# vitoplantamura/OnnxStream

Measured on AMD Instinct MI355X. Metric: sd15_unet_step_latency_ms+images_per_sec_512x512_20step, higher is better.
Workload: dtype f16

## Files before the change

### include/osgpu.h

```cpp
#ifndef OSGPU_H
#define OSGPU_H

#include <stddef.h>
#include <stdint.h>

#ifdef __cplusplus
extern "C" {
#endif

typedef struct osg_ctx osg_ctx;
typedef struct osg_graph osg_graph;

typedef enum { OSG_U8 = 1, OSG_F16 = 2, OSG_F32 = 3, OSG_I64 = 4 } osg_dtype;

typedef enum {
  OSG_ACT_NONE = 0,
  OSG_ACT_SILU = 1,
  OSG_ACT_SIGMOID = 2,
  OSG_ACT_GEGLU = 3
} osg_act;

typedef enum {
  OSG_UN_SIGMOID = 0,
  OSG_UN_ERF = 1,
  OSG_UN_SQRT = 2,
  OSG_UN_SIN = 3,
  OSG_UN_COS = 4,
  OSG_UN_NEG = 5,
  OSG_UN_POW = 6,
  OSG_UN_SILU = 7,
  OSG_UN_GELU_ERF = 8
} osg_unary_kind;

typedef enum {
  OSG_BIN_ADD = 0,
  OSG_BIN_SUB = 1,
  OSG_BIN_MUL = 2,
  OSG_BIN_DIV = 3
} osg_binary_kind;

int osg_device_count(void);
int osg_init(int device, osg_ctx** out);
void osg_destroy(osg_ctx* ctx);
const char* osg_last_error(const osg_ctx* ctx);
const char* osg_device_name(const osg_ctx* ctx);
void* osg_stream(const osg_ctx* ctx);
int osg_set_autotune(osg_ctx* ctx, int on);
int osg_tune_misses(void);

int osg_malloc(osg_ctx* ctx, size_t bytes, void** dptr);
int osg_free(osg_ctx* ctx, void* dptr);
int osg_upload(osg_ctx* ctx, void* dst, const void* host_src, size_t bytes);
int osg_upload_sync(osg_ctx* ctx, void* dst, const void* host_src, size_t bytes);
int osg_host_register(osg_ctx* ctx, void* host_ptr, size_t bytes);
int osg_host_unregister(osg_ctx* ctx, void* host_ptr);
int osg_upload_pinned(osg_ctx* ctx, void* dst, const void* pinned_host_src, size_t bytes);
int osg_upload_pinned_async(osg_ctx* ctx, void* dst, const void* pinned_host_src, size_t bytes);
int osg_copy_fence(osg_ctx* ctx);
int osg_download(osg_ctx* ctx, void* host_dst, const void* src, size_t bytes);
int osg_marker_record(osg_ctx* ctx, int slot);
int osg_copy_wait_marker(osg_ctx* ctx, int slot);
int osg_copy(osg_ctx* ctx, void* dst, const void* src, size_t bytes);
int osg_memset(osg_ctx* ctx, void* dst, int value, size_t bytes);
int osg_sync(osg_ctx* ctx);

int osg_graph_begin(osg_ctx* ctx);
int osg_graph_end(osg_ctx* ctx, osg_graph** out);
int osg_graph_launch(osg_ctx* ctx, osg_graph* g);
void osg_graph_destroy(osg_graph* g);

int osg_timer_start(osg_ctx* ctx);
int osg_timer_stop(osg_ctx* ctx, float* ms);
int osg_timer_mark(osg_ctx* ctx, int index);
int osg_timer_between(osg_ctx* ctx, int a, int b, float* ms);

void osg_range_push(const char* name);
void osg_range_pop(void);

int osg_conv2d_nhwc(osg_ctx* ctx, osg_dtype dtype, const void* x, const void* w_ohwi, const void* bias, osg_dtype bias_dtype,
                    const void* residual, void* y, int N, int H, int W, int Cin, int Cout, int KH, int KW, int stride_h,
                    int stride_w, int pad_top, int pad_left, int pad_bottom, int pad_right, osg_act act);

int osg_conv2d_nhwc_rb(osg_ctx* ctx, osg_dtype dtype, const void* x, const void* w_ohwi, const void* bias, osg_dtype bias_dtype,
                       const void* image_bias, long image_bias_ld, const void* residual, void* y, int N, int H, int W, int Cin, int Cout,
                       int KH, int KW, int stride_h, int stride_w, int pad_top, int pad_left, int pad_bottom, int pad_right, osg_act act);

int osg_conv2d_nhwc_v(osg_ctx* ctx, osg_dtype dtype, const void* x, const void* w_ohwi, const void* bias, osg_dtype bias_dtype,
                      const void* image_bias, long image_bias_ld, const void* residual, void* y, long y_ld, void* y2, long y2_ld, int N, int H, int W,
                      int Cin, int Cout, int KH, int KW, int stride_h, int stride_w, int pad_top, int pad_left, int pad_bottom, int pad_right,
                      osg_act act);

int osg_gemm(osg_ctx* ctx, osg_dtype dtype, const void* A, const void* B, int b_is_nk, const void* bias, osg_dtype bias_dtype,
             const void* residual, void* C, int M, int N, int K, int batch, long stride_a, long stride_b, long stride_c,
             osg_act act);

int osg_gemm_w8(osg_ctx* ctx, const void* A, const void* Bq_nk, float w_scale, int w_zero_point, const void* bias, osg_dtype bias_dtype,
                const void* residual, void* C, int M, int N, int K, osg_act act);
int osg_conv2d_nhwc_w8(osg_ctx* ctx, const void* x, const void* wq_ohwi, float w_scale, int w_zero_point, const void* bias,
                       osg_dtype bias_dtype, const void* image_bias, long image_bias_ld, const void* residual, void* y, int N, int H, int W,
                       int Cin, int Cout, int KH, int KW, int stride_h, int stride_w, int pad_top, int pad_left, int pad_bottom,
                       int pad_right, osg_act act);
int osg_gemm_w8_v(osg_ctx* ctx, const void* A, const void* Bq_nk, float w_scale, int w_zero_point, const float* w_scale_vec,
                  const float* w_zero_point_vec, const void* bias, osg_dtype bias_dtype, const void* residual, void* C, int M, int N, int K,
                  osg_act act);
int osg_conv2d_nhwc_w8_v(osg_ctx* ctx, const void* x, const void* wq_ohwi, float w_scale, int w_zero_point, const float* w_scale_vec,
                         const float* w_zero_point_vec, const void* bias, osg_dtype bias_dtype, const void* image_bias, long image_bias_ld,
                         const void* residual, void* y, long y_ld, void* y2, long y2_ld, int N, int H, int W, int Cin, int Cout, int KH, int KW,
                         int stride_h, int stride_w, int pad_top, int pad_left, int pad_bottom, int pad_right, osg_act act);

int osg_transpose_kn_to_nk(osg_ctx* ctx, osg_dtype dtype, const void* src_kn, void* dst_nk, int K, int N);
int osg_gemm_ln(osg_ctx* ctx, const void* x, const void* w_nk_folded, const float* c1, const float* c2, float eps, const float* rowstats,
                const void* residual, void* y, int M, int N, int K, osg_act act);
int osg_gemm_rowstats(osg_ctx* ctx, const void* A, const void* B_nk, const void* bias, osg_dtype bias_dtype, const void* residual, void* C,
                      int M, int N, int K, osg_act act, float* rowstats);
int osg_last_route(const osg_ctx* ctx, int out[5]);
int osg_last_kernel(const osg_ctx* ctx, int out[8]);

int osg_gemm_kernarg_check(osg_ctx* ctx, long lda, int splits);
int osg_attention_kernarg_check(osg_ctx* ctx, long kv_stride, int heads, int kv_div);

int osg_attention(osg_ctx* ctx, osg_dtype dtype, const void* q, const void* k, const void* v, void* o, int heads, int Tq, int Tkv,
                  int D, float scale, int k_is_dt);
int osg_attention_strided(osg_ctx* ctx, osg_dtype dtype, const void* q, long q_tok, long q_head, long q_batch, const void* k,
                          long k_tok, long k_head, long k_batch, const void* v, long v_tok, long v_head, long v_batch, void* o,
                          long o_tok, long o_head, long o_batch, int batch, int heads, int Tq, int Tkv, int D, float scale);
typedef struct {
  const void *a1, *x0;
  const void *wo1, *bo1;
  const void *g2, *be2;
  float eps2;
  const void *wq2, *bq2;
  const void *kp, *vtp;
  float scale;
  int Tk;
  const void *wo2, *bo2;
  const void *g3, *be3;
  float eps3;
  const void *w1, *b1, *w2, *b2;
  const void *wpo, *bpo, *xin;
  void *out, *out2;
  long ldo, ldo2;
  int M, rows_per_img, C, heads;
  void* dbg[8];
  int rows_per_block;
} osg_tblock_tail_args;
int osg_tblock_tail_supported(int M, int rows_per_img, int C, int heads, int Tk);
int osg_tblock_tail(osg_ctx* ctx, const osg_tblock_tail_args* a);
int osg_tblock_pack_weight(osg_ctx* ctx, const void* w_nk, int N, int K, void* w_kn8);
size_t osg_tblock_kv_pack_elems(int imgs, int heads, int D);
int osg_tblock_kv_pack_jobs(osg_ctx* ctx, const void* base, long ld, int imgs, int Tk, int heads, int njobs, const int* jobs_dev, void* dst);
int osg_rms_norm(osg_ctx* ctx, osg_dtype dtype, const void* x, const void* w, void* y, long rows, int C, float eps);
int osg_rope(osg_ctx* ctx, osg_dtype dtype, const void* x, const void* cos_t, const void* sin_t, void* y, long bh, long T, int d);
int osg_sdpa(osg_ctx* ctx, osg_dtype dtype, const void* q, const void* k, const void* v, const void* mask, void* o, int batch, int q_heads,
             int kv_heads, int Tq, int Tkv, int D, float scale);

int osg_instance_norm(osg_ctx* ctx, osg_dtype dtype, const void* x, const float* scale, const float* bias, void* y, int rows,
                      long L, int n_scale, float eps);
int osg_group_norm_nhwc(osg_ctx* ctx, osg_dtype dtype, const void* x, const void* gamma, const void* beta, void* y, int N, long HW,
                        int C, int groups, float eps, osg_act act);
int osg_set_stat_sinks(osg_ctx* ctx, void* table0, int groups0, int cpg0, int ch_off0, void* table1, int groups1, int cpg1, int ch_off1, int rows_per_image);
int osg_group_norm_stats_nhwc(osg_ctx* ctx, const void* x, const void* gamma, const void* beta, void* y, int N, long HW, int C, int G, float eps, osg_act act,
                              const void* stat_table);
int osg_layer_norm(osg_ctx* ctx, osg_dtype dtype, const void* x, const void* gamma, const void* beta, void* y, long rows, int C,
                   float eps);
int osg_reduce_mean_last(osg_ctx* ctx, osg_dtype dtype, const void* x, void* y, long rows, long C);
int osg_softmax_last(osg_ctx* ctx, osg_dtype dtype, const void* x, void* y, long rows, long C);

int osg_unary(osg_ctx* ctx, osg_dtype dtype, osg_unary_kind kind, const void* x, void* y, long n, float param);
int osg_binary(osg_ctx* ctx, osg_dtype dtype, osg_binary_kind kind, const void* a, const long* a_shape, const void* b,
               const long* b_shape, void* y, int rank);
int osg_geglu(osg_ctx* ctx, osg_dtype dtype, const void* x, void* y, long rows, long C);

int osg_sampler_prepare(osg_ctx* ctx, const float* x, float* sample, float* timestep, int prompts, long L, float c_in, float t,
                        long t_per_sample);
int osg_sampler_cfg_euler_a(osg_ctx* ctx, float* x, const float* eps, const float* noise, int prompts, long L, float c_out,
                            float guidance, float sigma, float d_sigma, float sigma_up, float clip);
typedef enum {
    OSG_MS_DPMPP_FIRST = 0, OSG_MS_DPMPP_2M = 1, OSG_MS_EULER_D = 2, OSG_MS_IPNDM1 = 3, OSG_MS_IPNDM_V1 = 4, OSG_MS_IPNDM2 = 5, OSG_MS_IPNDM3 = 6,
    OSG_MS_IPNDM_VO1 = 7, OSG_MS_IPNDM_VO2 = 8, OSG_MS_IPNDM_VO3 = 9, OSG_MS_TAYLOR1 = 10, OSG_MS_TAYLOR2 = 11, OSG_MS_DDIM = 12, OSG_MS_FORMS = 13
} osg_multistep_form;
int osg_sampler_cfg_multistep(osg_ctx* ctx, int form, float* x, const float* eps, float* h0, const float* h1, const float* h2, const float* h3,
                              int prompts, long L, float c_out, float guidance, float sigma, float k0, float k1, float k2, float k3, float k4,
                              double da, double db);
int osg_sampler_prepare_rescale(osg_ctx* ctx, float* x, float* sample, float* timestep, int prompts, long L, float x_scale, float c_in, float t,
                                long t_per_sample);
int osg_sampler_prepare_single(osg_ctx* ctx, float* x, float* sample, float* timestep, int prompts, long L, float x_scale, float c_in, float t,
                               long t_per_sample);
int osg_sampler_euler_a_single(osg_ctx* ctx, float* x, const float* eps, const float* noise, int prompts, long L, float c_out, float sigma,
                               float d_sigma, float sigma_up, float clip);
int osg_sampler_multistep_single(osg_ctx* ctx, int form, float* x, const float* eps, float* h0, const float* h1, const float* h2, const float* h3,
                                 int prompts, long L, float c_out, float sigma, float k0, float k1, float k2, float k3, float k4, double da,
                                 double db);

int osg_decode_gather(osg_ctx* ctx, const float* latents, float* tiles, int images, int H, int W, int tile, float factor);
int osg_decode_blend(osg_ctx* ctx, const float* tiles, float* image, unsigned char* pixels, int images, int H, int W, int tile, int up);

int osg_transpose(osg_ctx* ctx, int elem_size, const void* x, void* y, int rank, const long* shape, const int* perm);
int osg_copy_2d(osg_ctx* ctx, int elem_size, const void* src, long src_pitch, long src_off, void* dst, long dst_pitch,
                long dst_off, long outer, long inner);
int osg_concat2(osg_ctx* ctx, int elem_size, const void* a, long inner_a, const void* b, long inner_b, void* dst, long outer);
int osg_resize_nearest(osg_ctx* ctx, int elem_size, const void* x, void* y, int N, int C, int H, int W, int Ho, int Wo, int nhwc);
int osg_gather_rows(osg_ctx* ctx, int elem_size, const void* x, const int64_t* idx, void* y, long n_idx, long row_elems, long n_rows);
int osg_maxpool_nhwc(osg_ctx* ctx, osg_dtype dtype, const void* x, void* y, int N, int H, int W, int C, int KH, int KW, int sh,
                     int sw, int pt, int pl, int pb, int pr);

int osg_convert(osg_ctx* ctx, osg_dtype src_dtype, osg_dtype dst_dtype, const void* x, void* y, long n, float scale, int zero_point);

int osg_qu8_conv2d_nhwc(osg_ctx* ctx, const void* x, float x_scale, int x_zp, const void* w_ohwi, float w_scale, int w_zp, const float* bias_f32,
                        float out_scale, int out_zp, void* y, int N, int H, int W, int Cin, int Cout, int KH, int KW, int stride_h, int stride_w,
                        int pad_top, int pad_left, int pad_bottom, int pad_right);
int osg_qu8_conv_tap_sums(osg_ctx* ctx, const void* w_ohwi, int Cout, int KH, int KW, int Cin, int* tap_sums);
int osg_qu8_conv2d_nhwc_t(osg_ctx* ctx, const void* x, float x_scale, int x_zp, const void* w_ohwi, float w_scale, int w_zp, const float* bias_f32,
                          float out_scale, int out_zp, void* y, int N, int H, int W, int Cin, int Cout, int KH, int KW, int stride_h, int stride_w,
                          int pad_top, int pad_left, int pad_bottom, int pad_right, const int* tap_sums);
int osg_qu8_gemm(osg_ctx* ctx, const void* A, long lda, float a_scale, int a_zp, const void* B_nk, float b_scale, int b_zp, const float* bias_f32,
                 float out_scale, int out_zp, void* C, int M, int N, int K, int batch, long stride_a, long stride_b, long stride_c);
int osg_qu8_lut(osg_ctx* ctx, const void* x, void* y, long n, const void* lut256);
int osg_qu8_binary(osg_ctx* ctx, osg_binary_kind kind, const void* a, const long* a_shape, float a_scale, int a_zp, const void* b, const long* b_shape,
                   float b_scale, int b_zp, void* y, float out_scale, int out_zp, int rank);
int osg_qu8_instance_norm(osg_ctx* ctx, const void* x, void* y, int rows, long L, int n_scale, const float* scale, const float* bias, float eps,
                          float in_scale, int in_zp, float out_scale, int out_zp);
int osg_qu8_affine_act(osg_ctx* ctx, const void* x, float x_scale, int x_zp, const void* g, float g_scale, int g_zp, float m_scale, int m_zp, const void* b,
                       float b_scale, int b_zp, float a_scale, int a_zp, const void* sig_lut, float s_scale, int s_zp, float o_scale, int o_zp, void* y, long n, int C,
                       long inner);
int osg_qu8_norm_affine_act_nhwc(osg_ctx* ctx, const void* x, long HW, int C, int G, int n_scale, const float* scale, const float* bias, float eps, float x_scale,
                                 int x_zp, float n_out_scale, int n_out_zp, const void* g, float g_scale, int g_zp, float m_scale, int m_zp, const void* b, float b_scale,
                                 int b_zp, float a_scale, int a_zp, const void* sig_lut, float s_scale, int s_zp, float o_scale, int o_zp, void* y);
int osg_qu8_instance_norm_nhwc(osg_ctx* ctx, const void* x, void* y, long HW, int C, int G, int n_scale, const float* scale, const float* bias, float eps,
                               float in_scale, int in_zp, float out_scale, int out_zp);
int osg_qu8_softmax_last(osg_ctx* ctx, const void* x, void* y, long rows, long C, const void* lut_u32_256);

int osg_kdbg_read(osg_ctx* ctx, void* host_dst, size_t bytes);

#ifdef __cplusplus
}
#endif
#endif
```

### onnxstream_amd/csrc/osg_common.h

```cpp
#pragma once
#include <hip/hip_runtime.h>
#include <hip/hip_fp16.h>
#include <cstdio>
#include <cstdint>
#include <string>
#include <map>
#include <vector>
#include "osgpu.h"

struct osg_ctx {
    int device = 0;
    hipStream_t compute = nullptr;
    hipStream_t copy = nullptr;
    hipStream_t copy2 = nullptr;
    hipEvent_t ev_copy2 = nullptr;
    int copy_streams = 2, copy_rr = 0;
    bool copy_dirty[2] = {false, false};
    hipEvent_t ev_copy = nullptr;
    struct PendingSink { long long* table = nullptr; int groups = 0, cpg = 0, ch_off = 0; } pending_sink[2];
    int pending_hw = 0;
    bool tuning = false, sink_fused = false;
    int last_route[5] = {-1, -1, 0, 0, 0};
    int last_kernel[8] = {-1, 0, 0, 0, 0, 0, 0, 0};
    hipEvent_t ev_t0 = nullptr, ev_t1 = nullptr;
    static constexpr int kStages = 2;
    void* stage[kStages] = {nullptr, nullptr};
    hipEvent_t stage_free[kStages] = {nullptr, nullptr};
    size_t stage_bytes = 0;
    int stage_next = 0;
    void* ws = nullptr;
    size_t ws_bytes = 0;
    void* ws2 = nullptr;
    size_t ws2_bytes = 0;
    static constexpr long kTickets = 1 << 16;
    int* tickets = nullptr;
    bool xcd_ids8 = false;
    int* xcd_err = nullptr;
    int* xcd_err_dev = nullptr;
    bool capturing = false;
    bool autotune = false;
    hipEvent_t ev_a0 = nullptr, ev_a1 = nullptr;
    void* evict = nullptr;
    std::vector<hipEvent_t> marks;
    static constexpr int kMarkers = 256;
    hipEvent_t markers[kMarkers] = {};
    std::string err;
    std::string name;
    int num_cu = 256;
};

inline bool osg_first_on_device(unsigned long long& mask) {
    int dev = 0;
    if (hipGetDevice(&dev) != hipSuccess || dev < 0 || dev > 63) return true;
    if ((mask >> dev) & 1ull) return false;
    mask |= 1ull << dev;
    return true;
}

inline void osg_set_route(osg_ctx* ctx, int family, int instantiation, int splits, int fold) {
    int* r = ctx->last_route;
    r[0] = family; r[1] = instantiation; r[2] = splits; r[3] = fold; r[4] = 0;
}

inline void osg_set_kernel(osg_ctx* ctx, int family, int a = 0, int b = 0, int c = 0, int d = 0, int e = 0, int f = 0, int g = 0) {
    int* r = ctx->last_kernel;
    r[0] = family; r[1] = a; r[2] = b; r[3] = c; r[4] = d; r[5] = e; r[6] = f; r[7] = g;
}

struct osg_graph {
    hipGraph_t graph = nullptr;
    hipGraphExec_t exec = nullptr;
};

#define OSG_FAIL(ctx, msg)                 \
    do {                                   \
        (ctx)->err = (msg);                \
        return 1;                          \
    } while (0)

#define OSG_HIP(ctx, call)                                                                        \
    do {                                                                                          \
        hipError_t e__ = (call);                                                                  \
        if (e__ != hipSuccess) {                                                                  \
            (ctx)->err = std::string(#call) + ": " + hipGetErrorString(e__);                      \
            return 1;                                                                             \
        }                                                                                         \
    } while (0)

#define OSG_LAUNCH_CHECK(ctx)                                                                     \
    do {                                                                                          \
        hipError_t e__ = hipGetLastError();                                                       \
        if (e__ != hipSuccess) {                                                                  \
            (ctx)->err = std::string("kernel launch: ") + hipGetErrorString(e__);                 \
            return 1;                                                                             \
        }                                                                                         \
    } while (0)

int osg_ensure_workspace(osg_ctx* ctx, size_t bytes);
int osg_ensure_workspace2(osg_ctx* ctx, size_t bytes);

typedef _Float16 f16;
typedef _Float16 f16x8 __attribute__((ext_vector_type(8)));
typedef _Float16 f16x4 __attribute__((ext_vector_type(4)));
typedef _Float16 f16x2 __attribute__((ext_vector_type(2)));
typedef float f32x4 __attribute__((ext_vector_type(4)));
typedef float f32x16 __attribute__((ext_vector_type(16)));

__device__ __forceinline__ float osg_sigmoid(float x) {
    return __builtin_amdgcn_rcpf(1.0f + __builtin_amdgcn_exp2f(x * -1.44269504088896341f));
}
__device__ __forceinline__ float osg_gelu_erf(float g) {
    const float xs = g * 0.70710678118654752440f, ax = fabsf(xs);
    const float t = __builtin_amdgcn_rcpf(fmaf(0.3275911f, ax, 1.0f));
    const float poly = ((((1.061405429f * t - 1.453152027f) * t + 1.421413741f) * t - 0.284496736f) * t + 0.254829592f) * t;
    const float e = __builtin_amdgcn_exp2f(ax * ax * -1.44269504088896341f);
    const float er = copysignf(fmaf(-poly, e, 1.0f), xs);
    return 0.5f * g * (1.0f + er);
}
__device__ __forceinline__ float osg_apply_act(float v, int act) {
    if (act == OSG_ACT_SILU) return v * osg_sigmoid(v);
    if (act == OSG_ACT_SIGMOID) return osg_sigmoid(v);
    return v;
}

template <typename T> __device__ __forceinline__ float to_f32(T v);
template <> __device__ __forceinline__ float to_f32<f16>(f16 v) { return (float)v; }
template <> __device__ __forceinline__ float to_f32<float>(float v) { return v; }
template <typename T> __device__ __forceinline__ T from_f32(float v);
template <> __device__ __forceinline__ f16 from_f32<f16>(float v) { return (f16)v; }
template <> __device__ __forceinline__ float from_f32<float>(float v) { return v; }

template <class T>
__device__ __forceinline__ void osg_pin_one(const T& v) { asm volatile("" ::"s"(v)); }
template <class... T>
__device__ __forceinline__ void osg_pin_all(const T&... v) { (osg_pin_one(v), ...); }

template <int CTRL>
__device__ __forceinline__ float osg_dpp(float v) {
    return __int_as_float(__builtin_amdgcn_update_dpp(0, __float_as_int(v), CTRL, 0xf, 0xf, false));
}
__device__ __forceinline__ float wave_sum_valu(float v) {
    v += osg_dpp<0xB1>(v);
    v += osg_dpp<0x4E>(v);
    v += osg_dpp<0x124>(v);
    v += osg_dpp<0x128>(v);
    float a = v, b = v;
    asm volatile("s_nop 1\n\tv_permlane16_swap_b32 %0, %1" : "+v"(a), "+v"(b));
    v = a + b;
    a = v; b = v;
    asm volatile("s_nop 1\n\tv_permlane32_swap_b32 %0, %1" : "+v"(a), "+v"(b));
    return a + b;
}

__device__ __forceinline__ float wave_sum(float v) {
#pragma unroll
    for (int o = 32; o > 0; o >>= 1) v += __shfl_xor(v, o, 64);
    return v;
}
__device__ __forceinline__ float wave_max(float v) {
#pragma unroll
    for (int o = 32; o > 0; o >>= 1) v = fmaxf(v, __shfl_xor(v, o, 64));
    return v;
}
```

### onnxstream_amd/csrc/osg_ctx.hip

```cpp
#include "osg_common.h"
#include "osg_gemm_common.h"
#include "osg_tune.h"
#include <algorithm>
#include <cstring>
#include <map>
#include <mutex>
#include <set>

namespace osg_tune {
static std::mutex g_mu;
static std::map<Key, Choice> g_table;
static bool g_loaded = false;
static const char* cache_path() { return getenv("OSG_TUNE_CACHE"); }
static void load_locked() {
    if (g_loaded) return;
    g_loaded = true;
    const char* path = cache_path();
    if (!path) return;
    FILE* f = fopen(path, "r");
    if (!f) return;
    Key k{};
    Choice c{};
    while (fscanf(f, "%d %d %d %d %d %d %d %d %d %d %d %d %d %d %d %d %d %d %f", &k.kind, &k.device, &k.M, &k.N, &k.K, &k.batch, &k.H, &k.W, &k.Cin, &k.KW,
                  &k.sh, &k.sw, &k.flags, &c.family, &c.cfg, &c.nst, &c.splits, &c.bn, &c.us) == 19) {
// ... 50 lines not shown
    int (*pop)() = nullptr;
    Roctx() {
        void* h = dlopen("libroctx64.so", RTLD_NOW | RTLD_GLOBAL);
        if (!h) h = dlopen("libroctx64.so.4", RTLD_NOW | RTLD_GLOBAL);
        if (!h) return;
        push = (int (*)(const char*))dlsym(h, "roctxRangePushA");
        pop = (int (*)())dlsym(h, "roctxRangePop");
    }
};
Roctx& roctx() { static Roctx r; return r; }
}

namespace {
__global__ void xcc_probe_kernel(int* out) {
    unsigned v;
    asm volatile("s_getreg_b32 %0, hwreg(HW_REG_XCC_ID)" : "=s"(v));
    if (threadIdx.x == 0) out[blockIdx.x] = (int)(v & 15u);
}

void calibrate_xcd(osg_ctx* c) {
    constexpr int kBlocks = 256;
    int* d = nullptr;
    int h[kBlocks];
    if (hipHostMalloc((void**)&c->xcd_err, 64, hipHostMallocMapped) != hipSuccess) { c->xcd_err = nullptr; return; }
    *c->xcd_err = 0;
    if (hipHostGetDevicePointer((void**)&c->xcd_err_dev, c->xcd_err, 0) != hipSuccess) return;
    if (hipMalloc((void**)&d, sizeof(h)) != hipSuccess) return;
    bool ok = true;
    for (int rep = 0; rep < 3 && ok; rep++) {
        hipLaunchKernelGGL(xcc_probe_kernel, dim3(kBlocks), dim3(64), 0, c->compute, d);
        ok = hipMemcpyAsync(h, d, sizeof(h), hipMemcpyDeviceToHost, c->compute) == hipSuccess && hipStreamSynchronize(c->compute) == hipSuccess;
        for (int i = 0; ok && i < kBlocks; i++) ok = h[i] == h[i & 7];
        for (int i = 0; ok && i < 8; i++)
            for (int j = 0; j < i; j++) ok = ok && h[i] != h[j];
    }
    (void)hipGetLastError();
    hipFree(d);
    if (getenv("OSG_XCD_DEBUG")) {
        fprintf(stderr, "[osg] XCC_ID of workgroups 0..15 of a launch:");
        for (int i = 0; i < 16; i++) fprintf(stderr, " %d", h[i]);
        fprintf(stderr, "  -> round robin over 8 XCDs: %s\n", ok ? "yes" : "no");
    }
    if (!ok) return;
    c->xcd_ids8 = true;
    for (int i = 0; i < 8; i++) c->xcd_ids8 = c->xcd_ids8 && h[i] >= 0 && h[i] < 8;
}

int xcd_check(osg_ctx* c) {
    if (c->xcd_err && *(volatile int*)c->xcd_err) {
        const int what = *(volatile int*)c->xcd_err;
        *c->xcd_err = 0;
        if (c->tickets && hipMemsetAsync(c->tickets, 0, osg_ctx::kTickets * sizeof(int), c->compute) == hipSuccess) hipStreamSynchronize(c->compute);
        if (what == 2) OSG_FAIL(c, "split-K fold: a k-slice workgroup did not publish its partial sums within 20 ms (results of this pass are invalid); set OSG_SPLITK_FOLD=0");
        OSG_FAIL(c, "split-K fold: the device raised its error flag (results of this pass are invalid); set OSG_SPLITK_FOLD=0");
    }
    return 0;
}
}

extern "C" {

void osg_range_push(const char* name) { if (roctx().push) roctx().push(name); }
void osg_range_pop(void) { if (roctx().pop) roctx().pop(); }

int osg_device_count(void) {
    int n = 0;
    if (hipGetDeviceCount(&n) != hipSuccess) return 0;
    return n;
}

int osg_init(int device, osg_ctx** out) {
    if (!out) return 1;
    *out = nullptr;
    int n = 0;
    if (hipGetDeviceCount(&n) != hipSuccess || n <= 0) return 2;
    if (device < 0 || device >= n) return 3;
    if (hipSetDevice(device) != hipSuccess) return 4;
    osg_ctx* c = new osg_ctx();
    c->device = device;
    hipDeviceProp_t prop;
    if (hipGetDeviceProperties(&prop, device) == hipSuccess) {
        c->name = prop.gcnArchName;
        c->num_cu = prop.multiProcessorCount;
    }
    bool ok = hipStreamCreateWithFlags(&c->compute, hipStreamNonBlocking) == hipSuccess &&
              hipStreamCreateWithFlags(&c->copy, hipStreamNonBlocking) == hipSuccess &&
              hipStreamCreateWithFlags(&c->copy2, hipStreamNonBlocking) == hipSuccess &&
              hipEventCreateWithFlags(&c->ev_copy2, hipEventDisableTiming) == hipSuccess &&
              hipEventCreateWithFlags(&c->ev_copy, hipEventDisableTiming) == hipSuccess &&
              hipEventCreate(&c->ev_t0) == hipSuccess && hipEventCreate(&c->ev_t1) == hipSuccess &&
              hipEventCreate(&c->ev_a0) == hipSuccess && hipEventCreate(&c->ev_a1) == hipSuccess;
    c->stage_bytes = 64u << 20;
    if (const char* e = getenv("OSG_COPY_STREAMS")) c->copy_streams = atoi(e) > 1 ? 2 : 1;
    for (int i = 0; ok && i < osg_ctx::kStages; i++) {
        ok = hipHostMalloc(&c->stage[i], c->stage_bytes, hipHostMallocDefault) == hipSuccess &&
             hipEventCreateWithFlags(&c->stage_free[i], hipEventDisableTiming) == hipSuccess;
    }
    ok = ok && hipMalloc((void**)&c->tickets, osg_ctx::kTickets * sizeof(int)) == hipSuccess &&
         hipMemsetAsync(c->tickets, 0, osg_ctx::kTickets * sizeof(int), c->compute) == hipSuccess &&
         hipStreamSynchronize(c->compute) == hipSuccess;
    if (!ok) {
        delete c;
        return 5;
    }
    calibrate_xcd(c);
    *out = c;
    return 0;
}

void osg_destroy(osg_ctx* c) {
    if (!c) return;
    hipSetDevice(c->device);
    hipDeviceSynchronize();
    for (int i = 0; i < osg_ctx::kStages; i++) {
        if (c->stage[i]) hipHostFree(c->stage[i]);
        if (c->stage_free[i]) hipEventDestroy(c->stage_free[i]);
    }
    if (c->tickets) hipFree(c->tickets);
    if (c->xcd_err) hipHostFree(c->xcd_err);
    if (c->evict) hipFree(c->evict);
    if (c->ws) hipFree(c->ws);
    if (c->ws2) hipFree(c->ws2);
    if (c->ev_copy) hipEventDestroy(c->ev_copy);
    if (c->ev_copy2) hipEventDestroy(c->ev_copy2);
    if (c->copy2) hipStreamDestroy(c->copy2);
    if (c->ev_t0) hipEventDestroy(c->ev_t0);
    if (c->ev_t1) hipEventDestroy(c->ev_t1);
    if (c->ev_a0) hipEventDestroy(c->ev_a0);
    if (c->ev_a1) hipEventDestroy(c->ev_a1);
    for (auto& e : c->markers)
        if (e) hipEventDestroy(e);
    for (auto& e : c->marks)
        if (e) hipEventDestroy(e);
    if (c->compute) hipStreamDestroy(c->compute);
    if (c->copy) hipStreamDestroy(c->copy);
    delete c;
}

int osg_set_autotune(osg_ctx* c, int on) {
    if (!c) return 1;
    c->autotune = on != 0;
    return 0;
}

const char* osg_last_error(const osg_ctx* c) { return c ? c->err.c_str() : "null context"; }
const char* osg_device_name(const osg_ctx* c) { return c ? c->name.c_str() : ""; }
void* osg_stream(const osg_ctx* c) { return c ? (void*)c->compute : nullptr; }
int osg_last_route(const osg_ctx* c, int out[5]) {
    if (!c || !out) return 1;
    for (int i = 0; i < 5; i++) out[i] = c->last_route[i];
    return 0;
}

int osg_last_kernel(const osg_ctx* c, int out[8]) {
    if (!c || !out) return 1;
    for (int i = 0; i < 8; i++) out[i] = c->last_kernel[i];
    return 0;
}

int osg_malloc(osg_ctx* c, size_t bytes, void** dptr) {
    if (c->capturing) OSG_FAIL(c, "osg_malloc inside graph capture");
    OSG_HIP(c, hipSetDevice(c->device));
    OSG_HIP(c, hipMalloc(dptr, bytes ? bytes : 16));
    return 0;
}

int osg_free(osg_ctx* c, void* dptr) {
    if (!dptr) return 0;
    OSG_HIP(c, hipFree(dptr));
    return 0;
}

int osg_upload(osg_ctx* c, void* dst, const void* src, size_t bytes) {
    if (c->capturing) OSG_FAIL(c, "osg_upload inside graph capture");
    const char* s = (const char*)src;
    char* d = (char*)dst;
    size_t off = 0;
    while (off < bytes) {
        size_t n = bytes - off < c->stage_bytes ? bytes - off : c->stage_bytes;
        int i = c->stage_next;
        c->stage_next = (i + 1) % osg_ctx::kStages;
        OSG_HIP(c, hipEventSynchronize(c->stage_free[i]));
        std::memcpy(c->stage[i], s + off, n);
        OSG_HIP(c, hipMemcpyAsync(d + off, c->stage[i], n, hipMemcpyHostToDevice, c->copy));
        OSG_HIP(c, hipEventRecord(c->stage_free[i], c->copy));
        off += n;
    }
    OSG_HIP(c, hipEventRecord(c->ev_copy, c->copy));
    OSG_HIP(c, hipStreamWaitEvent(c->compute, c->ev_copy, 0));
    return 0;
}

int osg_upload_pinned(osg_ctx* c, void* dst, const void* pinned_src, size_t bytes) {
    if (c->capturing) OSG_FAIL(c, "osg_upload_pinned inside graph capture");
    OSG_HIP(c, hipMemcpyAsync(dst, pinned_src, bytes, hipMemcpyHostToDevice, c->copy));
    OSG_HIP(c, hipEventRecord(c->ev_copy, c->copy));
    OSG_HIP(c, hipStreamWaitEvent(c->compute, c->ev_copy, 0));
    return 0;
}

int osg_upload_pinned_async(osg_ctx* c, void* dst, const void* pinned_src, size_t bytes) {
    if (c->capturing) OSG_FAIL(c, "osg_upload_pinned_async inside graph capture");
    const int q = c->copy_streams > 1 ? (c->copy_rr++ & 1) : 0;
    OSG_HIP(c, hipMemcpyAsync(dst, pinned_src, bytes, hipMemcpyHostToDevice, q ? c->copy2 : c->copy));
    c->copy_dirty[q] = true;
    return 0;
}

int osg_copy_fence(osg_ctx* c) {
    if (c->capturing) OSG_FAIL(c, "osg_copy_fence inside graph capture");
    if (c->copy_dirty[0]) {
        OSG_HIP(c, hipEventRecord(c->ev_copy, c->copy));
        OSG_HIP(c, hipStreamWaitEvent(c->compute, c->ev_copy, 0));
        c->copy_dirty[0] = false;
    }
    if (c->copy_dirty[1]) {
        OSG_HIP(c, hipEventRecord(c->ev_copy2, c->copy2));
        OSG_HIP(c, hipStreamWaitEvent(c->compute, c->ev_copy2, 0));
        c->copy_dirty[1] = false;
    }
    return 0;
}

int osg_marker_record(osg_ctx* c, int slot) {
    if (slot < 0 || slot >= osg_ctx::kMarkers) OSG_FAIL(c, "osg_marker_record: slot out of range");
    if (c->capturing) OSG_FAIL(c, "osg_marker_record inside graph capture");
    if (!c->markers[slot]) OSG_HIP(c, hipEventCreateWithFlags(&c->markers[slot], hipEventDisableTiming));
    OSG_HIP(c, hipEventRecord(c->markers[slot], c->compute));
    return 0;
}

int osg_copy_wait_marker(osg_ctx* c, int slot) {
    if (slot < 0 || slot >= osg_ctx::kMarkers) OSG_FAIL(c, "osg_copy_wait_marker: slot out of range");
    if (!c->markers[slot]) return 0;
    OSG_HIP(c, hipStreamWaitEvent(c->copy, c->markers[slot], 0));
    OSG_HIP(c, hipStreamWaitEvent(c->copy2, c->markers[slot], 0));
    return 0;
}

int osg_host_register(osg_ctx* c, void* ptr, size_t bytes) {
    OSG_HIP(c, hipHostRegister(ptr, bytes, hipHostRegisterDefault));
    return 0;
}

int osg_host_unregister(osg_ctx* c, void* ptr) {
    OSG_HIP(c, hipHostUnregister(ptr));
    return 0;
}

int osg_upload_sync(osg_ctx* c, void* dst, const void* src, size_t bytes) {
    if (c->capturing) OSG_FAIL(c, "osg_upload_sync inside graph capture");
    OSG_HIP(c, hipMemcpyAsync(dst, src, bytes, hipMemcpyHostToDevice, c->compute));
    OSG_HIP(c, hipStreamSynchronize(c->compute));
    return 0;
}

int osg_download(osg_ctx* c, void* dst, const void* src, size_t bytes) {
    if (c->capturing) OSG_FAIL(c, "osg_download inside graph capture");
    OSG_HIP(c, hipMemcpyAsync(dst, src, bytes, hipMemcpyDeviceToHost, c->compute));
    OSG_HIP(c, hipStreamSynchronize(c->compute));
    return xcd_check(c);
}

int osg_copy(osg_ctx* c, void* dst, const void* src, size_t bytes) {
    OSG_HIP(c, hipMemcpyAsync(dst, src, bytes, hipMemcpyDeviceToDevice, c->compute));
    return 0;
}

int osg_memset(osg_ctx* c, void* dst, int value, size_t bytes) {
    OSG_HIP(c, hipMemsetAsync(dst, value, bytes, c->compute));
    return 0;
}

int osg_sync(osg_ctx* c) {
    OSG_HIP(c, hipStreamSynchronize(c->copy));
    OSG_HIP(c, hipStreamSynchronize(c->copy2));
    OSG_HIP(c, hipStreamSynchronize(c->compute));
    return xcd_check(c);
}

int osg_graph_begin(osg_ctx* c) {
    if (c->capturing) OSG_FAIL(c, "already capturing");
    OSG_HIP(c, hipStreamSynchronize(c->copy));
    OSG_HIP(c, hipStreamSynchronize(c->copy2));
    if (c->tickets) OSG_HIP(c, hipMemsetAsync(c->tickets, 0, osg_ctx::kTickets * sizeof(int), c->compute));
    OSG_HIP(c, hipStreamBeginCapture(c->compute, hipStreamCaptureModeThreadLocal));
    c->capturing = true;
    return 0;
}

int osg_graph_end(osg_ctx* c, osg_graph** out) {
    if (!c->capturing) OSG_FAIL(c, "not capturing");
    c->capturing = false;
    hipGraph_t g = nullptr;
    OSG_HIP(c, hipStreamEndCapture(c->compute, &g));
    hipGraphExec_t ex = nullptr;
    hipError_t e = hipGraphInstantiate(&ex, g, nullptr, nullptr, 0);
    if (e != hipSuccess) {
        hipGraphDestroy(g);
        OSG_FAIL(c, std::string("hipGraphInstantiate: ") + hipGetErrorString(e));
    }
    osg_graph* r = new osg_graph();
    r->graph = g;
    r->exec = ex;
    *out = r;
    return 0;
// ... 80 lines not shown
```

### onnxstream_amd/csrc/osg_gemm.hip

```cpp
#include "osg_gemm_common.h"
#include "osg_tune.h"
#include <algorithm>
#include <climits>
#include <cmath>
#include <cstdio>
#include <cstdlib>

using namespace osg_mm;

namespace {

template <int BM, int BN, int BK, bool CONV, bool VEC>
__global__ __launch_bounds__(256) void gemm_kernel(GemmParams p) {
    constexpr int LDS = BK + 8;
    constexpr int CPR = BK / 8;
    constexpr int ROWS_PER_PASS = 256 / CPR;
    constexpr int A_IT = BM / ROWS_PER_PASS;
    constexpr int B_IT = BN / ROWS_PER_PASS;
    constexpr int WM = BM / 2, WN = BN / 2;
    constexpr int TM = WM / 16, TN = WN / 16;
    static_assert(A_IT >= 1 && B_IT >= 1, "tile too small for 256 threads");

    extern __shared__ __attribute__((aligned(16))) f16 smem[];
    f16* As0 = smem;
// ... 241 lines not shown
        if (p.C2) *reinterpret_cast<f16x4*>(p.C2 + (long)m * p.ldc2 + n) = o;
    }
}

__global__ __launch_bounds__(256) void splitk_reduce_kernel(const float* __restrict__ partial, f16* __restrict__ C,
                                                            const void* __restrict__ bias, int bias_f32,
                                                            const f16* __restrict__ residual, long MN, int N, int splits, int batch,
                                                            long strideC, int act, const f16* __restrict__ rowbias, int rb_rows, long rb_ld, long ldc,
                                                            f16* __restrict__ C2, long ldc2) {
    long idx = (long)blockIdx.x * 256 + threadIdx.x;
    long total = MN * batch;
    if (idx >= total) return;
    int b = (int)(idx / MN);
    long e = idx - (long)b * MN;
    float v = 0.f;
    for (int s = 0; s < splits; s++) v += partial[((long)(b * splits + s)) * MN + e];
    int n = (int)(e % N);
    if (bias) v += bias_f32 ? ((const float*)bias)[n] : (float)((const f16*)bias)[n];
    if (rowbias) v += (float)rowbias[(e / N / rb_rows) * rb_ld + n];
    if (residual) v += (float)residual[b * strideC + e];
    const f16 o = (f16)osg_apply_act(v, act);
    if (ldc == N && !C2) C[b * strideC + e] = o;
    else {
        const long m = e / N;
        C[m * ldc + n] = o;
        if (C2) C2[m * ldc2 + n] = o;
    }
}

template <int SB>
__global__ __launch_bounds__(256) void splitk_reduce4_kernel(const float* __restrict__ partial, f16* __restrict__ C, const void* __restrict__ bias, int bias_f32,
                                                             const f16* __restrict__ residual, long MN, int N, int splits, int batch, long strideC, int act,
                                                             const f16* __restrict__ rowbias, int rb_rows, long rb_ld, long ldc, f16* __restrict__ C2, long ldc2) {
    osg_pin_all(partial, C, bias, bias_f32, residual, MN, N, splits, batch, strideC, act, rowbias, rb_rows, rb_ld, ldc, C2, ldc2);
    const long idx = ((long)blockIdx.x * 256 + threadIdx.x) * 4;
    const long total = MN * batch;
    if (idx >= total) return;
    const int b = (int)(idx / MN);
    const long e = idx - (long)b * MN;
    const long m = e / N;
    const int n = (int)(e - m * N);
    const bool has_b32 = bias && bias_f32, has_b16 = bias && !bias_f32;
    const f16* safe = reinterpret_cast<const f16*>(partial);
    const f32x4 bv_l = *reinterpret_cast<const f32x4*>(has_b32 ? (const float*)bias + n : partial);
    const f16x4 b16_l = *reinterpret_cast<const f16x4*>(has_b16 ? (const f16*)bias + n : safe);
    const f16x4 rb_l = *reinterpret_cast<const f16x4*>(rowbias ? rowbias + (m / (rb_rows > 0 ? rb_rows : 1)) * rb_ld + n : safe);
    const f16x4 rv_l = *reinterpret_cast<const f16x4*>(residual ? residual + b * strideC + e : safe);
    const float* src = partial + (long)b * splits * MN + e;
    f32x4 v = {0.f, 0.f, 0.f, 0.f};
    for (int s0 = 0; s0 < splits; s0 += SB) {
        f32x4 part[SB];
#pragma unroll
        for (int u = 0; u < SB; u++) part[u] = *reinterpret_cast<const f32x4*>(src + (long)min(s0 + u, splits - 1) * MN);
#pragma unroll
        for (int u = 0; u < SB; u++)
            if (s0 + u < splits) v += part[u];
    }
#pragma unroll
    for (int r = 0; r < 4; r++) {
        v[r] += bias ? (has_b32 ? bv_l[r] : (float)b16_l[r]) : -0.0f;
        v[r] += rowbias ? (float)rb_l[r] : -0.0f;
        v[r] += residual ? (float)rv_l[r] : -0.0f;
    }
    f16x4 o;
#pragma unroll
    for (int r = 0; r < 4; r++) o[r] = (f16)osg_apply_act(v[r], act);
    if (ldc == N && !C2) *reinterpret_cast<f16x4*>(C + b * strideC + e) = o;
    else {
        *reinterpret_cast<f16x4*>(C + m * ldc + n) = o;
        if (C2) *reinterpret_cast<f16x4*>(C2 + m * ldc2 + n) = o;
    }
}

template <int BM, int BN, int BK, bool CONV, bool VEC>
int launch_cfg(osg_ctx* ctx, const GemmParams& p, int batch) {
    constexpr int LDS = BK + 8;
    size_t smem = (size_t)2 * (BM + BN) * LDS * sizeof(f16);
    auto kern = gemm_kernel<BM, BN, BK, CONV, VEC>;
    static unsigned long long attr_mask = 0;
    if (osg_first_on_device(attr_mask) && smem > 48 * 1024) {
        OSG_HIP(ctx, hipFuncSetAttribute((const void*)kern, hipFuncAttributeMaxDynamicSharedMemorySize, (int)smem));
    }
    dim3 grid((p.N + BN - 1) / BN, (p.M + BM - 1) / BM, batch * p.splits);
    hipLaunchKernelGGL(kern, grid, dim3(256), smem, ctx->compute, p);
    OSG_LAUNCH_CHECK(ctx);
    return 0;
}


static KeyForm key_form(const GemmParams& p) {
    KeyForm f;
    f.act = (int)p.act; f.residual = p.residual != nullptr; f.rowbias = p.rowbias != nullptr; f.bias_f32 = p.bias_f32 != 0; f.ln = p.ln_c1 != nullptr;
    f.rs_in = p.rs_in != nullptr; f.rs_out = p.rs_out != nullptr; f.w8 = p.w8 != 0;
    return f;
}
static bool tune_safe(const GemmParams& p) { return (const void*)p.C != (const void*)p.A && (const void*)p.C != (const void*)p.residual; }

static V2Form v2_form(const GemmParams& p, bool conv) {
    V2Form f;
    f.conv = conv; f.ln1 = p.ln_c1 && !p.rs_in; f.ln2 = p.ln_c1 && p.rs_in; f.geglu = p.act == OSG_ACT_GEGLU; f.rowstats = p.rs_out != nullptr; f.w8 = p.w8 != 0;
    f.nch = v2_nch(p.rs_np);
    return f;
}

template <class Candidates, class Launch>
int run_measured(osg_ctx* ctx, const osg_tune::Key& key, const GemmParams& p, const char* what, Candidates&& candidates, Launch&& launch) {
    osg_tune::Choice row;
    if (!osg_tune::lookup(key, &row)) {
        const std::vector<Candidate> cands = candidates();
        row = cands.empty() ? tune_row(V2Choice{0, 4, 1}) : cands[0].row;
        if (!ctx->capturing && tune_safe(p) && !cands.empty() && !osg_tune::frozen()) {
            static const bool dump = getenv("OSG_TUNE_DUMP") != nullptr;
            row.us = -1.f;
            for (const Candidate& c : cands) {
                const float us = osg_tune::time_us(ctx, [&] { return launch(c.row); });
                if (dump && c.row.family == 1) {
                    const Halo3Choice h = row_halo3(c.row);
                    fprintf(stderr, "[tune] %s M=%d N=%d K=%d flags=%d: halo bn=%d splits=%d loaders=%d fold=%d -> %.2f us (model %.0f)\n", what, p.M, p.N, p.K, key.flags, h.bn, h.splits,
                            h.loaders, h.fold, us, c.model);
                } else if (dump) {
                    const V2Choice v = row_v2(c.row);
                    fprintf(stderr, "[tune] %s M=%d N=%d K=%d flags=%d: tile %dx%d nst=%d splits=%d ks=%d fold=%d spec=%d -> %.2f us (model %.0f)\n", what, p.M, p.N, p.K, key.flags,
                            kV2BM[v.cfg], kV2BN[v.cfg], v.nst, v.splits, v.ks, v.fold, v.spec, us, c.model);
                }
                if (us >= 0.f && (row.us < 0.f || us < row.us)) { row = c.row; row.us = us; }
            }
            if (row.us < 0.f) OSG_FAIL(ctx, "osg_gemm / osg_conv2d_nhwc: autotune could not time any configuration");
            osg_tune::store(key, row);
        } else if (osg_tune::frozen())
            osg_tune::remember(key, row);
    }
    return launch(row);
}

template <bool CONV>
int launch_v2_choice(osg_ctx* ctx, GemmParams p, int batch, V2Choice ch) {
    const V2Route r = resolve_v2(ch, v2_form(p, CONV));
    if (r.entry < 0) OSG_FAIL(ctx, "osg_gemm: no kernel takes this form (LayerNorm or row statistics with uint8 weight codes, LayerNorm in a convolution)");
    const V2Entry& e = kV2Entries[r.entry];
    const auto [slices, kt_per] = split_slices(p.K / 64, ch.splits);
    p.splits = slices;
    p.k_per_split = kt_per * 64;
    p.tickets = nullptr;
    p.fold_acc = 0;
    if (p.splits > 1) {
        size_t need = (size_t)batch * p.splits * p.M * p.N * sizeof(float);
        if (r.fold) need = std::max(need, osg_mm::splitk_fold_route(ctx, p, (long)batch * ((p.M + e.bm - 1) / e.bm) * ((p.N + e.bn - 1) / e.bn), e.bm, e.bn));
        if (osg_ensure_workspace(ctx, need)) return 1;
        p.partial = (float*)ctx->ws;
    }
    const double a_unique = CONV ? (double)p.a_bytes : (double)p.M * p.K * 2.0;
    p.n_major = (double)p.N * p.K * (p.w8 ? 1.0 : 2.0) > a_unique;
    static constexpr int (*units[4])(int, osg_ctx*, GemmParams&, int) = {launch_v2_unit<0>, launch_v2_unit<1>, launch_v2_unit<2>, launch_v2_unit<3>};
    if (const int rc = units[v2_unit(e)](r.entry, ctx, p, batch)) return rc;
    osg_set_route(ctx, 0, r.entry, p.splits, p.fold_acc);
    if (p.splits > 1 && !p.fold_acc) return launch_splitk_reduce(ctx, p, batch);
    return 0;
}

template <bool CONV>
int run_gemm_v2(osg_ctx* ctx, GemmParams p, int batch, const V2Choice* forced) {
    if (forced) return launch_v2_choice<CONV>(ctx, p, batch, *forced);
    const SelectEnv env = select_env(ctx);
    const V2Form form = v2_form(p, CONV);
    if (env.measured && !apply_knobs<V2Choice>(kGemmKnobs, nullptr))
        return run_measured(ctx, tune_key(CONV ? 2 : 0, select_shape(p, batch), key_form(p)), p, CONV ? "conv" : "gemm",
                            [&] { return gemm_candidates(env, p.M, p.N, p.K, batch, form); },
                            [&](const osg_tune::Choice& row) { return launch_v2_choice<CONV>(ctx, p, batch, row_v2(row)); });
    V2Choice ch = model_choice(env, p.M, p.N, p.K, batch, form);
    apply_knobs(kGemmKnobs, &ch);
    if (!v2_allows_split(form)) ch.splits = 1;
    return launch_v2_choice<CONV>(ctx, p, batch, ch);
}

template <bool CONV>
int run_gemm(osg_ctx* ctx, GemmParams p, int batch, const V2Choice* forced = nullptr) {
    if (epi_check(ctx, p)) return 1;
    {
        static const bool force_v1 = getenv("OSG_GEMM_V1") != nullptr;
        const bool shape_ok = v2_takes(select_shape(p, batch), CONV);
        const bool align_ok = (((uintptr_t)p.A | (uintptr_t)p.Bt) & 15) == 0 && (p.strideA % 8 == 0) && (p.strideB % 8 == 0);
        const double a_ext = CONV ? (double)p.a_bytes_l : ((double)(p.M - 1) * p.lda + p.K) * 2.0;
        const double b_ext = (double)p.N * p.K * (p.w8 ? 1.0 : 2.0);
        if (p.w8 && !(shape_ok && align_ok && a_ext < 2147483648.0 && b_ext < 2147483648.0))
            OSG_FAIL(ctx, "osg_gemm_w8 / osg_conv2d_nhwc_w8: K (Cin) must be a multiple of 64, the operands 16-byte aligned and smaller than 2 GiB");
        if ((!force_v1 || p.w8) && shape_ok && align_ok && a_ext < 2147483648.0 && b_ext < 2147483648.0) {
            p.a_bytes = (unsigned)a_ext;
            p.b_bytes = (unsigned)b_ext;
            return run_gemm_v2<CONV>(ctx, p, batch, forced);
        }
        if (p.act == OSG_ACT_GEGLU) OSG_FAIL(ctx, "osg_gemm: GEGLU epilogue needs 16-byte aligned operands (direct-to-LDS kernel only)");
        if (p.ln_c1 || p.rs_out) OSG_FAIL(ctx, "osg_gemm_ln / osg_gemm_rowstats: need K % 64 == 0 and 16-byte aligned operands (direct-to-LDS kernel only)");
    }
    const bool vec = CONV ? (p.Cin % 8 == 0) : (p.K % 8 == 0 && p.lda % 8 == 0);
    const V1Choice v1 = choose_v1(ctx->num_cu, p.M, p.N, p.K, batch);
    const int cfg = v1.cfg, BK = 32;
    const auto [splits, kt_per] = split_slices((p.K + BK - 1) / BK, v1.splits);
    p.splits = splits;
    p.k_per_split = kt_per * BK;
    if (splits > 1) {
        size_t need = (size_t)batch * splits * p.M * p.N * sizeof(float);
        if (osg_ensure_workspace(ctx, need)) return 1;
        p.partial = (float*)ctx->ws;
    }
    int rc;
#define OSG_DISPATCH(BM_, BN_)                                                   \
    (vec ? launch_cfg<BM_, BN_, 32, CONV, true>(ctx, p, batch) : launch_cfg<BM_, BN_, 32, CONV, false>(ctx, p, batch))
    if (cfg == 0) rc = OSG_DISPATCH(128, 128);
    else if (cfg == 1) rc = OSG_DISPATCH(128, 64);
    else rc = OSG_DISPATCH(64, 64);
#undef OSG_DISPATCH
    if (rc) return rc;
    osg_set_route(ctx, 2, cfg | (vec ? 4 : 0) | (CONV ? 8 : 0), splits, 0);
    if (splits > 1) return launch_splitk_reduce(ctx, p, batch);
    return 0;
}


__global__ __launch_bounds__(256) void transpose_kn_nk_kernel(const f16* __restrict__ src, f16* __restrict__ dst, int K, int N) {
    __shared__ f16 tile[32][33];
    int k0 = blockIdx.y * 32, n0 = blockIdx.x * 32;
    int tx = threadIdx.x & 31, ty = threadIdx.x >> 5;
    for (int r = ty; r < 32; r += 8) {
        int k = k0 + r, n = n0 + tx;
        tile[r][tx] = (k < K && n < N) ? src[(long)k * N + n] : (f16)0;
    }
    __syncthreads();
    for (int r = ty; r < 32; r += 8) {
        int n = n0 + r, k = k0 + tx;
        if (n < N && k < K) dst[(long)n * K + k] = tile[tx][r];
    }
}

}

template <int SB>
__global__ __launch_bounds__(256) void splitk_reduce_stats_kernel(const float* __restrict__ partial, f16* __restrict__ C, const void* __restrict__ bias, int bias_f32,
                                                                  const f16* __restrict__ residual, int M, int N, int splits, int act, const f16* __restrict__ rowbias,
                                                                  int rb_rows, long rb_ld, long ldc, f16* __restrict__ C2, long ldc2, StatSink s0, StatSink s1, int hw,
                                                                  int imgs, int per_xcd) {
    osg_pin_all(partial, C, bias, bias_f32, residual, M, N, splits, act, rowbias, rb_rows, rb_ld, ldc, C2, ldc2, hw, imgs, per_xcd);
    constexpr int RPT = 2;
    __shared__ float st[16][64][2];
    const int cq = threadIdx.x & 15, rl = threadIdx.x >> 4;
    const int m0 = blockIdx.x * 32, n0 = blockIdx.y * 64, n = n0 + cq * 4;
    const long MN = (long)M * N;
    float cs[4] = {0.f, 0.f, 0.f, 0.f}, cq2[4] = {0.f, 0.f, 0.f, 0.f};
    if (n < N) {
        const bool has_b32 = bias && bias_f32, has_b16 = bias && !bias_f32;
        const f16* safe = reinterpret_cast<const f16*>(partial);
        const f32x4 bv_l = *reinterpret_cast<const f32x4*>(has_b32 ? (const float*)bias + n : partial);
        const f16x4 b16_l = *reinterpret_cast<const f16x4*>(has_b16 ? (const f16*)bias + n : safe);
        f32x4 part[RPT][SB];
        f16x4 rb_l[RPT], rv_l[RPT];
#pragma unroll
        for (int k = 0; k < RPT; k++) {
            const int m = min(m0 + rl + 16 * k, M - 1);
            const long e = (long)m * N + n;
            rb_l[k] = *reinterpret_cast<const f16x4*>(rowbias ? rowbias + (long)(m / (rb_rows > 0 ? rb_rows : 1)) * rb_ld + n : safe);
            rv_l[k] = *reinterpret_cast<const f16x4*>(residual ? residual + e : safe);
#pragma unroll
            for (int u = 0; u < SB; u++) part[k][u] = *reinterpret_cast<const f32x4*>(partial + (long)min(u, splits - 1) * MN + e);
        }
#pragma unroll
        for (int k = 0; k < RPT; k++) {
            const int m = m0 + rl + 16 * k;
            if (m >= M) break;
            const long e = (long)m * N + n;
            f32x4 v = {0.f, 0.f, 0.f, 0.f};
#pragma unroll
            for (int u = 0; u < SB; u++)
                if (u < splits) v += part[k][u];
            for (int z0 = SB; z0 < splits; z0 += SB) {
                f32x4 more[SB];
#pragma unroll
                for (int u = 0; u < SB; u++) more[u] = *reinterpret_cast<const f32x4*>(partial + (long)min(z0 + u, splits - 1) * MN + e);
#pragma unroll
                for (int u = 0; u < SB; u++)
                    if (z0 + u < splits) v += more[u];
            }
            f16x4 o;
#pragma unroll
            for (int r = 0; r < 4; r++) {
                float x = v[r];
                x += bias ? (has_b32 ? bv_l[r] : (float)b16_l[r]) : -0.0f;
                x += rowbias ? (float)rb_l[k][r] : -0.0f;
                x += residual ? (float)rv_l[k][r] : -0.0f;
                o[r] = (f16)osg_apply_act(x, act);
                const float f = (float)o[r];
                cs[r] += f;
                cq2[r] = fmaf(f, f, cq2[r]);
            }
            *reinterpret_cast<f16x4*>(C + (long)m * ldc + n) = o;
            if (C2) *reinterpret_cast<f16x4*>(C2 + (long)m * ldc2 + n) = o;
        }
    }
#pragma unroll
    for (int r = 0; r < 4; r++) { st[rl][cq * 4 + r][0] = cs[r]; st[rl][cq * 4 + r][1] = cq2[r]; }
    __syncthreads();
    if (threadIdx.x >= 64) return;
    const int lane = threadIdx.x, wn = min(64, N - n0), n_img = m0 / hw;
    const StatSink sk[2] = {s0, s1};
    for (int k = 0; k < 2; k++) {
        if (!sk[k].table) continue;
        const int c_lo = n0 + sk[k].ch_off, c_hi = c_lo + wn;
        const int g = c_lo / sk[k].cpg + lane;
        if (g * sk[k].cpg < c_hi) {
            const int a = max(g * sk[k].cpg, c_lo) - c_lo, b = min((g + 1) * sk[k].cpg, c_hi) - c_lo;
// ... 287 lines not shown
```

### onnxstream_amd/csrc/osg_gemm2.h

```cpp
#pragma once
#include "osg_gemm_common.h"
#include "osg_tune.h"
#include <array>
#include <type_traits>

#ifndef OSG_GEMM_PIN
#define OSG_GEMM_PIN 1
#endif

namespace {
using namespace osg_mm;

template <int BM, int BN, int NST, bool CONV, int MODE = 0, int SPEC = 0, int LN = 0, int NCH = 5, int KS = 1, int WGN = 2, int WQ = 0>
__global__ __launch_bounds__((SPEC || KS == 2) ? 512 : 256) void gemm2_kernel(const void* A, const void* Bt, int M, int N, int K, int k_per_split, unsigned a_bytes, unsigned b_bytes,
                                                                              int grid, int lda, unsigned sp_nm, GemmParams pk) {
    GemmParams p = pk;
    p.A = (const f16*)A; p.Bt = (const f16*)Bt; p.M = M; p.N = N; p.K = K; p.k_per_split = k_per_split; p.a_bytes = a_bytes; p.b_bytes = b_bytes; p.grid = grid; p.lda = lda;
    p.splits = (int)(sp_nm & ((1u << kPackSplitsBits) - 1)); p.n_major = (sp_nm & kPackNMajor) != 0;
    p.mt = (M + BM - 1) / BM; p.nt = (N + BN - 1) / BN;
    p.kdbg = nullptr;
    if (OSG_UNLIKELY(sp_nm & kPackKdbg)) p.kdbg = kernarg_rare(pk.kdbg);
#if OSG_GEMM_PIN
    if constexpr (CONV) {
        OSG_PIN(p.H); OSG_PIN(p.W); OSG_PIN(p.Cin); OSG_PIN(p.Ho); OSG_PIN(p.Wo); OSG_PIN(p.KW); OSG_PIN(p.sh); OSG_PIN(p.sw); OSG_PIN(p.pt); OSG_PIN(p.pl);
    }
    if constexpr (WQ) { OSG_PIN(p.wq_sc); OSG_PIN(p.wq_zp); OSG_PIN(p.w_zp); }
    if constexpr (LN == 2) { OSG_PIN(p.rs_in); OSG_PIN(p.rs_np); }
#endif
    static_assert(KS == 1 || (KS == 2 && !SPEC && MODE == 0 && LN != 1), "KS = 2: plain kernel only (row statistics come from the producer, LN = 2, or not at all)");
    static_assert(WGN == 1 || WGN == 2, "wave grid: 2 x 2 or 4 x 1");
    static_assert(!WQ || LN == 0, "W8: no folded LayerNorm");
    constexpr int ROWB = 128;
    constexpr int ROWB_B = WQ ? 64 : 128;
    constexpr int BRW = WQ ? 16 : 8;
    constexpr int BNP = (BN + 4 * BRW - 1) / (4 * BRW) * (4 * BRW);
    constexpr int A_BYTES = BM * ROWB, B_BYTES = BNP * ROWB_B, GSTAGE = A_BYTES + B_BYTES, STAGE = KS * GSTAGE;
    constexpr int A_LD = BM / 32, B_LD = BNP / (4 * BRW);
    constexpr int WM = BM / (4 / WGN), WN = BN / WGN, TM = WM / 16, TN = WN / 16;
    static_assert(BM % 32 == 0 && WM % 16 == 0 && WN % 16 == 0, "a wave's part of the tile is made of whole 16 x 16 blocks");
    constexpr int INFLIGHT = (NST - 2) * (A_LD + B_LD);
    constexpr unsigned OOB = 0x80000000u;
    static_assert(INFLIGHT <= 63, "vmcnt is a 6-bit counter");

    extern __shared__ __attribute__((aligned(16))) char smem2[];
    typedef __attribute__((address_space(3))) void* lds_ptr;

    kdbg_stamp(p, 0);
    const int tid = threadIdx.x;
    const int lane = tid & 63;
    const int wave8 = __builtin_amdgcn_readfirstlane(tid >> 6);
    const bool loader = SPEC && wave8 >= 4, math = !SPEC || wave8 < 4;
    const bool loads = !SPEC || loader;
    const int wave = wave8 & 3;
    const int grp = KS == 2 ? (wave8 >> 2) : 0;
    const int wm0 = (WGN == 2 ? (wave >> 1) : wave) * WM;
    const int wn0 = (WGN == 2 ? (wave & 1) : 0) * WN;

    const int total = p.grid;
    int L;
    {
        const int bid = blockIdx.x, x = bid & 7, i = bid >> 3, q = total >> 3, r = total & 7;
        L = (x < r ? x * (q + 1) : r * (q + 1) + (x - r) * q) + i;
    }
    const int per_batch = p.mt * p.nt * p.splits;
    int zb, m_tile, n_tile, zs;
    {
        zb = L / (per_batch);
        int rem = L - zb * per_batch;
        if (p.n_major) {
            n_tile = rem / (p.splits * p.mt); rem -= n_tile * p.splits * p.mt;
            zs = rem / (p.mt); m_tile = rem - zs * p.mt;
        } else {
            m_tile = rem / (p.splits * p.nt); rem -= m_tile * p.splits * p.nt;
            zs = rem / (p.nt); n_tile = rem - zs * p.nt;
        }
    }
    const int m0 = m_tile * BM, n0 = n_tile * BN;
    const int kbeg = zs * p.k_per_split;
    const int kend = min(p.K, kbeg + p.k_per_split);
    const int nkt = (kend - kbeg) >> 6;
    const int nsteps = (nkt + KS - 1) / KS;

    const f16* Ab = p.A;
    const f16* Bb = p.Bt;
    if (OSG_UNLIKELY(sp_nm & kPackBatch)) {
        Ab += (long)zb * kernarg_rare(pk.strideA);
        Bb += (long)zb * kernarg_rare(pk.strideB);
    }
    __amdgpu_buffer_rsrc_t rsA = __builtin_amdgcn_make_buffer_rsrc((void*)Ab, 0, p.a_bytes, 0x00020000);
    __amdgpu_buffer_rsrc_t rsB = __builtin_amdgcn_make_buffer_rsrc((void*)Bb, 0, p.b_bytes, 0x00020000);

    const int rsub = lane >> 3;
    const int gch = (lane & 7) ^ rsub;
    int a_base[A_LD];
    int a_hi0[A_LD], a_wi0[A_LD];
#pragma unroll
    for (int j = 0; j < A_LD; j++) {
        const int m = m0 + (j * 4 + wave) * 8 + rsub;
        if (CONV) {
            const int mm = m < p.M ? m : 0;
            const int hw = p.Ho * p.Wo;
            const int n_img = mm / hw;
            const int r2 = mm - n_img * hw;
            const int ho = r2 / p.Wo, wo = r2 - ho * p.Wo;
            a_hi0[j] = m < p.M ? ho * p.sh - p.pt : -0x40000000;
            a_wi0[j] = wo * p.sw - p.pl;
            a_base[j] = (((n_img * p.H + (ho * p.sh - p.pt)) * p.W + (wo * p.sw - p.pl)) * p.Cin + gch * 8) * 2;
        } else {
            a_base[j] = m < p.M ? (int)(((long)m * p.lda + gch * 8) * 2) : (int)OOB;
            a_hi0[j] = a_wi0[j] = 0;
        }
    }
    int b_base[B_LD];
#pragma unroll
    for (int j = 0; j < B_LD; j++) {
        if constexpr (WQ) {
            const int nl = (j * 4 + wave) * 16 + (lane >> 2), n = n0 + nl;
            b_base[j] = (n < p.N && (BNP == BN || nl < BN)) ? (int)((long)n * p.K + (((lane & 3) ^ ((lane >> 4) & 3)) << 4)) : (int)OOB;
        } else {
            const int nl = (j * 4 + wave) * 8 + rsub, n = n0 + nl;
            b_base[j] = (n < p.N && (BNP == BN || nl < BN)) ? (int)(((long)n * p.K + gch * 8) * 2) : (int)OOB;
        }
    }

    int ik = kbeg + 64 * grp, i_c0 = 0, i_kh = 0, i_kw = 0;
    if (CONV) {
        const int cell = ik / p.Cin;
        i_c0 = ik - cell * p.Cin;
        i_kh = cell / p.KW;
        i_kw = cell - i_kh * p.KW;
    }
    auto issue_tile = [&](int stage) {
        char* As = smem2 + stage * STAGE + grp * GSTAGE;
        char* Bs = As + A_BYTES;
        const bool live = ik < kend;
        const unsigned kill = live ? 0u : OOB;
        if (CONV) {
            const int tap_off = ((i_kh * p.W + i_kw) * p.Cin + i_c0) * 2;
#pragma unroll
            for (int j = 0; j < A_LD; j++) {
                const int hi = a_hi0[j] + i_kh, wi = a_wi0[j] + i_kw;
                const bool ok = live && (unsigned)hi < (unsigned)p.H && (unsigned)wi < (unsigned)p.W;
                const unsigned off = ok ? (unsigned)(a_base[j] + tap_off) : OOB;
                __builtin_amdgcn_raw_ptr_buffer_load_lds(rsA, (lds_ptr)(As + (j * 4 + wave) * 1024), 16, off, 0, 0, 0);
            }
#pragma unroll
            for (int adv = 0; adv < KS; adv++) {
                i_c0 += 64;
                if (i_c0 >= p.Cin) { i_c0 = 0; if (++i_kw == p.KW) { i_kw = 0; ++i_kh; } }
            }
        } else {
#pragma unroll
            for (int j = 0; j < A_LD; j++)
                __builtin_amdgcn_raw_ptr_buffer_load_lds(rsA, (lds_ptr)(As + (j * 4 + wave) * 1024), 16, (unsigned)a_base[j] | kill, ik * 2, 0, 0);
        }
#pragma unroll
        for (int j = 0; j < B_LD; j++)
            __builtin_amdgcn_raw_ptr_buffer_load_lds(rsB, (lds_ptr)(Bs + (j * 4 + wave) * 1024), 16, (unsigned)b_base[j] | kill, WQ ? ik : ik * 2, 0, 0);
        ik += 64 * KS;
    };

    f32x4 acc[TM][TN];
#pragma unroll
    for (int i = 0; i < TM; i++)
#pragma unroll
        for (int j = 0; j < TN; j++) acc[i][j] = f32x4{0.f, 0.f, 0.f, 0.f};

    const int frow = lane & 15;
    const int fsw = (((lane >> 4) ^ (frow & 7)) << 4);
    const int a_rd = (wm0 + frow) * ROWB + fsw;
    const int b_rd = WQ ? A_BYTES + (wn0 + frow) * ROWB_B + ((((lane >> 5) & 1) ^ ((frow >> 2) & 3)) << 4) + ((lane >> 4) & 1) * 8 : A_BYTES + (wn0 + frow) * ROWB + fsw;

    f32x4 pst[LN == 2 ? NCH : 1];
    if constexpr (LN == 2) {
        const int m = min(m0 + wm0 + (lane & 15) + 16 * ((lane >> 4) % TM), p.M - 1);
        const float* src = p.rs_in + (long)m * p.rs_np * 2;
        const int nch = p.rs_np >> 1;
#pragma unroll
        for (int c = 0; c < NCH; c++)
            pst[c] = *reinterpret_cast<const f32x4*>(src + 4 * min(c, nch - 1));
        asm volatile("" ::: "memory");
    }

    constexpr bool EPRE = TM * TN <= 8;
    W8Ops<WQ ? TN : 1, true> w8;
    if constexpr (WQ) { if (math) w8_prefetch<TN, true>(p, w8, n0, wn0, lane); }
    if (loads) {
#pragma unroll
        for (int s2 = 0; s2 < NST - 1; s2++) issue_tile(s2);
    }
#if OSG_GEMM_PIN
    OSG_PIN(p.bias); OSG_PIN(p.residual); OSG_PIN(p.rowbias); OSG_PIN(p.rb_ld); OSG_PIN(p.strideC); OSG_PIN(p.ln_c1); OSG_PIN(p.rb_rows);
    OSG_PIN(p.bias_f32); OSG_PIN(p.act); OSG_PIN(p.no_epre);
#endif
    EpiOps<TM, TN, CONV, EPRE> epre;
    epre.have = false;
    if (math && !p.ln_c1 && grp == 0) epi_prefetch<TM, TN, CONV, EPRE>(p, epre, m0, n0, wm0, wn0, lane, zb);
    kdbg_stamp(p, 1);
    if constexpr (WQ) { if (math) w8_finalize<TN, true>(w8); }

    float ls[TM], lq[TM];
#pragma unroll
    for (int i = 0; i < TM; i++) ls[i] = lq[i] = 0.f;

    int cur = 0, nxt = NST - 1;
    for (int kt = 0; kt < nsteps; kt++) {
        if (loads) asm volatile("s_waitcnt vmcnt(%0)" ::"n"(INFLIGHT) : "memory");
        __builtin_amdgcn_s_barrier();
        if (kt == 0) kdbg_stamp(p, 2);
        if (loads) issue_tile(nxt);
        const char* St = smem2 + cur * STAGE + grp * GSTAGE;
        if (math)
#pragma unroll
        for (int ks = 0; ks < (MODE == 1 ? 0 : 2); ks++) {
            f16x8 a[TM], b[TN];
#pragma unroll
            for (int i = 0; i < TM; i++) a[i] = *reinterpret_cast<const f16x8*>(St + ((a_rd + i * 16 * ROWB) ^ (ks << 6)));
#pragma unroll
            for (int j = 0; j < TN; j++) {
                if constexpr (WQ) b[j] = w8_frag(*reinterpret_cast<const u32x2v*>(St + ((b_rd + j * 16 * ROWB_B) ^ (ks << 5))), w8.zz[j]);
                else b[j] = *reinterpret_cast<const f16x8*>(St + ((b_rd + j * 16 * ROWB) ^ (ks << 6)));
            }
#pragma unroll
            for (int i = 0; i < TM; i++)
#pragma unroll
                for (int j = 0; j < TN; j++) acc[i][j] = __builtin_amdgcn_mfma_f32_16x16x32_f16(b[j], a[i], acc[i][j], 0, 0, 0);
            if constexpr (LN == 1) ln_accumulate<TM>(a, ls, lq);
        }
        cur = cur + 1 == NST ? 0 : cur + 1;
        nxt = nxt + 1 == NST ? 0 : nxt + 1;
    }
    kdbg_stamp(p, 3);
    asm volatile("s_waitcnt vmcnt(0)" ::: "memory");
    if (loader) return;
    if constexpr (WQ) w8_scale_acc<TM, TN>(w8, acc);
    if constexpr (KS == 2) {
        __builtin_amdgcn_s_barrier();
        f32x4* red = reinterpret_cast<f32x4*>(smem2) + (wave * (TM * TN + 1)) * 64 + lane;
        if (grp == 1) {
#pragma unroll
            for (int i = 0; i < TM; i++)
#pragma unroll
                for (int j = 0; j < TN; j++) red[(i * TN + j) * 64] = acc[i][j];
        }
        asm volatile("s_waitcnt lgkmcnt(0)" ::: "memory");
        __builtin_amdgcn_s_barrier();
        if (grp == 1) return;
#pragma unroll
        for (int i = 0; i < TM; i++)
#pragma unroll
            for (int j = 0; j < TN; j++) acc[i][j] += red[(i * TN + j) * 64];
    }
    if constexpr (LN == 2) {
        const int nch = p.rs_np >> 1;
        float S = 0.f, Q = 0.f;
#pragma unroll
        for (int c = 0; c < NCH; c++) {
            asm volatile("" : "+v"(pst[c]));
            if (c < nch) { S += pst[c][0] + pst[c][2]; Q += pst[c][1] + pst[c][3]; }
        }
#pragma unroll
        for (int i = 0; i < TM; i++) {
            ls[i] = __shfl(S, (lane & 15) + 16 * i, 64);
            lq[i] = __shfl(Q, (lane & 15) + 16 * i, 64);
        }
    }
    if constexpr (LN != 0) ln_apply<TM, TN, LN == 1>(p, acc, ls, lq, n0, wn0, lane);
    if (OSG_UNLIKELY_IF(!SPEC, p.act == OSG_ACT_GEGLU)) {
        if constexpr (TN % 2 == 0) gemm_epilogue_geglu<TM, TN>(p, acc, m0, n0, wm0, wn0, lane, zb);
        return;
    }
    kdbg_stamp(p, 4);
    float* stat_lds = nullptr;
    if (OSG_UNLIKELY_IF(!SPEC, p.sink[0].table || p.sink[1].table)) {
        __builtin_amdgcn_s_barrier();
        stat_lds = reinterpret_cast<float*>(smem2) + wave * (WN * 2);
    }
    if constexpr (KS == 1 && !SPEC && LN == 0 && MODE == 0) {
        if (OSG_UNLIKELY_IF(!SPEC, p.splits > 1 && p.fold_acc)) {
            if (!splitk_fold_acc<TM, TN>(p, acc, (zb * p.mt + m_tile) * p.nt + n_tile, zs, reinterpret_cast<int*>(smem2), tid)) return;
            EpiOps<TM, TN, CONV, false> none;
            none.have = false;
            gemm_epilogue_fast<TM, TN, CONV, false>(p, acc, m0, n0, wm0, wn0, lane, zb, none, nullptr);
            return;
        }
    }
    gemm_epilogue<TM, TN, CONV, EPRE, !SPEC>(p, acc, m0, n0, wm0, wn0, lane, zb, zb * p.splits + zs, epre, stat_lds);
    kdbg_stamp(p, 5);
    if (OSG_UNLIKELY_IF(!SPEC, p.kdbg != nullptr)) { asm volatile("s_waitcnt vmcnt(0)" ::: "memory"); kdbg_stamp(p, 6); }
}

template <int BM, int BN, int NST, bool CONV, int MODE = 0, int SPEC = 0, int LN = 0, int NCH = 5, int KS = 1, int WGN = 2, int WQ = 0>
int launch_v2(osg_ctx* ctx, GemmParams& p, int batch) {
    constexpr size_t smem = WQ ? (size_t)NST * KS * (BM * 128 + (BN + 63) / 64 * 64 * 64) : (size_t)NST * KS * (BM + (BN + 31) / 32 * 32) * 128;
    static_assert(smem <= 160 * 1024, "LDS budget");
    static_assert(KS == 1 || (size_t)4 * ((BM / 32) * (BN / 32) + 1) * 1024 <= smem, "KS = 2: the accumulator hand-over must fit the ring");
    auto kern = gemm2_kernel<BM, BN, NST, CONV, MODE, SPEC, LN, NCH, KS, WGN, WQ>;
    static unsigned long long attr_mask = 0;
    if (osg_first_on_device(attr_mask)) {
        OSG_HIP(ctx, hipFuncSetAttribute((const void*)kern, hipFuncAttributeMaxDynamicSharedMemorySize, (int)smem));
    }
    p.mt = (p.M + BM - 1) / BM;
    p.nt = (p.N + BN - 1) / BN;
    dim3 grid((unsigned)(p.mt * p.nt * batch * p.splits));
    p.grid = (int)grid.x;
    p.no_epre = osg_mm::no_epi_prefetch();
    p.kdbg = kdbg_buffer(ctx, grid.x);
    const osg_mm::StatSink sinks_in[2] = {p.sink[0], p.sink[1]};
    if (p.sink[0].table || p.sink[1].table) {
        const bool ok = !ctx->tuning && p.splits == 1 && batch == 1 && MODE == 0 && LN == 0 && !SPEC && p.act != OSG_ACT_GEGLU && (p.N & 3) == 0 && ((p.ldc | p.ldc2) & 3) == 0 &&
                        p.sink_hw > 0 && p.sink_hw % BM == 0 && p.M % p.sink_hw == 0;
        if (ok) { ctx->sink_fused = true; p.sink_imgs = p.M / p.sink_hw; p.sink_per_xcd = ctx->xcd_ids8 ? 1 : 0; }
        else p.sink[0].table = p.sink[1].table = nullptr;
    }
    int lda32;
    unsigned sp_nm;
    const int bad = kernarg_pack(ctx, p.lda, p.splits, p.n_major, p.kdbg != nullptr, batch > 1, &lda32, &sp_nm);
    if (!bad) hipLaunchKernelGGL(kern, grid, dim3((SPEC || KS == 2) ? 512 : 256), smem, ctx->compute, (const void*)p.A, (const void*)p.Bt, p.M, p.N, p.K, p.k_per_split, p.a_bytes, p.b_bytes, p.grid, lda32, sp_nm, p);
    p.sink[0] = sinks_in[0]; p.sink[1] = sinks_in[1];
    if (bad) return 1;
    OSG_LAUNCH_CHECK(ctx);
    return 0;
}

using V2Launch = int (*)(osg_ctx*, GemmParams&, int);
template <int UNIT, int I>
constexpr V2Launch v2_launcher() {
    constexpr V2Entry e = kV2Entries[I];
    if constexpr (v2_unit(e) == UNIT) return launch_v2<e.bm, e.bn, e.nst, e.conv != 0, 0, e.spec, e.ln, e.nch, e.ks, e.wgn, e.wq>;
    else return nullptr;
}
template <int UNIT, size_t... I>
constexpr std::array<V2Launch, kV2Count> v2_launchers(std::index_sequence<I...>) { return {v2_launcher<UNIT, (int)I>()...}; }
template <int UNIT>
int launch_v2_in_unit(int entry, osg_ctx* ctx, GemmParams& p, int batch) {
    static constexpr std::array<V2Launch, kV2Count> table = v2_launchers<UNIT>(std::make_index_sequence<kV2Count>{});
    return table[entry](ctx, p, batch);
}

}
```

### onnxstream_amd/csrc/osg_gemm_common.h

```cpp
#pragma once
#include <utility>
#include <vector>
#include "osg_common.h"
#include "osg_gemm_select.h"

#include <algorithm>
#include <type_traits>
#ifndef OSG_EPI_STORE_AUX
#define OSG_EPI_STORE_AUX 0
#endif
namespace osg_mm {

struct StatSink {
    long long* table;
    int groups, cpg, ch_off;
};
constexpr int kStatCopies = 8;
constexpr float kStatSX = 1048576.f;
__host__ __device__ inline int stat_q_shift(long elems) {
    int lg = 0;
    while ((1L << lg) < elems) lg++;
    const int e = 36 - lg;
    return e < 10 ? 10 : (e > 20 ? 20 : e);
}
__host__ __device__ inline float stat_q_scale(long elems) { return (float)(1L << stat_q_shift(elems)); }

struct GemmParams {
    const f16* A;
    const f16* Bt;
    long long* kdbg;
    long lda;
    long strideA, strideB;
    int M, N, K;
    int splits, k_per_split;
    unsigned a_bytes, b_bytes;
    int mt, nt, n_major;
    int grid;
    int H, W, Cin, Ho, Wo, KW, sh, sw, pt, pl;
    const void* bias;
    const f16* residual;
    const f16* rowbias;
    long rb_ld;
    long strideC;
    const float* ln_c1;
    const float* rs_in;
    int rb_rows;
    int bias_f32, act;
    int no_epre;
    int rs_np;
    unsigned rb_bytes;
    f16* C;
    float* partial;
    long a_bytes_l;
    int* tickets;
    int* xcd_err;
    float w_scale;
    int w_zp;
    const float* wq_sc;
    const float* wq_zp;
    int w8;
    float ln_eps;
    float* rs_out;
    long ldc;
    f16* C2;
    long ldc2;
    StatSink sink[2];
    int sink_hw;
    int sink_imgs, sink_per_xcd;
    int fold_acc;
};
constexpr int kPackSplitsBits = 16;
constexpr unsigned kPackNMajor = 1u << 16, kPackKdbg = 1u << 17, kPackBatch = 1u << 18;
template <class T>
__device__ __forceinline__ T kernarg_rare(T v) {
    asm volatile("" : "+s"(v));
    return v;
}
inline int kernarg_pack(osg_ctx* ctx, long lda, int splits, int n_major, bool kdbg, bool batched, int* lda32, unsigned* sp_nm) {
    if (lda < 0 || lda > 0x7fffffffL) {
        ctx->err = "contraction launch: the row pitch of A does not fit the 32-bit kernel parameter";
        return 1;
    }
    if (splits < 1 || splits >= (1 << kPackSplitsBits)) {
        ctx->err = "contraction launch: the number of k-slices does not fit its 16-bit kernel parameter field";
        return 1;
    }
    *lda32 = (int)lda;
    *sp_nm = (unsigned)splits | (n_major ? kPackNMajor : 0u) | (kdbg ? kPackKdbg : 0u) | (batched ? kPackBatch : 0u);
    return 0;
}
#define OSG_PIN(x) asm volatile("" ::"s"(x))
#define OSG_LIKELY(x) __builtin_expect(!!(x), 1)
#define OSG_UNLIKELY(x) __builtin_expect(!!(x), 0)
#define OSG_UNLIKELY_IF(h, x) ((h) ? __builtin_expect(!!(x), 0) : !!(x))

typedef unsigned int u32x2v __attribute__((ext_vector_type(2)));
typedef _Float16 f16x2w __attribute__((ext_vector_type(2)));
__device__ __forceinline__ f16x8 w8_frag(u32x2v c, f16x2w zz) {
    union { unsigned u; f16x2w h; } d0, d1, d2, d3;
    d0.u = __builtin_amdgcn_perm(0x64646464u, c[0], 0x04010400u);
    d1.u = __builtin_amdgcn_perm(0x64646464u, c[0], 0x04030402u);
    d2.u = __builtin_amdgcn_perm(0x64646464u, c[1], 0x04010400u);
    d3.u = __builtin_amdgcn_perm(0x64646464u, c[1], 0x04030402u);
    d0.h -= zz; d1.h -= zz; d2.h -= zz; d3.h -= zz;
    return f16x8{d0.h[0], d0.h[1], d1.h[0], d1.h[1], d2.h[0], d2.h[1], d3.h[0], d3.h[1]};
}
template <int TN, bool SC = true>
struct W8Ops {
    float zraw[TN];
    f16x2w zz[TN];
    f32x4 sc[SC ? TN : 1];
};
template <int TN, bool SC>
__device__ __forceinline__ void w8_prefetch(const GemmParams& p, W8Ops<TN, SC>& w, int n0, int wn0, int lane) {
    if (p.wq_sc) {
#pragma unroll
        for (int j = 0; j < TN; j++) {
            w.zraw[j] = p.wq_zp[min(n0 + wn0 + j * 16 + (lane & 15), p.N - 1)];
            if constexpr (SC) w.sc[j] = *reinterpret_cast<const f32x4*>(p.wq_sc + min(n0 + wn0 + j * 16 + (lane >> 4) * 4, p.N - 4));
        }
    } else {
#pragma unroll
        for (int j = 0; j < TN; j++) {
            w.zraw[j] = (float)p.w_zp;
            if constexpr (SC) w.sc[j] = f32x4{p.w_scale, p.w_scale, p.w_scale, p.w_scale};
        }
    }
    asm volatile("" ::: "memory");
}
template <int TN, bool SC>
__device__ __forceinline__ void w8_finalize(W8Ops<TN, SC>& w) {
#pragma unroll
    for (int j = 0; j < TN; j++) {
        const f16 h = (f16)(1024.0f + w.zraw[j]);
        w.zz[j] = f16x2w{h, h};
    }
}
template <int TM, int TN>
__device__ __forceinline__ void w8_scale_acc(const W8Ops<TN, true>& w, f32x4 (&acc)[TM][TN]) {
#pragma unroll
    for (int i = 0; i < TM; i++)
#pragma unroll
        for (int j = 0; j < TN; j++) acc[i][j] *= w.sc[j];
}
template <int TM, int TN>
__device__ __forceinline__ void w8_scale_acc_late(const GemmParams& p, f32x4 (&acc)[TM][TN], int n0, int wn0, int lane) {
#pragma unroll
    for (int j = 0; j < TN; j++) {
        f32x4 s = {p.w_scale, p.w_scale, p.w_scale, p.w_scale};
        if (p.wq_sc) s = *reinterpret_cast<const f32x4*>(p.wq_sc + min(n0 + wn0 + j * 16 + (lane >> 4) * 4, p.N - 4));
#pragma unroll
        for (int i = 0; i < TM; i++) acc[i][j] *= s;
    }
}

__device__ __forceinline__ void kdbg_stamp(const GemmParams& p, int slot) {
    if (__builtin_expect(p.kdbg != nullptr, 0) && threadIdx.x == 0) p.kdbg[(long)blockIdx.x * 8 + slot] = wall_clock64();
}

typedef _Float16 f16x2v __attribute__((ext_vector_type(2)));
template <int TM>
__device__ __forceinline__ void ln_accumulate(const f16x8 (&a)[TM], float (&ls)[TM], float (&lq)[TM]) {
    const f16x2v ones = {(f16)1.0f, (f16)1.0f};
#pragma unroll
    for (int i = 0; i < TM; i++)
#pragma unroll
        for (int e = 0; e < 4; e++) {
            const f16x2v pr = {a[i][2 * e], a[i][2 * e + 1]};
            ls[i] = __builtin_amdgcn_fdot2(pr, ones, ls[i], false);
            lq[i] = __builtin_amdgcn_fdot2(pr, pr, lq[i], false);
        }
}
template <int TM, int TN, bool PARTIAL>
__device__ __forceinline__ void ln_apply(const GemmParams& p, f32x4 (&acc)[TM][TN], float (&ls)[TM], float (&lq)[TM], int n0, int wn0, int lane) {
#pragma unroll
    for (int i = 0; i < TM; i++) {
        float s = ls[i], q = lq[i];
        if (PARTIAL) {
            s += __shfl_xor(s, 16, 64); q += __shfl_xor(q, 16, 64);
            s += __shfl_xor(s, 32, 64); q += __shfl_xor(q, 32, 64);
        }
        const double ik = (double)(1.0f / (float)p.K);
        const double mean_d = (double)s * ik;
        const float var = fmaxf((float)((double)q * ik - mean_d * mean_d), 0.f);
        const float mean = (float)mean_d;
        const float rstd = 1.0f / sqrtf(var + p.ln_eps);
#pragma unroll
        for (int j = 0; j < TN; j++) {
            const int n = n0 + wn0 + j * 16 + (lane >> 4) * 4;
            f32x4 c = {0.f, 0.f, 0.f, 0.f};
            if (n < p.N) c = *reinterpret_cast<const f32x4*>(p.ln_c1 + n);
#pragma unroll
            for (int r = 0; r < 4; r++) acc[i][j][r] = rstd * (acc[i][j][r] - mean * c[r]);
        }
    }
}

template <int TM, int TN, bool RB = true, bool ON = true>
struct EpiOps {
    bool have;
    f32x4 bias32[ON ? TN : 1];
    f16x4 bias16[ON ? TN : 1];
    f16x4 rb[ON && RB ? TM : 1][ON && RB ? TN : 1];
    f16x4 res[ON ? TM : 1][ON ? TN : 1];
};
template <int TM, int TN, bool RB, bool ON>
__device__ __forceinline__ void epi_prefetch(const GemmParams& p, EpiOps<TM, TN, RB, ON>& e, int m0, int n0, int wm0, int wn0, int lane, int zb) {
    const int N = p.N;
    e.have = ON && !p.no_epre && p.splits == 1 && (N & 3) == 0 && p.act != OSG_ACT_GEGLU && N >= 4 && (RB || !p.rowbias);
    if constexpr (!ON) return;
    if (__builtin_expect(!e.have, 0)) return;
    const f16* __restrict__ R = p.residual ? p.residual + zb * p.strideC : nullptr;
#pragma unroll
    for (int j = 0; j < TN; j++) {
        const int n = min(n0 + wn0 + j * 16 + (lane >> 4) * 4, N - 4);
        if (p.bias) {
            if (p.bias_f32) e.bias32[j] = *reinterpret_cast<const f32x4*>((const float*)p.bias + n);
            else e.bias16[j] = *reinterpret_cast<const f16x4*>((const f16*)p.bias + n);
        }
    }
#pragma unroll
    for (int i = 0; i < TM; i++) {
        const int m = min(m0 + wm0 + i * 16 + (lane & 15), p.M - 1);
#pragma unroll
        for (int j = 0; j < TN; j++) {
            const int n = min(n0 + wn0 + j * 16 + (lane >> 4) * 4, N - 4);
            if constexpr (RB) {
                if (p.rowbias) e.rb[i][j] = *reinterpret_cast<const f16x4*>(p.rowbias + (long)(m / p.rb_rows) * p.rb_ld + n);
            }
            if (R) e.res[i][j] = *reinterpret_cast<const f16x4*>(R + (long)m * N + n);
        }
    }
    asm volatile("" ::: "memory");
}

__device__ __forceinline__ void stat_add(int per_xcd, unsigned long long* table, long copy_stride, long cell, float S, float Q, float qscale) {
    const unsigned long long vs = (unsigned long long)__float2ll_rn(S * kStatSX), vq = (unsigned long long)__float2ll_rn(Q * qscale);
    if (per_xcd) {
        unsigned xcc;
        asm volatile("s_getreg_b32 %0, hwreg(HW_REG_XCC_ID)" : "=s"(xcc));
        unsigned long long* c = table + (long)(xcc & 7u) * copy_stride + cell;
        __hip_atomic_fetch_add(c, vs, __ATOMIC_RELAXED, __HIP_MEMORY_SCOPE_WORKGROUP);
        __hip_atomic_fetch_add(c + 1, vq, __ATOMIC_RELAXED, __HIP_MEMORY_SCOPE_WORKGROUP);
    } else {
        atomicAdd(table + cell, vs);
        atomicAdd(table + cell + 1, vq);
    }
}

template <int CTRL>
__device__ __forceinline__ float dpp_get(float v) {
    return __int_as_float(__builtin_amdgcn_update_dpp(0, __float_as_int(v), CTRL, 0xf, 0xf, false));
}
__device__ __forceinline__ float dpp_sum16(float v) {
    v += dpp_get<0xB1>(v);
    v += dpp_get<0x4E>(v);
    v += dpp_get<0x124>(v);
    v += dpp_get<0x128>(v);
    return v;
}
template <int TM, int TN>
__device__ __forceinline__ void gemm_colstats(const GemmParams& p, const f16x4 (&o)[TM][TN], int mrow0, int ncol0, int lane, float* st) {
    const int mb = mrow0 + (lane & 15);
#pragma unroll
    for (int j = 0; j < TN; j++)
#pragma unroll
        for (int r = 0; r < 4; r++) {
            float s = 0.f, q = 0.f;
#pragma unroll
            for (int i = 0; i < TM; i++)
                if (mb + i * 16 < p.M) {
                    const float f = (float)o[i][j][r];
                    s += f;
                    q = fmaf(f, f, q);
                }
            s = dpp_sum16(s);
            q = dpp_sum16(q);
            if ((lane & 15) == 0) {
                const int c = j * 16 + (lane >> 4) * 4 + r;
                st[c * 2] = s;
                st[c * 2 + 1] = q;
            }
        }
    asm volatile("s_waitcnt lgkmcnt(0)" ::: "memory");
    const int n_img = mrow0 / p.sink_hw;
    const int wn = min(TN * 16, p.N - ncol0);
#pragma unroll
    for (int k = 0; k < 2; k++) {
        const StatSink sk = p.sink[k];
        if (!sk.table || wn <= 0) continue;
        const int c_lo = ncol0 + sk.ch_off, c_hi = c_lo + wn;
        const int g = c_lo / sk.cpg + lane;
        if (g * sk.cpg < c_hi) {
            const int a = max(g * sk.cpg, c_lo) - c_lo, b = min((g + 1) * sk.cpg, c_hi) - c_lo;
            float S = 0.f, Q = 0.f;
            for (int c = a; c < b; c++) { S += st[c * 2]; Q += st[c * 2 + 1]; }
            stat_add(p.sink_per_xcd, reinterpret_cast<unsigned long long*>(sk.table), (long)p.sink_imgs * sk.groups * 2, ((long)n_img * sk.groups + g) * 2, S, Q,
                     stat_q_scale((long)p.sink_hw * sk.cpg));
        }
    }
}

constexpr unsigned kEpiOob = 0x80000000u;
constexpr int kEpiMaxBM = 128;
__host__ __device__ inline unsigned epi_extent(int rows_left, long pitch, int N) {
    const long bytes = ((long)(rows_left - 1) * pitch + N) * 2;
    return bytes < (long)kEpiOob ? (unsigned)bytes : kEpiOob;
}
inline int epi_check(osg_ctx* ctx, GemmParams& p) {
    const long ldc = p.ldc ? p.ldc : (long)p.N;
    const long pitch = std::max(std::max(ldc, p.C2 ? p.ldc2 : 0L), (long)p.N);
    if ((long)kEpiMaxBM * pitch * 2 >= (long)kEpiOob) {
        ctx->err = "contraction epilogue: an output row pitch of 8 Mi elements or more does not fit the 32-bit store offsets of a 128-row tile";
        return 1;
    }
    p.rb_bytes = 0;
    if (p.rowbias) {
        const long rb_rows = p.rb_rows > 0 ? p.rb_rows : 1;
        const long bytes = (((long)p.M - 1) / rb_rows * p.rb_ld + p.N) * 2;
        if (bytes >= (long)kEpiOob) {
            ctx->err = "contraction epilogue: the per-image bias must be smaller than 2 GiB";
            return 1;
        }
        p.rb_bytes = (unsigned)bytes;
    }
    return 0;
}

template <int TM, int TN, bool RB, bool ON, bool BATCH = true>
__device__ __forceinline__ void gemm_epilogue_fast(const GemmParams& p, f32x4 (&acc)[TM][TN], int m0, int n0, int wm0, int wn0, int lane, int zb,
                                                   const EpiOps<TM, TN, RB, ON>& pre, float* stat_lds = nullptr) {
    const int N = p.N;
    f16* __restrict__ C = p.C + zb * p.strideC;
    const f16* __restrict__ R = p.residual ? p.residual + zb * p.strideC : nullptr;
    const long ldc = p.ldc ? p.ldc : (long)N;
    const int nb = n0 + wn0 + (lane >> 4) * 4;
    const int mb = m0 + wm0 + (lane & 15);
    bool done = false;
    if constexpr (ON) {
        if (pre.have) {
            done = true;
            if (p.bias) {
                if (p.bias_f32) {
#pragma unroll
                    for (int i = 0; i < TM; i++)
#pragma unroll
                        for (int j = 0; j < TN; j++) acc[i][j] += pre.bias32[j];
                } else {
#pragma unroll
                    for (int i = 0; i < TM; i++)
#pragma unroll
                        for (int j = 0; j < TN; j++)
#pragma unroll
                            for (int r = 0; r < 4; r++) acc[i][j][r] += (float)pre.bias16[j][r];
                }
            }
            if constexpr (RB) {
                if (p.rowbias) {
#pragma unroll
                    for (int i = 0; i < TM; i++)
#pragma unroll
                        for (int j = 0; j < TN; j++)
#pragma unroll
                            for (int r = 0; r < 4; r++) acc[i][j][r] += (float)pre.rb[i][j][r];
                }
            }
            if (R) {
#pragma unroll
                for (int i = 0; i < TM; i++)
#pragma unroll
                    for (int j = 0; j < TN; j++)
#pragma unroll
                        for (int r = 0; r < 4; r++) acc[i][j][r] += (float)pre.res[i][j][r];
            }
        }
    }
    if constexpr (BATCH) if (!done) {
        const bool hb32 = p.bias && p.bias_f32, hb16 = p.bias && !p.bias_f32, hrb = p.rowbias != nullptr, hres = R != nullptr;
        typedef unsigned u32x2 __attribute__((ext_vector_type(2)));
        typedef unsigned u32x4 __attribute__((ext_vector_type(4)));
        const unsigned nbytes = (unsigned)N * 2u;
        __amdgpu_buffer_rsrc_t rsB32 = __builtin_amdgcn_make_buffer_rsrc((void*)p.bias, 0, hb32 ? nbytes * 2u : 0u, 0x00020000);
        __amdgpu_buffer_rsrc_t rsB16 = __builtin_amdgcn_make_buffer_rsrc((void*)p.bias, 0, hb16 ? nbytes : 0u, 0x00020000);
        __amdgpu_buffer_rsrc_t rsRB = __builtin_amdgcn_make_buffer_rsrc((void*)p.rowbias, 0, hrb ? p.rb_bytes : 0u, 0x00020000);
        __amdgpu_buffer_rsrc_t rsR = __builtin_amdgcn_make_buffer_rsrc((void*)(hres ? R + (long)m0 * N : nullptr), 0, hres ? epi_extent(p.M - m0, N, N) : 0u, 0x00020000);
        if (TM * TN <= 16 && OSG_LIKELY(!hrb && !hres)) {
            if (hb32) {
                f32x4 b32[TN];
#pragma unroll
                for (int j = 0; j < TN; j++) b32[j] = __builtin_bit_cast(f32x4, __builtin_amdgcn_raw_buffer_load_b128(rsB32, (unsigned)nb * 4u + j * 64, 0, 0));
#pragma unroll
                for (int i = 0; i < TM; i++)
#pragma unroll
                    for (int j = 0; j < TN; j++)
#pragma unroll
                        for (int r = 0; r < 4; r++) acc[i][j][r] += b32[j][r];
            } else if (hb16) {
                f16x4 b16[TN];
#pragma unroll
                for (int j = 0; j < TN; j++) b16[j] = __builtin_bit_cast(f16x4, __builtin_amdgcn_raw_buffer_load_b64(rsB16, (unsigned)nb * 2u + j * 32, 0, 0));
#pragma unroll
                for (int i = 0; i < TM; i++)
#pragma unroll
                    for (int j = 0; j < TN; j++)
#pragma unroll
                        for (int r = 0; r < 4; r++) acc[i][j][r] += (float)b16[j][r];
            }
        } else {
        f32x4 b32[TN];
        f16x4 b16[TN];
#pragma unroll
        for (int j = 0; j < TN; j++) {
            b32[j] = __builtin_bit_cast(f32x4, __builtin_amdgcn_raw_buffer_load_b128(rsB32, (unsigned)nb * 4u + j * 64, 0, 0));
            b16[j] = __builtin_bit_cast(f16x4, __builtin_amdgcn_raw_buffer_load_b64(rsB16, (unsigned)nb * 2u + j * 32, 0, 0));
        }
        constexpr int IB = TM * TN <= 16 ? TM : 1, JB = (TM * TN <= 16 || TN % 2) ? TN : TN / 2;
        static_assert(TN % JB == 0, "column blocks per chunk");
#pragma unroll
        for (int i0 = 0; i0 < TM; i0 += IB)
#pragma unroll
            for (int j0 = 0; j0 < TN; j0 += JB) {
                f16x4 rbv[IB][JB], rsv[IB][JB];
#pragma unroll
                for (int ii = 0; ii < IB; ii++) {
                    const int m = mb + (i0 + ii) * 16;
                    const unsigned ro = hrb ? (unsigned)(((long)(min(m, p.M - 1) / (p.rb_rows > 0 ? p.rb_rows : 1)) * p.rb_ld + nb) * 2) : 0u;
                    const unsigned rs = (unsigned)(wm0 + (lane & 15) + (i0 + ii) * 16) * nbytes + (unsigned)nb * 2u;
#pragma unroll
                    for (int jj = 0; jj < JB; jj++) {
                        rbv[ii][jj] = __builtin_bit_cast(f16x4, __builtin_amdgcn_raw_buffer_load_b64(rsRB, ro + (j0 + jj) * 32, 0, 0));
                        rsv[ii][jj] = __builtin_bit_cast(f16x4, __builtin_amdgcn_raw_buffer_load_b64(rsR, rs + (j0 + jj) * 32, 0, 0));
                    }
                }
#pragma unroll
                for (int ii = 0; ii < IB; ii++)
#pragma unroll
                    for (int jj = 0; jj < JB; jj++)
#pragma unroll
                        for (int r = 0; r < 4; r++) {
                            float x = acc[i0 + ii][j0 + jj][r];
                            x += p.bias ? (hb32 ? b32[j0 + jj][r] : (float)b16[j0 + jj][r]) : -0.0f;
                            x += hrb ? (float)rbv[ii][jj][r] : -0.0f;
                            x += hres ? (float)rsv[ii][jj][r] : -0.0f;
                            acc[i0 + ii][j0 + jj][r] = x;
                        }
            }
        }
    }
    if constexpr (!BATCH) if (!done) {
        if (p.bias) {
#pragma unroll
            for (int j = 0; j < TN; j++) {
                const int n = min(nb + j * 16, N - 4);
                f32x4 bv;
                if (p.bias_f32) bv = *reinterpret_cast<const f32x4*>((const float*)p.bias + n);
                else {
                    const f16x4 b16 = *reinterpret_cast<const f16x4*>((const f16*)p.bias + n);
#pragma unroll
                    for (int r = 0; r < 4; r++) bv[r] = (float)b16[r];
                }
#pragma unroll
                for (int i = 0; i < TM; i++) acc[i][j] += bv;
            }
        }
        if (p.rowbias) {
#pragma unroll
            for (int i = 0; i < TM; i++) {
                const long ro = (long)(min(mb + i * 16, p.M - 1) / p.rb_rows) * p.rb_ld;
#pragma unroll
                for (int j = 0; j < TN; j++) {
                    const f16x4 rb = *reinterpret_cast<const f16x4*>(p.rowbias + ro + min(nb + j * 16, N - 4));
#pragma unroll
                    for (int r = 0; r < 4; r++) acc[i][j][r] += (float)rb[r];
                }
            }
        }
        if (R) {
#pragma unroll
            for (int i = 0; i < TM; i++) {
                const long ro = (long)min(mb + i * 16, p.M - 1) * N;
#pragma unroll
                for (int j = 0; j < TN; j++) {
                    const f16x4 rv = *reinterpret_cast<const f16x4*>(R + ro + min(nb + j * 16, N - 4));
#pragma unroll
                    for (int r = 0; r < 4; r++) acc[i][j][r] += (float)rv[r];
                }
            }
        }
    }
    if (OSG_UNLIKELY_IF(BATCH, p.act != OSG_ACT_NONE)) {
        const int act = p.act;
#pragma unroll
        for (int i = 0; i < TM; i++)
#pragma unroll
            for (int j = 0; j < TN; j++)
#pragma unroll
                for (int r = 0; r < 4; r++) acc[i][j][r] = osg_apply_act(acc[i][j][r], act);
    }
    f16x4 o[TM][TN];
#pragma unroll
    for (int i = 0; i < TM; i++)
#pragma unroll
        for (int j = 0; j < TN; j++)
#pragma unroll
            for (int r = 0; r < 4; r++) o[i][j][r] = (f16)acc[i][j][r];
#if OSG_EPI_STORE_AUX >= 0
    {
        typedef unsigned u32x2 __attribute__((ext_vector_type(2)));
        const int mr = wm0 + (lane & 15), rows_left = p.M - m0;
        __amdgpu_buffer_rsrc_t rsC = __builtin_amdgcn_make_buffer_rsrc((void*)(C + (long)m0 * ldc), 0, epi_extent(rows_left, ldc, N), 0x00020000);
#pragma unroll
        for (int i = 0; i < TM; i++) {
            const int r = mr + i * 16;
#pragma unroll
            for (int j = 0; j < TN; j++) {
                const int n = nb + j * 16;
                const unsigned off = (r < rows_left && n < N) ? ((unsigned)r * (unsigned)ldc + (unsigned)n) * 2u : kEpiOob;
                __builtin_amdgcn_raw_buffer_store_b64(__builtin_bit_cast(u32x2, o[i][j]), rsC, off, 0, OSG_EPI_STORE_AUX);
            }
        }
        if (OSG_UNLIKELY_IF(BATCH, p.C2 != nullptr)) {
            __amdgpu_buffer_rsrc_t rsC2 = __builtin_amdgcn_make_buffer_rsrc((void*)(p.C2 + (long)m0 * p.ldc2), 0, epi_extent(rows_left, p.ldc2, N), 0x00020000);
#pragma unroll
            for (int i = 0; i < TM; i++) {
                const int r = mr + i * 16;
#pragma unroll
                for (int j = 0; j < TN; j++) {
                    const int n = nb + j * 16;
                    const unsigned off = (r < rows_left && n < N) ? ((unsigned)r * (unsigned)p.ldc2 + (unsigned)n) * 2u : kEpiOob;
                    __builtin_amdgcn_raw_buffer_store_b64(__builtin_bit_cast(u32x2, o[i][j]), rsC2, off, 0, OSG_EPI_STORE_AUX);
                }
            }
        }
    }
#else
#pragma unroll
    for (int i = 0; i < TM; i++) {
        const int m = mb + i * 16;
#pragma unroll
        for (int j = 0; j < TN; j++) {
            const int n = nb + j * 16;
            if (m < p.M && n < N) *reinterpret_cast<f16x4*>(C + (long)m * ldc + n) = o[i][j];
        }
    }
    if (p.C2) {
        f16* __restrict__ C2 = p.C2;
#pragma unroll
        for (int i = 0; i < TM; i++) {
            const int m = mb + i * 16;
#pragma unroll
            for (int j = 0; j < TN; j++) {
                const int n = nb + j * 16;
                if (m < p.M && n < N) *reinterpret_cast<f16x4*>(C2 + (long)m * p.ldc2 + n) = o[i][j];
            }
        }
    }
#endif
    if (OSG_UNLIKELY_IF(BATCH, stat_lds != nullptr)) gemm_colstats<TM, TN>(p, o, m0 + wm0, n0 + wn0, lane, stat_lds);
    if (OSG_UNLIKELY_IF(BATCH, p.rs_out != nullptr)) {
#pragma unroll
        for (int i = 0; i < TM; i++) {
            const int m = mb + i * 16;
            if (m >= p.M) continue;
#pragma unroll
            for (int h = 0; h < TN / 2; h++) {
                float s = 0.f, q = 0.f;
#pragma unroll
                for (int jj = 0; jj < 2; jj++) {
                    const int j = 2 * h + jj;
                    if (nb + j * 16 < N) {
#pragma unroll
                        for (int r = 0; r < 4; r++) {
                            const float f = (float)o[i][j][r];
                            s += f;
                            q = fmaf(f, f, q);
                        }
                    }
                }
                s += __shfl_xor(s, 16, 64); q += __shfl_xor(q, 16, 64);
                s += __shfl_xor(s, 32, 64); q += __shfl_xor(q, 32, 64);
                const int slot = ((n0 + wn0) >> 5) + h;
                if ((lane >> 4) == 0 && slot < p.rs_np) {
                    float* d = p.rs_out + ((long)m * p.rs_np + slot) * 2;
                    d[0] = s;
                    d[1] = q;
                }
            }
        }
    }
}

template <int TM, int TN, bool RB, bool ON, bool BATCH = true>
__device__ __forceinline__ void gemm_epilogue(const GemmParams& p, f32x4 (&acc)[TM][TN], int m0, int n0, int wm0, int wn0, int lane,
                                              int zb, int zslab, const EpiOps<TM, TN, RB, ON>& pre, float* stat_lds = nullptr) {
    const int N = p.N;
    if (OSG_LIKELY(p.splits == 1)) {
        if (OSG_LIKELY((N & 3) == 0 && ((p.ldc | p.ldc2) & 3) == 0)) {
            gemm_epilogue_fast<TM, TN, RB, ON, BATCH>(p, acc, m0, n0, wm0, wn0, lane, zb, pre, stat_lds);
            return;
        }
        f16* __restrict__ C = p.C + zb * p.strideC;
        const f16* __restrict__ R = p.residual ? p.residual + zb * p.strideC : nullptr;
        const long ldc = p.ldc ? p.ldc : (long)N;
        f16* __restrict__ C2 = p.C2;
#pragma unroll
        for (int i = 0; i < TM; i++) {
            const int m = m0 + wm0 + i * 16 + (lane & 15);
            if (m >= p.M) continue;
#pragma unroll
            for (int j = 0; j < TN; j++) {
                const int n = n0 + wn0 + j * 16 + (lane >> 4) * 4;
                if (n >= N) continue;
#pragma unroll
                for (int r = 0; r < 4; r++) {
                    if (n + r >= N) break;
                    float x = acc[i][j][r];
                    if (p.bias) x += p.bias_f32 ? ((const float*)p.bias)[n + r] : (float)((const f16*)p.bias)[n + r];
                    if (p.rowbias) x += (float)p.rowbias[(long)(m / p.rb_rows) * p.rb_ld + n + r];
                    if (R) x += (float)R[(long)m * N + n + r];
                    const f16 o1 = (f16)osg_apply_act(x, p.act);
                    C[(long)m * ldc + n + r] = o1;
                    if (C2) C2[(long)m * p.ldc2 + n + r] = o1;
                }
            }
        }
    } else {
        float* __restrict__ P = p.partial + ((long)zslab) * p.M * N;
#pragma unroll
        for (int i = 0; i < TM; i++) {
            const int m = m0 + wm0 + i * 16 + (lane & 15);
            if (m >= p.M) continue;
#pragma unroll
            for (int j = 0; j < TN; j++) {
                const int n = n0 + wn0 + j * 16 + (lane >> 4) * 4;
                if (n >= N) continue;
                if ((N & 3) == 0) {
                    *reinterpret_cast<f32x4*>(P + (long)m * N + n) = acc[i][j];
                } else {
#pragma unroll
                    for (int r = 0; r < 4; r++)
                        if (n + r < N) P[(long)m * N + n + r] = acc[i][j][r];
                }
            }
        }
    }
}


template <int TM, int TN>
__device__ __forceinline__ void gemm_epilogue(const GemmParams& p, f32x4 (&acc)[TM][TN], int m0, int n0, int wm0, int wn0, int lane, int zb, int zslab) {
    EpiOps<TM, TN, false, false> none;
    none.have = false;
    gemm_epilogue<TM, TN, false, false>(p, acc, m0, n0, wm0, wn0, lane, zb, zslab, none);
}

template <int TM, int TN>
__device__ __forceinline__ void gemm_epilogue_geglu(const GemmParams& p, f32x4 (&acc)[TM][TN], int m0, int n0, int wm0, int wn0, int lane,
                                                    int zb) {
    static_assert(TN % 2 == 0, "GEGLU epilogue needs value/gate tile pairs");
    const int No = p.N >> 1;
    f16* __restrict__ C = p.C + zb * p.strideC;
    const bool hb32 = p.bias && p.bias_f32, hb16 = p.bias && !p.bias_f32;
    f32x4 b32[TN];
    f16x4 b16[TN];
#pragma unroll
    for (int j = 0; j < TN; j++) {
        const int n = min(n0 + wn0 + j * 16 + (lane >> 4) * 4, p.N - 4);
        b32[j] = *reinterpret_cast<const f32x4*>(hb32 ? (const float*)p.bias + n : (const float*)p.A);
        b16[j] = *reinterpret_cast<const f16x4*>(hb16 ? (const f16*)p.bias + n : p.A);
    }
#pragma unroll
    for (int i = 0; i < TM; i++) {
        const int m = m0 + wm0 + i * 16 + (lane & 15);
        if (m >= p.M) continue;
#pragma unroll
        for (int j = 0; j < TN; j += 2) {
            const int n = n0 + wn0 + j * 16 + (lane >> 4) * 4;
            if (n >= p.N) continue;
            const int c = ((n0 + wn0 + j * 16) >> 1) + (lane >> 4) * 4;
            f16x4 o;
#pragma unroll
            for (int r = 0; r < 4; r++) {
                const float v = acc[i][j][r] + (p.bias ? (hb32 ? b32[j][r] : (float)b16[j][r]) : -0.0f);
                const float g = acc[i][j + 1][r] + (p.bias ? (hb32 ? b32[j + 1][r] : (float)b16[j + 1][r]) : -0.0f);
                o[r] = (f16)(v * osg_gelu_erf(g));
            }
            *reinterpret_cast<f16x4*>(C + (long)m * No + c) = o;
        }
    }
}

template <int TM, int TN>
__device__ __forceinline__ bool splitk_fold_acc(const GemmParams& p, f32x4 (&acc)[TM][TN], int tile_id, int zs, int* flag, int tid) {
    constexpr int NV = TM * TN;
    f32x4* __restrict__ slab = reinterpret_cast<f32x4*>(p.partial) + ((long)tile_id * p.splits) * (NV * 256) + tid;
    unsigned* w = reinterpret_cast<unsigned*>(p.tickets) + 2 * tile_id;
    __syncthreads();
    if (tid == 0) *flag = (int)__hip_atomic_fetch_add(w, 1u, __ATOMIC_RELAXED, __HIP_MEMORY_SCOPE_AGENT);
    __syncthreads();
    const bool is_last = *flag == p.splits - 1;
    if (!is_last) {
        f32x4* dst = slab + (long)zs * (NV * 256);
#pragma unroll
        for (int i = 0; i < TM; i++)
#pragma unroll
            for (int j = 0; j < TN; j++) {
                asm volatile("global_store_dwordx4 %0, %1, off sc1" ::"v"(dst + (i * TN + j) * 256), "v"(acc[i][j]) : "memory");
            }
        asm volatile("s_waitcnt vmcnt(0)" ::: "memory");
        __syncthreads();
        if (tid == 0) __hip_atomic_fetch_add(w + 1, 1u, __ATOMIC_RELAXED, __HIP_MEMORY_SCOPE_AGENT);
        return false;
    }
    if (tid == 0) {
        const unsigned want = (unsigned)p.splits - 1;
        const unsigned long long t0 = wall_clock64();
        bool complete = true;
        while (__hip_atomic_load(w + 1, __ATOMIC_RELAXED, __HIP_MEMORY_SCOPE_AGENT) != want) {
            if (wall_clock64() - t0 > 2000000ull) {
                if (p.xcd_err) __hip_atomic_store(p.xcd_err, 2, __ATOMIC_RELAXED, __HIP_MEMORY_SCOPE_SYSTEM);
                complete = false;
                break;
            }
            __builtin_amdgcn_s_sleep(1);
        }
        if (complete) {
            __hip_atomic_store(w, 0u, __ATOMIC_RELAXED, __HIP_MEMORY_SCOPE_AGENT);
            __hip_atomic_store(w + 1, 0u, __ATOMIC_RELAXED, __HIP_MEMORY_SCOPE_AGENT);
        }
    }
    __syncthreads();
    f32x4 sum[TM][TN];
    for (int s = 0; s < p.splits; s++) {
        if (s == zs) {
#pragma unroll
            for (int i = 0; i < TM; i++)
#pragma unroll
                for (int j = 0; j < TN; j++) sum[i][j] = s == 0 ? acc[i][j] : sum[i][j] + acc[i][j];
        } else {
            const f32x4* src = slab + (long)s * (NV * 256);
            f32x4 part[TM][TN];
#pragma unroll
            for (int i = 0; i < TM; i++)
#pragma unroll
                for (int j = 0; j < TN; j++) {
                    asm volatile("global_load_dwordx4 %0, %1, off sc1" : "=v"(part[i][j]) : "v"(src + (i * TN + j) * 256) : "memory");
                }
            asm volatile("s_waitcnt vmcnt(0)" ::: "memory");
#pragma unroll
            for (int i = 0; i < TM; i++)
#pragma unroll
                for (int j = 0; j < TN; j++) {
                    asm volatile("" : "+v"(part[i][j]));
                    sum[i][j] = s == 0 ? part[i][j] : sum[i][j] + part[i][j];
                }
        }
    }
#pragma unroll
    for (int i = 0; i < TM; i++)
#pragma unroll
        for (int j = 0; j < TN; j++) acc[i][j] = sum[i][j];
    return true;
}

int launch_splitk_reduce(osg_ctx* ctx, const GemmParams& p, int batch);
template <int UNIT> int launch_v2_unit(int entry, osg_ctx* ctx, GemmParams& p, int batch);
template <> int launch_v2_unit<0>(int entry, osg_ctx* ctx, GemmParams& p, int batch);
template <> int launch_v2_unit<1>(int entry, osg_ctx* ctx, GemmParams& p, int batch);
template <> int launch_v2_unit<2>(int entry, osg_ctx* ctx, GemmParams& p, int batch);
template <> int launch_v2_unit<3>(int entry, osg_ctx* ctx, GemmParams& p, int batch);
template <int UNIT> int launch3_unit(int entry, osg_ctx* ctx, GemmParams& p);
template <> int launch3_unit<0>(int entry, osg_ctx* ctx, GemmParams& p);
template <> int launch3_unit<1>(int entry, osg_ctx* ctx, GemmParams& p);
int launch_colstats(osg_ctx* ctx, const f16* C, long ldc, int M, int N, int rows_per_image, const StatSink* sinks);
long long* kdbg_buffer(osg_ctx* ctx, long workgroups);
inline int no_epi_prefetch() { static const int v = getenv("OSG_NO_EPI_PREFETCH") ? 1 : 0; return v; }
inline int splitk_fold_mode() {
    const char* e = getenv("OSG_SPLITK_FOLD");
    return e ? atoi(e) : 1;
}
inline size_t splitk_fold_route(osg_ctx* ctx, GemmParams& p, long n_tiles, int bm, int bn) {
    p.fold_acc = 0;
    const int mode = splitk_fold_mode();
    if (mode == 0 || p.splits < 2 || p.splits > 4 || !ctx->tickets || 2 * n_tiles + 16 > osg_ctx::kTickets / 2) return 0;
    if ((p.N & 3) != 0 || ((p.ldc | p.ldc2) & 3) != 0 || p.act == OSG_ACT_GEGLU || p.ln_c1 || p.rs_out) return 0;
    if (p.sink[0].table || p.sink[1].table) return 0;
    p.fold_acc = 1;
    p.tickets = ctx->tickets;
    p.xcd_err = ctx->xcd_err_dev;
    return (size_t)n_tiles * p.splits * bm * bn * sizeof(float);
}
inline SelectEnv select_env(const osg_ctx* ctx) {
    static const bool no_wide = getenv("OSG_TUNE_NO_WIDE") != nullptr, no_spec = getenv("OSG_TUNE_NO_SPEC") != nullptr, no_ks2 = getenv("OSG_TUNE_NO_KS2") != nullptr;
    return SelectEnv{ctx->num_cu, ctx->autotune, splitk_fold_mode(), no_wide, no_spec, no_ks2};
}
inline SelectShape select_shape(const GemmParams& p, int batch) {
    SelectShape s;
    s.M = p.M; s.N = p.N; s.K = p.K; s.batch = batch; s.lda = p.lda;
    s.H = p.H; s.W = p.W; s.Cin = p.Cin; s.Ho = p.Ho; s.Wo = p.Wo; s.KW = p.KW; s.sh = p.sh; s.sw = p.sw; s.pt = p.pt; s.pl = p.pl;
    s.w8 = p.w8 != 0;
    return s;
}
template <class C> struct Knob { const char* name; int C::*field; int (*value)(int); };
inline int knob_int(int v) { return v; }
inline int knob_flag(int v) { return v != 0; }
inline constexpr Knob<V2Choice> kGemmKnobs[] = {
    {"OSG_GEMM_CFG", &V2Choice::cfg, knob_int}, {"OSG_GEMM_SPLITS", &V2Choice::splits, knob_int}, {"OSG_GEMM_NST", &V2Choice::nst, knob_int},
    {"OSG_GEMM_KS", &V2Choice::ks, [](int v) { return v == 2 ? 2 : 1; }},
    {"OSG_GEMM_SPEC", &V2Choice::spec, knob_flag},
    {"OSG_GEMM_FOLD", &V2Choice::fold, knob_flag},
};
inline constexpr Knob<Halo3Choice> kHalo3Knobs[] = {
    {"OSG_CONV3X3_BN", &Halo3Choice::bn, knob_int}, {"OSG_CONV3X3_SPLITS", &Halo3Choice::splits, knob_int},
    {"OSG_CONV3X3_NL", &Halo3Choice::loaders, [](int v) { return v == 8 ? 8 : 4; }}, {"OSG_CONV3X3_FOLD", &Halo3Choice::fold, knob_flag},
};
template <class C, size_t N> bool apply_knobs(const Knob<C> (&knobs)[N], C* ch) {
    bool any = false;
    for (const Knob<C>& k : knobs)
        if (const char* e = getenv(k.name)) {
            any = true;
            if (ch) ch->*k.field = k.value(atoi(e));
        }
    return any;
}
}

int osg_conv3x3_run(osg_ctx* ctx, osg_mm::GemmParams& p);
int osg_conv3x3_prepare(osg_ctx* ctx, osg_mm::GemmParams& p);
int osg_conv3x3_launch(osg_ctx* ctx, osg_mm::GemmParams p, osg_mm::Halo3Choice ch);
```

### onnxstream_amd/osgpu.py

```python
from __future__ import annotations

import ctypes
import os
from typing import Optional, Sequence

import numpy as np

_HERE = os.path.dirname(os.path.abspath(__file__))
LIB_PATH = os.environ.get("OSGPU_LIB") or os.path.join(_HERE, "libosgpu.so")

U8, F16, F32, I64 = 1, 2, 3, 4
_NP2DT = {np.dtype(np.uint8): U8, np.dtype(np.float16): F16, np.dtype(np.float32): F32, np.dtype(np.int64): I64}
ACT_NONE, ACT_SILU, ACT_SIGMOID = 0, 1, 2
UN = dict(sigmoid=0, erf=1, sqrt=2, sin=3, cos=4, neg=5, pow=6, silu=7, gelu_erf=8)
BIN = dict(add=0, sub=1, mul=2, div=3)

EXPORTS = [
    "osg_device_count", "osg_init", "osg_destroy", "osg_last_error", "osg_device_name", "osg_stream", "osg_set_autotune", "osg_tune_misses",
    "osg_malloc", "osg_free", "osg_upload", "osg_upload_sync", "osg_host_register", "osg_host_unregister", "osg_upload_pinned", "osg_upload_pinned_async", "osg_copy_fence", "osg_download", "osg_copy", "osg_memset", "osg_sync",
    "osg_graph_begin", "osg_graph_end", "osg_graph_launch", "osg_graph_destroy", "osg_timer_start", "osg_timer_stop",
    "osg_conv2d_nhwc", "osg_conv2d_nhwc_rb", "osg_conv2d_nhwc_v", "osg_gemm", "osg_gemm_ln", "osg_gemm_rowstats", "osg_last_route", "osg_last_kernel", "osg_gemm_kernarg_check", "osg_attention_kernarg_check", "osg_gemm_w8", "osg_conv2d_nhwc_w8", "osg_gemm_w8_v", "osg_conv2d_nhwc_w8_v", "osg_transpose_kn_to_nk", "osg_attention", "osg_attention_strided", "osg_sdpa", "osg_rms_norm", "osg_rope",
    "osg_instance_norm", "osg_group_norm_nhwc", "osg_layer_norm", "osg_reduce_mean_last", "osg_softmax_last",
    "osg_unary", "osg_binary", "osg_geglu", "osg_transpose", "osg_copy_2d", "osg_concat2", "osg_resize_nearest", "osg_gather_rows",
    "osg_maxpool_nhwc", "osg_convert", "osg_sampler_prepare", "osg_sampler_cfg_euler_a", "osg_sampler_cfg_multistep", "osg_sampler_prepare_rescale",
    "osg_sampler_prepare_single", "osg_sampler_euler_a_single", "osg_sampler_multistep_single",
    "osg_decode_gather", "osg_decode_blend",
    "osg_range_push", "osg_range_pop", "osg_marker_record", "osg_copy_wait_marker", "osg_timer_mark", "osg_timer_between", "osg_set_stat_sinks", "osg_group_norm_stats_nhwc", "osg_qu8_conv2d_nhwc", "osg_qu8_conv2d_nhwc_t", "osg_qu8_conv_tap_sums", "osg_qu8_gemm", "osg_qu8_lut", "osg_qu8_binary", "osg_qu8_instance_norm", "osg_qu8_instance_norm_nhwc", "osg_qu8_affine_act", "osg_qu8_norm_affine_act_nhwc", "osg_qu8_softmax_last", "osg_kdbg_read",
    "osg_tblock_tail_supported", "osg_tblock_tail", "osg_tblock_kv_pack_elems", "osg_tblock_kv_pack_jobs", "osg_tblock_pack_weight", 
]


class OsgError(RuntimeError):
    pass


class TBlockTailArgs(ctypes.Structure):
    _vp, _cf, _ci, _cl = ctypes.c_void_p, ctypes.c_float, ctypes.c_int, ctypes.c_long
    _fields_ = [("a1", _vp), ("x0", _vp), ("wo1", _vp), ("bo1", _vp), ("g2", _vp), ("be2", _vp), ("eps2", _cf), ("wq2", _vp), ("bq2", _vp),
                ("kp", _vp), ("vtp", _vp), ("scale", _cf), ("Tk", _ci), ("wo2", _vp), ("bo2", _vp), ("g3", _vp), ("be3", _vp), ("eps3", _cf),
                ("w1", _vp), ("b1", _vp), ("w2", _vp), ("b2", _vp), ("wpo", _vp), ("bpo", _vp), ("xin", _vp), ("out", _vp), ("out2", _vp),
                ("ldo", _cl), ("ldo2", _cl), ("M", _ci), ("rows_per_img", _ci), ("C", _ci), ("heads", _ci), ("dbg", _vp * 8), ("rows_per_block", _ci)]


def load_library(path: str = LIB_PATH) -> ctypes.CDLL:
    if not os.path.exists(path):
        raise OsgError(f"{path} not found: build it with `python -m onnxstream_amd.build` (hipcc, gfx950)")
    lib = ctypes.CDLL(path)
    vp, ci, cl, cf = ctypes.c_void_p, ctypes.c_int, ctypes.c_long, ctypes.c_float
    lib.osg_init.argtypes = [ci, ctypes.POINTER(vp)]
    lib.osg_destroy.argtypes = [vp]
    lib.osg_destroy.restype = None
    lib.osg_last_error.argtypes = [vp]
    lib.osg_last_error.restype = ctypes.c_char_p
    lib.osg_device_name.argtypes = [vp]
    lib.osg_device_name.restype = ctypes.c_char_p
    lib.osg_stream.argtypes = [vp]
    lib.osg_stream.restype = vp
    lib.osg_malloc.argtypes = [vp, ctypes.c_size_t, ctypes.POINTER(vp)]
    lib.osg_free.argtypes = [vp, vp]
    lib.osg_host_register.argtypes = [vp, vp, ctypes.c_size_t]
    lib.osg_host_unregister.argtypes = [vp, vp]
    for f in ("osg_upload", "osg_upload_sync", "osg_upload_pinned", "osg_upload_pinned_async", "osg_download", "osg_copy"):
        getattr(lib, f).argtypes = [vp, vp, vp, ctypes.c_size_t]
    lib.osg_memset.argtypes = [vp, vp, ci, ctypes.c_size_t]
    lib.osg_sync.argtypes = [vp]
    lib.osg_copy_fence.argtypes = [vp]
    lib.osg_graph_begin.argtypes = [vp]
    lib.osg_graph_end.argtypes = [vp, ctypes.POINTER(vp)]
    lib.osg_graph_launch.argtypes = [vp, vp]
    lib.osg_graph_destroy.argtypes = [vp]
    lib.osg_graph_destroy.restype = None
    lib.osg_timer_start.argtypes = [vp]
    lib.osg_timer_stop.argtypes = [vp, ctypes.POINTER(cf)]
    lib.osg_conv2d_nhwc.argtypes = [vp, ci, vp, vp, vp, ci, vp, vp] + [ci] * 14
    lib.osg_conv2d_nhwc_rb.argtypes = [vp, ci, vp, vp, vp, ci, vp, cl, vp, vp] + [ci] * 14
    lib.osg_conv2d_nhwc_v.argtypes = [vp, ci, vp, vp, vp, ci, vp, cl, vp, vp, cl, vp, cl] + [ci] * 14
    lib.osg_gemm_w8.argtypes = [vp, vp, vp, cf, ci, vp, ci, vp, vp, ci, ci, ci, ci]
    lib.osg_conv2d_nhwc_w8.argtypes = [vp, vp, vp, cf, ci, vp, ci, vp, cl, vp, vp] + [ci] * 14
    lib.osg_gemm_w8_v.argtypes = [vp, vp, vp, cf, ci, vp, vp, vp, ci, vp, vp, ci, ci, ci, ci]
    lib.osg_conv2d_nhwc_w8_v.argtypes = [vp, vp, vp, cf, ci, vp, vp, vp, ci, vp, cl, vp, vp, cl, vp, cl] + [ci] * 14
    lib.osg_gemm.argtypes = [vp, ci, vp, vp, ci, vp, ci, vp, vp, ci, ci, ci, ci, cl, cl, cl, ci]
    lib.osg_transpose_kn_to_nk.argtypes = [vp, ci, vp, vp, ci, ci]
    lib.osg_attention.argtypes = [vp, ci, vp, vp, vp, vp, ci, ci, ci, ci, cf, ci]
    lib.osg_attention_strided.argtypes = [vp, ci, vp, cl, cl, cl, vp, cl, cl, cl, vp, cl, cl, cl, vp, cl, cl, cl, ci, ci, ci, ci,
                                          ci, cf]
    lib.osg_sdpa.argtypes = [vp, ci, vp, vp, vp, vp, vp, ci, ci, ci, ci, ci, ci, cf]
    lib.osg_rms_norm.argtypes = [vp, ci, vp, vp, vp, cl, ci, cf]
    lib.osg_rope.argtypes = [vp, ci, vp, vp, vp, vp, cl, cl, ci]
    lib.osg_instance_norm.argtypes = [vp, ci, vp, vp, vp, vp, ci, cl, ci, cf]
    lib.osg_group_norm_nhwc.argtypes = [vp, ci, vp, vp, vp, vp, ci, cl, ci, ci, cf, ci]
    lib.osg_layer_norm.argtypes = [vp, ci, vp, vp, vp, vp, cl, ci, cf]
    lib.osg_reduce_mean_last.argtypes = [vp, ci, vp, vp, cl, cl]
    lib.osg_softmax_last.argtypes = [vp, ci, vp, vp, cl, cl]
    lib.osg_unary.argtypes = [vp, ci, ci, vp, vp, cl, cf]
    lib.osg_binary.argtypes = [vp, ci, ci, vp, ctypes.POINTER(cl), vp, ctypes.POINTER(cl), vp, ci]
    lib.osg_geglu.argtypes = [vp, ci, vp, vp, cl, cl]
    lib.osg_transpose.argtypes = [vp, ci, vp, vp, ci, ctypes.POINTER(cl), ctypes.POINTER(ci)]
    lib.osg_copy_2d.argtypes = [vp, ci, vp, cl, cl, vp, cl, cl, cl, cl]
    lib.osg_resize_nearest.argtypes = [vp, ci, vp, vp] + [ci] * 7
    lib.osg_gather_rows.argtypes = [vp, ci, vp, vp, vp, cl, cl, cl]
    lib.osg_maxpool_nhwc.argtypes = [vp, ci, vp, vp] + [ci] * 12
    lib.osg_convert.argtypes = [vp, ci, ci, vp, vp, cl, cf, ci]
    lib.osg_concat2.argtypes = [vp, ci, vp, cl, vp, cl, vp, cl]
    lib.osg_gemm_ln.argtypes = [vp, vp, vp, vp, vp, cf, vp, vp, vp, ci, ci, ci, ci]
    lib.osg_gemm_rowstats.argtypes = [vp, vp, vp, vp, ci, vp, vp, ci, ci, ci, ci, vp]
    lib.osg_last_route.argtypes = [vp, ctypes.POINTER(ci)]
    lib.osg_last_kernel.argtypes = [vp, ctypes.POINTER(ci)]
    if hasattr(lib, "osg_gemm_kernarg_check"):
        lib.osg_gemm_kernarg_check.argtypes = [vp, cl, ci]
        lib.osg_attention_kernarg_check.argtypes = [vp, cl, ci, ci]
    lib.osg_sampler_prepare.argtypes = [vp, vp, vp, vp, ci, cl, cf, cf, cl]
    lib.osg_sampler_cfg_euler_a.argtypes = [vp, vp, vp, vp, ci, cl, cf, cf, cf, cf, cf, cf]
    lib.osg_sampler_cfg_multistep.argtypes = [vp, ci, vp, vp, vp, vp, vp, vp, ci, cl, cf, cf, cf, cf, cf, cf, cf, cf, ctypes.c_double, ctypes.c_double]
    lib.osg_sampler_prepare_rescale.argtypes = [vp, vp, vp, vp, ci, cl, cf, cf, cf, cl]
    lib.osg_sampler_prepare_single.argtypes = [vp, vp, vp, vp, ci, cl, cf, cf, cf, cl]
    lib.osg_sampler_euler_a_single.argtypes = [vp, vp, vp, vp, ci, cl, cf, cf, cf, cf, cf]
    lib.osg_sampler_multistep_single.argtypes = [vp, ci, vp, vp, vp, vp, vp, vp, ci, cl, cf, cf, cf, cf, cf, cf, cf, ctypes.c_double, ctypes.c_double]
    lib.osg_decode_gather.argtypes = [vp, vp, vp, ci, ci, ci, ci, cf]
    lib.osg_decode_blend.argtypes = [vp, vp, vp, vp, ci, ci, ci, ci, ci]
    lib.osg_set_stat_sinks.argtypes = [vp, vp, ci, ci, ci, vp, ci, ci, ci, ci]
    lib.osg_group_norm_stats_nhwc.argtypes = [vp, vp, vp, vp, vp, ci, ctypes.c_long, ci, ci, cf, ci, vp]
    lib.osg_qu8_conv2d_nhwc.argtypes = [vp, vp, cf, ci, vp, cf, ci, vp, cf, ci, vp] + [ci] * 13
    lib.osg_qu8_conv2d_nhwc_t.argtypes = [vp, vp, cf, ci, vp, cf, ci, vp, cf, ci, vp] + [ci] * 13 + [vp]
    lib.osg_qu8_conv_tap_sums.argtypes = [vp, vp, ci, ci, ci, ci, vp]
    lib.osg_qu8_gemm.argtypes = [vp, vp, cl, cf, ci, vp, cf, ci, vp, cf, ci, vp, ci, ci, ci, ci, cl, cl, cl]
    lib.osg_qu8_lut.argtypes = [vp, vp, vp, cl, vp]
    lib.osg_qu8_binary.argtypes = [vp, ci, vp, ctypes.POINTER(cl), cf, ci, vp, ctypes.POINTER(cl), cf, ci, vp, cf, ci, ci]
    lib.osg_qu8_instance_norm.argtypes = [vp, vp, vp, ci, cl, ci, vp, vp, cf, cf, ci, cf, ci]
    lib.osg_qu8_affine_act.argtypes = [vp, vp, cf, ci, vp, cf, ci, cf, ci, vp, cf, ci, cf, ci, vp, cf, ci, cf, ci, vp, cl, ci, cl]
    lib.osg_qu8_instance_norm_nhwc.argtypes = [vp, vp, vp, cl, ci, ci, ci, vp, vp, cf, cf, ci, cf, ci]
    lib.osg_qu8_norm_affine_act_nhwc.argtypes = [vp, vp, cl, ci, ci, ci, vp, vp, cf, cf, ci, cf, ci, vp, cf, ci, cf, ci, vp, cf, ci, cf, ci, vp, cf, ci, cf, ci, vp]
    lib.osg_qu8_softmax_last.argtypes = [vp, vp, vp, cl, cl, vp]
    lib.osg_tblock_tail_supported.argtypes = [ci] * 5
    lib.osg_tblock_tail.argtypes = [vp, ctypes.POINTER(TBlockTailArgs)]
    lib.osg_tblock_kv_pack_elems.argtypes = [ci, ci, ci]
    lib.osg_tblock_kv_pack_elems.restype = ctypes.c_size_t
    lib.osg_tblock_kv_pack_jobs.argtypes = [vp, vp, cl, ci, ci, ci, ci, vp, vp]
    lib.osg_tblock_pack_weight.argtypes = [vp, vp, ci, ci, vp]
    return lib


class DevBuf:

    def __init__(self, gpu: "Gpu", shape, dtype):
        self.gpu = gpu
        self.shape = tuple(int(s) for s in shape)
        self.dtype = np.dtype(dtype)
        self.nbytes = int(np.prod(self.shape, dtype=np.int64)) * self.dtype.itemsize
        p = ctypes.c_void_p()
        gpu._ck(gpu.lib.osg_malloc(gpu.ctx, max(self.nbytes, 16), ctypes.byref(p)))
        self.ptr = p.value

    @property
    def size(self):
        return int(np.prod(self.shape, dtype=np.int64))

    def numpy(self) -> np.ndarray:
        out = np.empty(self.shape, self.dtype)
        if self.nbytes:
            self.gpu._ck(self.gpu.lib.osg_download(self.gpu.ctx, out.ctypes.data, self.ptr, self.nbytes))
        return out

    def read_rows(self, lo: int, hi: int) -> np.ndarray:
        row = self.shape[-1]
        assert 0 <= lo <= hi <= self.size // row, (lo, hi, self.shape)
        out = np.empty((hi - lo, row), self.dtype)
        if out.nbytes:
            self.gpu._ck(self.gpu.lib.osg_download(self.gpu.ctx, out.ctypes.data, self.ptr + lo * row * self.dtype.itemsize, out.nbytes))
        return out

    def view(self, offset: int, shape) -> "DevBuf":
        v = DevBuf.__new__(DevBuf)
        v.gpu, v.shape, v.dtype = self.gpu, tuple(int(s) for s in shape), self.dtype
        v.nbytes = int(np.prod(v.shape, dtype=np.int64)) * self.dtype.itemsize
        assert 0 <= offset and offset * self.dtype.itemsize + v.nbytes <= self.nbytes, (offset, shape, self.shape)
        v.ptr, v.base = self.ptr + offset * self.dtype.itemsize, self
        return v

    def free(self):
        if self.ptr and getattr(self, "base", None) is None:
            self.gpu.lib.osg_free(self.gpu.ctx, self.ptr)
        self.ptr = None

    def __del__(self):
        try:
            self.free()
        except Exception:
            pass


class Gpu:
    def __init__(self, device: int = 0, lib_path: str = LIB_PATH):
        self.lib = load_library(lib_path)
        if self.lib.osg_device_count() <= 0:
            raise OsgError("no HIP device visible: the osgpu backend has no CPU fallback")
        c = ctypes.c_void_p()
        rc = self.lib.osg_init(device, ctypes.byref(c))
        if rc:
            raise OsgError(f"osg_init failed with code {rc}")
        self.ctx = c

    def close(self):
        if self.ctx:
            self.lib.osg_destroy(self.ctx)
            self.ctx = None

    def _ck(self, rc):
        if rc:
            raise OsgError(self.lib.osg_last_error(self.ctx).decode())

    @property
    def name(self):
        return self.lib.osg_device_name(self.ctx).decode()

    def empty(self, shape, dtype=np.float16) -> DevBuf:
        b = DevBuf(self, shape, dtype)
        if b.nbytes:
            self.memset(b, 0xFF)
        return b

    def last_route(self):
        r = (ctypes.c_int * 5)()
        self._ck(self.lib.osg_last_route(self.ctx, r))
        return tuple(r)

    def last_kernel(self):
        r = (ctypes.c_int * 8)()
        self._ck(self.lib.osg_last_kernel(self.ctx, r))
        return tuple(r)

    def to_dev(self, arr: np.ndarray, staged: bool = False) -> DevBuf:
        arr = np.ascontiguousarray(arr)
        b = DevBuf(self, arr.shape, arr.dtype)
        if arr.nbytes:
            fn = self.lib.osg_upload if staged else self.lib.osg_upload_sync
            self._ck(fn(self.ctx, b.ptr, arr.ctypes.data, arr.nbytes))
        return b

    def sync(self):
        self._ck(self.lib.osg_sync(self.ctx))

    def memset(self, b: DevBuf, byte: int):
        self._ck(self.lib.osg_memset(self.ctx, b.ptr, byte, b.nbytes))

    def _out(self, out: Optional[DevBuf], shape, dtype) -> DevBuf:
        if out is None:
            return self.empty(shape, dtype)
        if out.size != int(np.prod(shape, dtype=np.int64)) or out.dtype != np.dtype(dtype):
            raise OsgError(f"out= holds {out.shape} {out.dtype}, the op writes {tuple(shape)} {np.dtype(dtype)}")
        return out

    def timer_start(self):
        self._ck(self.lib.osg_timer_start(self.ctx))

    def timer_stop(self) -> float:
        ms = ctypes.c_float()
        self._ck(self.lib.osg_timer_stop(self.ctx, ctypes.byref(ms)))
        return ms.value

    @staticmethod
    def _p(b: Optional[DevBuf]):
        return b.ptr if b is not None else None

    def conv2d_nhwc(self, x: DevBuf, w: DevBuf, bias: Optional[DevBuf], stride=1, pads=(1, 1, 1, 1), residual=None, act=ACT_NONE,
                    image_bias: Optional[DevBuf] = None):
        n, h, wd, cin = x.shape
        cout, kh, kw, cin2 = w.shape
        assert cin == cin2
        sh, sw = (stride, stride) if isinstance(stride, int) else stride
        pt, pl, pb, pr = pads
        ho, wo = (h + pt + pb - kh) // sh + 1, (wd + pl + pr - kw) // sw + 1
        y = self.empty((n, ho, wo, cout), x.dtype)
        bdt = _NP2DT[bias.dtype] if bias is not None else F16
        if image_bias is not None:
            self._ck(self.lib.osg_conv2d_nhwc_rb(self.ctx, _NP2DT[x.dtype], x.ptr, w.ptr, self._p(bias), bdt, image_bias.ptr, cout,
                                                 self._p(residual), y.ptr, n, h, wd, cin, cout, kh, kw, sh, sw, pt, pl, pb, pr, act))
            return y
        self._ck(self.lib.osg_conv2d_nhwc(self.ctx, _NP2DT[x.dtype], x.ptr, w.ptr, self._p(bias), bdt, self._p(residual), y.ptr, n, h,
                                          wd, cin, cout, kh, kw, sh, sw, pt, pl, pb, pr, act))
        return y

    def conv2d_nhwc_view(self, x: DevBuf, w: DevBuf, bias: Optional[DevBuf], wide: DevBuf, col: int, dense: Optional[DevBuf] = None, stride=1,
                         pads=(1, 1, 1, 1), residual=None, act=ACT_NONE, image_bias: Optional[DevBuf] = None, swap=False):
        n, h, wd, cin = x.shape
        cout, kh, kw, _ = w.shape
        sh, sw = (stride, stride) if isinstance(stride, int) else stride
        pt, pl, pb, pr = pads
        bdt = _NP2DT[bias.dtype] if bias is not None else F16
        es = x.dtype.itemsize
        v_ptr, v_ld = wide.ptr + col * es, wide.shape[-1]
        if dense is None:
            y, y_ld, y2, y2_ld = v_ptr, v_ld, None, 0
        elif swap:
            y, y_ld, y2, y2_ld = dense.ptr, 0, v_ptr, v_ld
        else:
            y, y_ld, y2, y2_ld = v_ptr, v_ld, dense.ptr, cout
        self._ck(self.lib.osg_conv2d_nhwc_v(self.ctx, _NP2DT[x.dtype], x.ptr, w.ptr, self._p(bias), bdt, self._p(image_bias), cout if image_bias is not None else 0,
                                            self._p(residual), y, y_ld, y2, y2_ld, n, h, wd, cin, cout, kh, kw, sh, sw, pt, pl, pb, pr, act))

    def gemm(self, a: DevBuf, b: DevBuf, bias=None, residual=None, b_is_nk=False, act=ACT_NONE):
        batch = a.shape[0] if len(a.shape) == 3 else 1
        m, k = a.shape[-2:]
        n = b.shape[-2] if b_is_nk else b.shape[-1]
        sb = 0 if len(b.shape) == 2 else k * n
        c = self.empty(a.shape[:-1] + (n,), a.dtype)
        bdt = _NP2DT[bias.dtype] if bias is not None else F16
        self._ck(self.lib.osg_gemm(self.ctx, _NP2DT[a.dtype], a.ptr, b.ptr, int(b_is_nk), self._p(bias), bdt, self._p(residual), c.ptr, m,
                                   n, k, batch, m * k if batch > 1 else 0, sb, m * n if batch > 1 else 0, act))
        return c

    def gemm_rowstats(self, a: DevBuf, b_nk: DevBuf, bias=None, residual=None, act=ACT_NONE):
        m, k = a.shape
        n = b_nk.shape[0]
        c = self.empty((m, n), a.dtype)
        rs = self.empty((m, n // 32, 2), np.dtype(np.float32))
        bdt = _NP2DT[bias.dtype] if bias is not None else F16
        self._ck(self.lib.osg_gemm_rowstats(self.ctx, a.ptr, b_nk.ptr, self._p(bias), bdt, self._p(residual), c.ptr, m, n, k, act, rs.ptr))
        return c, rs

    def gemm_ln(self, x: DevBuf, w_nk: np.ndarray, gamma: np.ndarray, beta: np.ndarray, bias=None, eps: float = 1e-5, residual=None, act=ACT_NONE,
                rowstats=None):
        m, k = x.shape
        n = w_nk.shape[0]
        wf = (gamma.astype(np.float32)[None, :] * w_nk.astype(np.float32)).astype(np.float16)
        c1 = wf.astype(np.float64).sum(axis=1).astype(np.float32)
        c2 = (w_nk.astype(np.float64) @ beta.astype(np.float64) + (bias.astype(np.float64) if bias is not None else 0.0)).astype(np.float32)
        dw, d1, d2 = self.to_dev(wf), self.to_dev(c1), self.to_dev(c2)
        y = self.empty((m, n // 2 if act == 3 else n), x.dtype)
        self._ck(self.lib.osg_gemm_ln(self.ctx, x.ptr, dw.ptr, d1.ptr, d2.ptr, eps, self._p(rowstats), self._p(residual), y.ptr, m, n, k, act))
        return y

    def transpose_kn_to_nk(self, w: DevBuf):
        k, n = w.shape
        o = self.empty((n, k), w.dtype)
        self._ck(self.lib.osg_transpose_kn_to_nk(self.ctx, _NP2DT[w.dtype], w.ptr, o.ptr, k, n))
        return o

    def attention(self, q: DevBuf, k: DevBuf, v: DevBuf, scale: float, k_is_dt: bool, out: Optional[DevBuf] = None):
        heads, tq, d = q.shape
        tkv = v.shape[1]
        o = self._out(out, q.shape, q.dtype)
        self._ck(self.lib.osg_attention(self.ctx, _NP2DT[q.dtype], q.ptr, k.ptr, v.ptr, o.ptr, heads, tq, tkv, d, scale, int(k_is_dt)))
        return o

    def attention_tokens(self, q: DevBuf, k: DevBuf, v: DevBuf, heads: int, scale: float, out: Optional[DevBuf] = None):
        bsz, tq, c = q.shape
        tkv = k.shape[1]
        d = c // heads
        o = self._out(out, q.shape, q.dtype)
        self._ck(self.lib.osg_attention_strided(self.ctx, F16, q.ptr, c, d, tq * c, k.ptr, c, d, tkv * c, v.ptr, c, d, tkv * c, o.ptr, c, d,
                                                tq * c, bsz, heads, tq, tkv, d, scale))
        return o

    def attention_strided(self, q, k, v, o, batch: int, heads: int, tq: int, tkv: int, d: int, scale: float):
        self._ck(self.lib.osg_attention_strided(self.ctx, F16, *q, *k, *v, *o, batch, heads, tq, tkv, d, scale))

    def tblock_kv_pack(self, k: DevBuf, v: DevBuf, heads: int):
        imgs, tk, c = k.shape
        d = c // heads
        dp = (d + 15) // 16 * 16
        n = self.lib.osg_tblock_kv_pack_elems(imgs, heads, d)
        assert n == imgs * heads * 80 * dp
        kv = self.to_dev(np.concatenate([k.numpy().reshape(imgs * tk, c), v.numpy().reshape(imgs * tk, c)], axis=1))
        jobs = self.to_dev(np.array([0, c, d, 0], np.int32))
        dst = self.empty((2 * n,), k.dtype)
        self._ck(self.lib.osg_tblock_kv_pack_jobs(self.ctx, kv.ptr, 2 * c, imgs, tk, heads, 1, jobs.ptr, dst.ptr))
        kp, vtp = self.empty((imgs, heads, 80, dp), k.dtype), self.empty((imgs, heads, dp, 80), k.dtype)
        self._ck(self.lib.osg_copy(self.ctx, kp.ptr, dst.ptr, n * 2))
        self._ck(self.lib.osg_copy(self.ctx, vtp.ptr, dst.ptr + n * 2, n * 2))
        return kp, vtp

    def tblock_kv_pack_jobs(self, base: DevBuf, ld: int, imgs: int, tk: int, heads: int, jobs, out: Optional[DevBuf] = None):
        offs, total = [], 0
        for _, _, d in jobs:
            offs.append(total)
            total += 2 * self.lib.osg_tblock_kv_pack_elems(imgs, heads, d)
        table = self.to_dev(np.array([[kc, vc, d, o] for (kc, vc, d), o in zip(jobs, offs)], np.int32))
        dst = self._out(out, (total,), base.dtype)
# ... 312 lines not shown
```

Before: 10.03.

## Add epilogue-specialized lean GEMM kernel variants selected per launch form

Adds a compile-time EPI mask template parameter to the v2 GEMM kernel so that bias, residual, rowbias, activation, split and bounds checks become constants. A table of (tile config, epilogue mask) pairs is instantiated, and at launch a matching lean variant is picked when shapes tile evenly and alignment holds. Otherwise the generic kernel runs. The aim is to cut runtime branching, clamping and bounds checks in the epilogue and prefetch. The cost is more kernel instantiations, larger code size, and possible register-allocation changes.

```diff
diff --git a/include/osgpu.h b/include/osgpu.h
--- a/include/osgpu.h
+++ b/include/osgpu.h
@@ -114,6 +114,7 @@
 int osg_gemm_rowstats(osg_ctx* ctx, const void* A, const void* B_nk, const void* bias, osg_dtype bias_dtype, const void* residual, void* C,
                       int M, int N, int K, osg_act act, float* rowstats);
 int osg_last_route(const osg_ctx* ctx, int out[5]);
+int osg_last_epilogue(const osg_ctx* ctx, int out[2]);
 int osg_last_kernel(const osg_ctx* ctx, int out[8]);
 
 int osg_gemm_kernarg_check(osg_ctx* ctx, long lda, int splits);
diff --git a/onnxstream_amd/csrc/osg_common.h b/onnxstream_amd/csrc/osg_common.h
--- a/onnxstream_amd/csrc/osg_common.h
+++ b/onnxstream_amd/csrc/osg_common.h
@@ -21,6 +21,7 @@
     int pending_hw = 0;
     bool tuning = false, sink_fused = false;
     int last_route[5] = {-1, -1, 0, 0, 0};
+    int last_epi[2] = {-1, -1};
     int last_kernel[8] = {-1, 0, 0, 0, 0, 0, 0, 0};
     hipEvent_t ev_t0 = nullptr, ev_t1 = nullptr;
     static constexpr int kStages = 2;
@@ -60,6 +61,7 @@
 inline void osg_set_route(osg_ctx* ctx, int family, int instantiation, int splits, int fold) {
     int* r = ctx->last_route;
     r[0] = family; r[1] = instantiation; r[2] = splits; r[3] = fold; r[4] = 0;
+    ctx->last_epi[0] = ctx->last_epi[1] = -1;
 }
 
 inline void osg_set_kernel(osg_ctx* ctx, int family, int a = 0, int b = 0, int c = 0, int d = 0, int e = 0, int f = 0, int g = 0) {
diff --git a/onnxstream_amd/csrc/osg_ctx.hip b/onnxstream_amd/csrc/osg_ctx.hip
--- a/onnxstream_amd/csrc/osg_ctx.hip
+++ b/onnxstream_amd/csrc/osg_ctx.hip
@@ -226,6 +226,12 @@
     return 0;
 }
 
+int osg_last_epilogue(const osg_ctx* c, int out[2]) {
+    if (!c || !out) return 1;
+    out[0] = c->last_epi[0]; out[1] = c->last_epi[1];
+    return 0;
+}
+
 int osg_last_kernel(const osg_ctx* c, int out[8]) {
     if (!c || !out) return 1;
     for (int i = 0; i < 8; i++) out[i] = c->last_kernel[i];
diff --git a/onnxstream_amd/csrc/osg_gemm.hip b/onnxstream_amd/csrc/osg_gemm.hip
--- a/onnxstream_amd/csrc/osg_gemm.hip
+++ b/onnxstream_amd/csrc/osg_gemm.hip
@@ -417,8 +417,14 @@
     const double a_unique = CONV ? (double)p.a_bytes : (double)p.M * p.K * 2.0;
     p.n_major = (double)p.N * p.K * (p.w8 ? 1.0 : 2.0) > a_unique;
     static constexpr int (*units[4])(int, osg_ctx*, GemmParams&, int) = {launch_v2_unit<0>, launch_v2_unit<1>, launch_v2_unit<2>, launch_v2_unit<3>};
-    if (const int rc = units[v2_unit(e)](r.entry, ctx, p, batch)) return rc;
+    const EpiLaunch el = epi_launch_of(p, batch);
+    const int lean = select_epi(r.entry, el, epi_generic_forced());
+    if (OSG_UNLIKELY(getenv("OSG_EPI_LOG") != nullptr))
+        fprintf(stderr, "[epi] entry=%d form=%d whole=%d lean=%d capturing=%d tuning=%d M=%d N=%d K=%d splits=%d\n", r.entry, epi_form(el), (int)epi_whole(el, e.bm, e.bn), lean,
+                (int)ctx->capturing, (int)ctx->tuning, p.M, p.N, p.K, p.splits);
+    if (const int rc = lean >= 0 ? launch_v2_lean(lean, ctx, p, batch) : units[v2_unit(e)](r.entry, ctx, p, batch)) return rc;
     osg_set_route(ctx, 0, r.entry, p.splits, p.fold_acc);
+    ctx->last_epi[0] = lean; ctx->last_epi[1] = lean >= 0 ? kLeanEntries[lean].mask : EPI_ANY;
     if (p.splits > 1 && !p.fold_acc) return launch_splitk_reduce(ctx, p, batch);
     return 0;
 }
diff --git a/onnxstream_amd/csrc/osg_gemm2.h b/onnxstream_amd/csrc/osg_gemm2.h
--- a/onnxstream_amd/csrc/osg_gemm2.h
+++ b/onnxstream_amd/csrc/osg_gemm2.h
@@ -11,7 +11,7 @@
 namespace {
 using namespace osg_mm;
 
-template <int BM, int BN, int NST, bool CONV, int MODE = 0, int SPEC = 0, int LN = 0, int NCH = 5, int KS = 1, int WGN = 2, int WQ = 0>
+template <int BM, int BN, int NST, bool CONV, int MODE = 0, int SPEC = 0, int LN = 0, int NCH = 5, int KS = 1, int WGN = 2, int WQ = 0, int EPI = EPI_ANY>
 __global__ __launch_bounds__((SPEC || KS == 2) ? 512 : 256) void gemm2_kernel(const void* A, const void* Bt, int M, int N, int K, int k_per_split, unsigned a_bytes, unsigned b_bytes,
                                                                               int grid, int lda, unsigned sp_nm, GemmParams pk) {
     GemmParams p = pk;
@@ -83,7 +83,7 @@
 
     const f16* Ab = p.A;
     const f16* Bb = p.Bt;
-    if (OSG_UNLIKELY(sp_nm & kPackBatch)) {
+    if (OSG_UNLIKELY(EPI_NEVER((sp_nm & kPackBatch) != 0))) {
         Ab += (long)zb * kernarg_rare(pk.strideA);
         Bb += (long)zb * kernarg_rare(pk.strideB);
     }
@@ -98,16 +98,16 @@
     for (int j = 0; j < A_LD; j++) {
         const int m = m0 + (j * 4 + wave) * 8 + rsub;
         if (CONV) {
-            const int mm = m < p.M ? m : 0;
+            const int mm = EPI_ALWAYS(m < p.M) ? m : 0;
             const int hw = p.Ho * p.Wo;
             const int n_img = mm / hw;
             const int r2 = mm - n_img * hw;
             const int ho = r2 / p.Wo, wo = r2 - ho * p.Wo;
-            a_hi0[j] = m < p.M ? ho * p.sh - p.pt : -0x40000000;
+            a_hi0[j] = EPI_ALWAYS(m < p.M) ? ho * p.sh - p.pt : -0x40000000;
             a_wi0[j] = wo * p.sw - p.pl;
             a_base[j] = (((n_img * p.H + (ho * p.sh - p.pt)) * p.W + (wo * p.sw - p.pl)) * p.Cin + gch * 8) * 2;
         } else {
-            a_base[j] = m < p.M ? (int)(((long)m * p.lda + gch * 8) * 2) : (int)OOB;
+            a_base[j] = EPI_ALWAYS(m < p.M) ? (int)(((long)m * p.lda + gch * 8) * 2) : (int)OOB;
             a_hi0[j] = a_wi0[j] = 0;
         }
     }
@@ -116,10 +116,10 @@
     for (int j = 0; j < B_LD; j++) {
         if constexpr (WQ) {
             const int nl = (j * 4 + wave) * 16 + (lane >> 2), n = n0 + nl;
-            b_base[j] = (n < p.N && (BNP == BN || nl < BN)) ? (int)((long)n * p.K + (((lane & 3) ^ ((lane >> 4) & 3)) << 4)) : (int)OOB;
+            b_base[j] = (EPI_ALWAYS(n < p.N) && (BNP == BN || nl < BN)) ? (int)((long)n * p.K + (((lane & 3) ^ ((lane >> 4) & 3)) << 4)) : (int)OOB;
         } else {
             const int nl = (j * 4 + wave) * 8 + rsub, n = n0 + nl;
-            b_base[j] = (n < p.N && (BNP == BN || nl < BN)) ? (int)(((long)n * p.K + gch * 8) * 2) : (int)OOB;
+            b_base[j] = (EPI_ALWAYS(n < p.N) && (BNP == BN || nl < BN)) ? (int)(((long)n * p.K + gch * 8) * 2) : (int)OOB;
         }
     }
 
@@ -182,7 +182,7 @@
         asm volatile("" ::: "memory");
     }
 
-    constexpr bool EPRE = TM * TN <= 8;
+    constexpr bool EPRE = EPI == EPI_ANY ? TM * TN <= 8 : epi_lean_prefetch(EPI, TM * TN <= 8, CONV, LN);
     W8Ops<WQ ? TN : 1, true> w8;
     if constexpr (WQ) { if (math) w8_prefetch<TN, true>(p, w8, n0, wn0, lane); }
     if (loads) {
@@ -195,7 +195,7 @@
 #endif
     EpiOps<TM, TN, CONV, EPRE> epre;
     epre.have = false;
-    if (math && !p.ln_c1 && grp == 0) epi_prefetch<TM, TN, CONV, EPRE>(p, epre, m0, n0, wm0, wn0, lane, zb);
+    if (math && EPI_ALWAYS(!p.ln_c1) && grp == 0) epi_prefetch<TM, TN, CONV, EPRE, EPI>(p, epre, m0, n0, wm0, wn0, lane, zb);
     kdbg_stamp(p, 1);
     if constexpr (WQ) { if (math) w8_finalize<TN, true>(w8); }
 
@@ -266,18 +266,24 @@
         }
     }
     if constexpr (LN != 0) ln_apply<TM, TN, LN == 1>(p, acc, ls, lq, n0, wn0, lane);
-    if (OSG_UNLIKELY_IF(!SPEC, p.act == OSG_ACT_GEGLU)) {
-        if constexpr (TN % 2 == 0) gemm_epilogue_geglu<TM, TN>(p, acc, m0, n0, wm0, wn0, lane, zb);
+    if constexpr (EPI != EPI_ANY && (LN != 0 || WQ != 0)) {
+#pragma unroll
+        for (int i = 0; i < TM; i++)
+#pragma unroll
+            for (int j = 0; j < TN; j++) asm volatile("" : "+v"(acc[i][j]));
+    }
+    if (OSG_UNLIKELY_IF(!SPEC, (EPI_ON(EPI_GEGLU, p.act == OSG_ACT_GEGLU)))) {
+        if constexpr (TN % 2 == 0) gemm_epilogue_geglu<TM, TN, EPI>(p, acc, m0, n0, wm0, wn0, lane, zb);
         return;
     }
     kdbg_stamp(p, 4);
     float* stat_lds = nullptr;
-    if (OSG_UNLIKELY_IF(!SPEC, p.sink[0].table || p.sink[1].table)) {
+    if (OSG_UNLIKELY_IF(!SPEC, (EPI_ON(EPI_SINKS, p.sink[0].table || p.sink[1].table)))) {
         __builtin_amdgcn_s_barrier();
         stat_lds = reinterpret_cast<float*>(smem2) + wave * (WN * 2);
     }
     if constexpr (KS == 1 && !SPEC && LN == 0 && MODE == 0) {
-        if (OSG_UNLIKELY_IF(!SPEC, p.splits > 1 && p.fold_acc)) {
+        if (OSG_UNLIKELY_IF(!SPEC, (EPI_ON(EPI_FOLD, p.splits > 1 && p.fold_acc)))) {
             if (!splitk_fold_acc<TM, TN>(p, acc, (zb * p.mt + m_tile) * p.nt + n_tile, zs, reinterpret_cast<int*>(smem2), tid)) return;
             EpiOps<TM, TN, CONV, false> none;
             none.have = false;
@@ -285,17 +291,17 @@
             return;
         }
     }
-    gemm_epilogue<TM, TN, CONV, EPRE, !SPEC>(p, acc, m0, n0, wm0, wn0, lane, zb, zb * p.splits + zs, epre, stat_lds);
+    gemm_epilogue<TM, TN, CONV, EPRE, !SPEC, EPI>(p, acc, m0, n0, wm0, wn0, lane, zb, zb * p.splits + zs, epre, stat_lds);
     kdbg_stamp(p, 5);
     if (OSG_UNLIKELY_IF(!SPEC, p.kdbg != nullptr)) { asm volatile("s_waitcnt vmcnt(0)" ::: "memory"); kdbg_stamp(p, 6); }
 }
 
-template <int BM, int BN, int NST, bool CONV, int MODE = 0, int SPEC = 0, int LN = 0, int NCH = 5, int KS = 1, int WGN = 2, int WQ = 0>
+template <int BM, int BN, int NST, bool CONV, int MODE = 0, int SPEC = 0, int LN = 0, int NCH = 5, int KS = 1, int WGN = 2, int WQ = 0, int EPI = EPI_ANY>
 int launch_v2(osg_ctx* ctx, GemmParams& p, int batch) {
     constexpr size_t smem = WQ ? (size_t)NST * KS * (BM * 128 + (BN + 63) / 64 * 64 * 64) : (size_t)NST * KS * (BM + (BN + 31) / 32 * 32) * 128;
     static_assert(smem <= 160 * 1024, "LDS budget");
     static_assert(KS == 1 || (size_t)4 * ((BM / 32) * (BN / 32) + 1) * 1024 <= smem, "KS = 2: the accumulator hand-over must fit the ring");
-    auto kern = gemm2_kernel<BM, BN, NST, CONV, MODE, SPEC, LN, NCH, KS, WGN, WQ>;
+    auto kern = gemm2_kernel<BM, BN, NST, CONV, MODE, SPEC, LN, NCH, KS, WGN, WQ, EPI>;
     static unsigned long long attr_mask = 0;
     if (osg_first_on_device(attr_mask)) {
         OSG_HIP(ctx, hipFuncSetAttribute((const void*)kern, hipFuncAttributeMaxDynamicSharedMemorySize, (int)smem));
diff --git a/onnxstream_amd/csrc/osg_gemm_common.h b/onnxstream_amd/csrc/osg_gemm_common.h
--- a/onnxstream_amd/csrc/osg_gemm_common.h
+++ b/onnxstream_amd/csrc/osg_gemm_common.h
@@ -3,6 +3,7 @@
 #include <vector>
 #include "osg_common.h"
 #include "osg_gemm_select.h"
+#include "osg_gemm_epi.h"
 
 #include <algorithm>
 #include <type_traits>
@@ -93,6 +94,13 @@
 #define OSG_LIKELY(x) __builtin_expect(!!(x), 1)
 #define OSG_UNLIKELY(x) __builtin_expect(!!(x), 0)
 #define OSG_UNLIKELY_IF(h, x) ((h) ? __builtin_expect(!!(x), 0) : !!(x))
+#define EPI_ON(bits, x) (EPI == EPI_ANY ? (x) : ((EPI & (bits)) != 0))
+#define EPI_OFF(bits, x) (EPI == EPI_ANY ? (x) : ((EPI & (bits)) == 0))
+#define EPI_ALWAYS(x) (EPI == EPI_ANY ? (x) : true)
+#define EPI_NEVER(x) (EPI == EPI_ANY ? (x) : false)
+#define EPI_CLAMP(v, hi) (EPI == EPI_ANY ? min(v, hi) : (v))
+#define EPI_ACT(a) (EPI == EPI_ANY ? (int)(a) : (int)OSG_ACT_SILU)
+constexpr bool epi_lean_prefetch(int epi, bool on, bool conv, int ln) { return on && ln == 0 && !(epi & (EPI_SPLIT | EPI_FOLD | EPI_GEGLU)) && (conv || !(epi & EPI_ROWBIAS)); }
 
 typedef unsigned int u32x2v __attribute__((ext_vector_type(2)));
 typedef _Float16 f16x2w __attribute__((ext_vector_type(2)));
@@ -204,31 +212,31 @@
     f16x4 rb[ON && RB ? TM : 1][ON && RB ? TN : 1];
     f16x4 res[ON ? TM : 1][ON ? TN : 1];
 };
-template <int TM, int TN, bool RB, bool ON>
+template <int TM, int TN, bool RB, bool ON, int EPI = EPI_ANY>
 __device__ __forceinline__ void epi_prefetch(const GemmParams& p, EpiOps<TM, TN, RB, ON>& e, int m0, int n0, int wm0, int wn0, int lane, int zb) {
     const int N = p.N;
-    e.have = ON && !p.no_epre && p.splits == 1 && (N & 3) == 0 && p.act != OSG_ACT_GEGLU && N >= 4 && (RB || !p.rowbias);
+    e.have = ON && EPI_ALWAYS(!p.no_epre && p.splits == 1 && (N & 3) == 0 && p.act != OSG_ACT_GEGLU && N >= 4 && (RB || !p.rowbias));
     if constexpr (!ON) return;
     if (__builtin_expect(!e.have, 0)) return;
-    const f16* __restrict__ R = p.residual ? p.residual + zb * p.strideC : nullptr;
+    const f16* __restrict__ R = EPI_ON(EPI_RESIDUAL, p.residual != nullptr) ? p.residual + zb * p.strideC : nullptr;
 #pragma unroll
     for (int j = 0; j < TN; j++) {
-        const int n = min(n0 + wn0 + j * 16 + (lane >> 4) * 4, N - 4);
-        if (p.bias) {
-            if (p.bias_f32) e.bias32[j] = *reinterpret_cast<const f32x4*>((const float*)p.bias + n);
+        const int n = EPI_CLAMP(n0 + wn0 + j * 16 + (lane >> 4) * 4, N - 4);
+        if (EPI_ON(EPI_BIAS16 | EPI_BIAS32, p.bias != nullptr)) {
+            if (EPI_ON(EPI_BIAS32, p.bias_f32 != 0)) e.bias32[j] = *reinterpret_cast<const f32x4*>((const float*)p.bias + n);
             else e.bias16[j] = *reinterpret_cast<const f16x4*>((const f16*)p.bias + n);
         }
     }
 #pragma unroll
     for (int i = 0; i < TM; i++) {
-        const int m = min(m0 + wm0 + i * 16 + (lane & 15), p.M - 1);
+        const int m = EPI_CLAMP(m0 + wm0 + i * 16 + (lane & 15), p.M - 1);
 #pragma unroll
         for (int j = 0; j < TN; j++) {
-            const int n = min(n0 + wn0 + j * 16 + (lane >> 4) * 4, N - 4);
+            const int n = EPI_CLAMP(n0 + wn0 + j * 16 + (lane >> 4) * 4, N - 4);
             if constexpr (RB) {
-                if (p.rowbias) e.rb[i][j] = *reinterpret_cast<const f16x4*>(p.rowbias + (long)(m / p.rb_rows) * p.rb_ld + n);
-            }
-            if (R) e.res[i][j] = *reinterpret_cast<const f16x4*>(R + (long)m * N + n);
+                if (EPI_ON(EPI_ROWBIAS, p.rowbias != nullptr)) e.rb[i][j] = *reinterpret_cast<const f16x4*>(p.rowbias + (long)(m / p.rb_rows) * p.rb_ld + n);
+            }
+            if (EPI_ON(EPI_RESIDUAL, R != nullptr)) e.res[i][j] = *reinterpret_cast<const f16x4*>(R + (long)m * N + n);
         }
     }
     asm volatile("" ::: "memory");
@@ -327,21 +335,21 @@
     return 0;
 }
 
-template <int TM, int TN, bool RB, bool ON, bool BATCH = true>
+template <int TM, int TN, bool RB, bool ON, bool BATCH = true, int EPI = EPI_ANY>
 __device__ __forceinline__ void gemm_epilogue_fast(const GemmParams& p, f32x4 (&acc)[TM][TN], int m0, int n0, int wm0, int wn0, int lane, int zb,
                                                    const EpiOps<TM, TN, RB, ON>& pre, float* stat_lds = nullptr) {
     const int N = p.N;
     f16* __restrict__ C = p.C + zb * p.strideC;
-    const f16* __restrict__ R = p.residual ? p.residual + zb * p.strideC : nullptr;
+    const f16* __restrict__ R = EPI_ON(EPI_RESIDUAL, p.residual != nullptr) ? p.residual + zb * p.strideC : nullptr;
     const long ldc = p.ldc ? p.ldc : (long)N;
     const int nb = n0 + wn0 + (lane >> 4) * 4;
     const int mb = m0 + wm0 + (lane & 15);
     bool done = false;
     if constexpr (ON) {
-        if (pre.have) {
+        if (EPI_ALWAYS(pre.have)) {
             done = true;
-            if (p.bias) {
-                if (p.bias_f32) {
+            if (EPI_ON(EPI_BIAS16 | EPI_BIAS32, p.bias != nullptr)) {
+                if (EPI_ON(EPI_BIAS32, p.bias_f32 != 0)) {
 #pragma unroll
                     for (int i = 0; i < TM; i++)
 #pragma unroll
@@ -356,7 +364,7 @@
                 }
             }
             if constexpr (RB) {
-                if (p.rowbias) {
+                if (EPI_ON(EPI_ROWBIAS, p.rowbias != nullptr)) {
 #pragma unroll
                     for (int i = 0; i < TM; i++)
 #pragma unroll
@@ -365,7 +373,7 @@
                             for (int r = 0; r < 4; r++) acc[i][j][r] += (float)pre.rb[i][j][r];
                 }
             }
-            if (R) {
+            if (EPI_ON(EPI_RESIDUAL, R != nullptr)) {
 #pragma unroll
                 for (int i = 0; i < TM; i++)
 #pragma unroll
@@ -376,7 +384,8 @@
         }
     }
     if constexpr (BATCH) if (!done) {
-        const bool hb32 = p.bias && p.bias_f32, hb16 = p.bias && !p.bias_f32, hrb = p.rowbias != nullptr, hres = R != nullptr;
+        const bool hb32 = EPI_ON(EPI_BIAS32, p.bias && p.bias_f32), hb16 = EPI_ON(EPI_BIAS16, p.bias && !p.bias_f32), hrb = EPI_ON(EPI_ROWBIAS, p.rowbias != nullptr),
+                   hres = EPI_ON(EPI_RESIDUAL, R != nullptr);
         typedef unsigned u32x2 __attribute__((ext_vector_type(2)));
         typedef unsigned u32x4 __attribute__((ext_vector_type(4)));
         const unsigned nbytes = (unsigned)N * 2u;
@@ -439,7 +448,7 @@
 #pragma unroll
                         for (int r = 0; r < 4; r++) {
                             float x = acc[i0 + ii][j0 + jj][r];
-                            x += p.bias ? (hb32 ? b32[j0 + jj][r] : (float)b16[j0 + jj][r]) : -0.0f;
+                            x += EPI_ON(EPI_BIAS16 | EPI_BIAS32, p.bias != nullptr) ? (hb32 ? b32[j0 + jj][r] : (float)b16[j0 + jj][r]) : -0.0f;
                             x += hrb ? (float)rbv[ii][jj][r] : -0.0f;
                             x += hres ? (float)rsv[ii][jj][r] : -0.0f;
                             acc[i0 + ii][j0 + jj][r] = x;
@@ -448,12 +457,12 @@
         }
     }
     if constexpr (!BATCH) if (!done) {
-        if (p.bias) {
+        if (EPI_ON(EPI_BIAS16 | EPI_BIAS32, p.bias != nullptr)) {
 #pragma unroll
             for (int j = 0; j < TN; j++) {
                 const int n = min(nb + j * 16, N - 4);
                 f32x4 bv;
-                if (p.bias_f32) bv = *reinterpret_cast<const f32x4*>((const float*)p.bias + n);
+                if (EPI_ON(EPI_BIAS32, p.bias_f32 != 0)) bv = *reinterpret_cast<const f32x4*>((const float*)p.bias + n);
                 else {
                     const f16x4 b16 = *reinterpret_cast<const f16x4*>((const f16*)p.bias + n);
 #pragma unroll
@@ -463,7 +472,7 @@
                 for (int i = 0; i < TM; i++) acc[i][j] += bv;
             }
         }
-        if (p.rowbias) {
+        if (EPI_ON(EPI_ROWBIAS, p.rowbias != nullptr)) {
 #pragma unroll
             for (int i = 0; i < TM; i++) {
                 const long ro = (long)(min(mb + i * 16, p.M - 1) / p.rb_rows) * p.rb_ld;
@@ -475,7 +484,7 @@
                 }
             }
         }
-        if (R) {
+        if (EPI_ON(EPI_RESIDUAL, R != nullptr)) {
 #pragma unroll
             for (int i = 0; i < TM; i++) {
                 const long ro = (long)min(mb + i * 16, p.M - 1) * N;
@@ -488,8 +497,8 @@
             }
         }
     }
-    if (OSG_UNLIKELY_IF(BATCH, p.act != OSG_ACT_NONE)) {
-        const int act = p.act;
+    if (OSG_UNLIKELY_IF(BATCH, (EPI_ON(EPI_SILU, p.act != OSG_ACT_NONE)))) {
+        const int act = EPI_ACT(p.act);
 #pragma unroll
         for (int i = 0; i < TM; i++)
 #pragma unroll
@@ -515,11 +524,11 @@
 #pragma unroll
             for (int j = 0; j < TN; j++) {
                 const int n = nb + j * 16;
-                const unsigned off = (r < rows_left && n < N) ? ((unsigned)r * (unsigned)ldc + (unsigned)n) * 2u : kEpiOob;
+                const unsigned off = EPI_ALWAYS(r < rows_left && n < N) ? ((unsigned)r * (unsigned)ldc + (unsigned)n) * 2u : kEpiOob;
                 __builtin_amdgcn_raw_buffer_store_b64(__builtin_bit_cast(u32x2, o[i][j]), rsC, off, 0, OSG_EPI_STORE_AUX);
             }
         }
-        if (OSG_UNLIKELY_IF(BATCH, p.C2 != nullptr)) {
+        if (OSG_UNLIKELY_IF(BATCH, (EPI_ON(EPI_C2, p.C2 != nullptr)))) {
             __amdgpu_buffer_rsrc_t rsC2 = __builtin_amdgcn_make_buffer_rsrc((void*)(p.C2 + (long)m0 * p.ldc2), 0, epi_extent(rows_left, p.ldc2, N), 0x00020000);
 #pragma unroll
             for (int i = 0; i < TM; i++) {
@@ -527,7 +536,7 @@
 #pragma unroll
                 for (int j = 0; j < TN; j++) {
                     const int n = nb + j * 16;
-                    const unsigned off = (r < rows_left && n < N) ? ((unsigned)r * (unsigned)p.ldc2 + (unsigned)n) * 2u : kEpiOob;
+                    const unsigned off = EPI_ALWAYS(r < rows_left && n < N) ? ((unsigned)r * (unsigned)p.ldc2 + (unsigned)n) * 2u : kEpiOob;
                     __builtin_amdgcn_raw_buffer_store_b64(__builtin_bit_cast(u32x2, o[i][j]), rsC2, off, 0, OSG_EPI_STORE_AUX);
                 }
             }
@@ -556,19 +565,19 @@
         }
     }
 #endif
-    if (OSG_UNLIKELY_IF(BATCH, stat_lds != nullptr)) gemm_colstats<TM, TN>(p, o, m0 + wm0, n0 + wn0, lane, stat_lds);
-    if (OSG_UNLIKELY_IF(BATCH, p.rs_out != nullptr)) {
+    if (OSG_UNLIKELY_IF(BATCH, (EPI_ON(EPI_SINKS, stat_lds != nullptr)))) gemm_colstats<TM, TN>(p, o, m0 + wm0, n0 + wn0, lane, stat_lds);
+    if (OSG_UNLIKELY_IF(BATCH, (EPI_ON(EPI_ROWSTATS, p.rs_out != nullptr)))) {
 #pragma unroll
         for (int i = 0; i < TM; i++) {
             const int m = mb + i * 16;
-            if (m >= p.M) continue;
+            if (!EPI_ALWAYS(m < p.M)) continue;
 #pragma unroll
             for (int h = 0; h < TN / 2; h++) {
                 float s = 0.f, q = 0.f;
 #pragma unroll
                 for (int jj = 0; jj < 2; jj++) {
                     const int j = 2 * h + jj;
-                    if (nb + j * 16 < N) {
+                    if (EPI_ALWAYS(nb + j * 16 < N)) {
 #pragma unroll
                         for (int r = 0; r < 4; r++) {
                             const float f = (float)o[i][j][r];
@@ -580,7 +589,7 @@
                 s += __shfl_xor(s, 16, 64); q += __shfl_xor(q, 16, 64);
                 s += __shfl_xor(s, 32, 64); q += __shfl_xor(q, 32, 64);
                 const int slot = ((n0 + wn0) >> 5) + h;
-                if ((lane >> 4) == 0 && slot < p.rs_np) {
+                if ((lane >> 4) == 0 && EPI_ALWAYS(slot < p.rs_np)) {
                     float* d = p.rs_out + ((long)m * p.rs_np + slot) * 2;
                     d[0] = s;
                     d[1] = q;
@@ -590,13 +599,13 @@
     }
 }
 
-template <int TM, int TN, bool RB, bool ON, bool BATCH = true>
+template <int TM, int TN, bool RB, bool ON, bool BATCH = true, int EPI = EPI_ANY>
 __device__ __forceinline__ void gemm_epilogue(const GemmParams& p, f32x4 (&acc)[TM][TN], int m0, int n0, int wm0, int wn0, int lane,
                                               int zb, int zslab, const EpiOps<TM, TN, RB, ON>& pre, float* stat_lds = nullptr) {
     const int N = p.N;
-    if (OSG_LIKELY(p.splits == 1)) {
-        if (OSG_LIKELY((N & 3) == 0 && ((p.ldc | p.ldc2) & 3) == 0)) {
-            gemm_epilogue_fast<TM, TN, RB, ON, BATCH>(p, acc, m0, n0, wm0, wn0, lane, zb, pre, stat_lds);
+    if (OSG_LIKELY(EPI_OFF(EPI_SPLIT, p.splits == 1))) {
+        if (OSG_LIKELY(EPI_ALWAYS((N & 3) == 0 && ((p.ldc | p.ldc2) & 3) == 0))) {
+            gemm_epilogue_fast<TM, TN, RB, ON, BATCH, EPI>(p, acc, m0, n0, wm0, wn0, lane, zb, pre, stat_lds);
             return;
         }
         f16* __restrict__ C = p.C + zb * p.strideC;
@@ -629,12 +638,12 @@
 #pragma unroll
         for (int i = 0; i < TM; i++) {
             const int m = m0 + wm0 + i * 16 + (lane & 15);
-            if (m >= p.M) continue;
+            if (!EPI_ALWAYS(m < p.M)) continue;
 #pragma unroll
             for (int j = 0; j < TN; j++) {
                 const int n = n0 + wn0 + j * 16 + (lane >> 4) * 4;
-                if (n >= N) continue;
-                if ((N & 3) == 0) {
+                if (!EPI_ALWAYS(n < N)) continue;
+                if (EPI_ALWAYS((N & 3) == 0)) {
                     *reinterpret_cast<f32x4*>(P + (long)m * N + n) = acc[i][j];
                 } else {
 #pragma unroll
@@ -654,35 +663,35 @@
     gemm_epilogue<TM, TN, false, false>(p, acc, m0, n0, wm0, wn0, lane, zb, zslab, none);
 }
 
-template <int TM, int TN>
+template <int TM, int TN, int EPI = EPI_ANY>
 __device__ __forceinline__ void gemm_epilogue_geglu(const GemmParams& p, f32x4 (&acc)[TM][TN], int m0, int n0, int wm0, int wn0, int lane,
                                                     int zb) {
     static_assert(TN % 2 == 0, "GEGLU epilogue needs value/gate tile pairs");
     const int No = p.N >> 1;
     f16* __restrict__ C = p.C + zb * p.strideC;
-    const bool hb32 = p.bias && p.bias_f32, hb16 = p.bias && !p.bias_f32;
+    const bool hb32 = EPI_ON(EPI_BIAS32, p.bias && p.bias_f32), hb16 = EPI_ON(EPI_BIAS16, p.bias && !p.bias_f32);
     f32x4 b32[TN];
     f16x4 b16[TN];
 #pragma unroll
     for (int j = 0; j < TN; j++) {
-        const int n = min(n0 + wn0 + j * 16 + (lane >> 4) * 4, p.N - 4);
+        const int n = EPI_CLAMP(n0 + wn0 + j * 16 + (lane >> 4) * 4, p.N - 4);
         b32[j] = *reinterpret_cast<const f32x4*>(hb32 ? (const float*)p.bias + n : (const float*)p.A);
         b16[j] = *reinterpret_cast<const f16x4*>(hb16 ? (const f16*)p.bias + n : p.A);
     }
 #pragma unroll
     for (int i = 0; i < TM; i++) {
         const int m = m0 + wm0 + i * 16 + (lane & 15);
-        if (m >= p.M) continue;
+        if (EPI_NEVER(m >= p.M)) continue;
 #pragma unroll
         for (int j = 0; j < TN; j += 2) {
             const int n = n0 + wn0 + j * 16 + (lane >> 4) * 4;
-            if (n >= p.N) continue;
+            if (EPI_NEVER(n >= p.N)) continue;
             const int c = ((n0 + wn0 + j * 16) >> 1) + (lane >> 4) * 4;
             f16x4 o;
 #pragma unroll
             for (int r = 0; r < 4; r++) {
-                const float v = acc[i][j][r] + (p.bias ? (hb32 ? b32[j][r] : (float)b16[j][r]) : -0.0f);
-                const float g = acc[i][j + 1][r] + (p.bias ? (hb32 ? b32[j + 1][r] : (float)b16[j + 1][r]) : -0.0f);
+                const float v = acc[i][j][r] + (EPI_ON(EPI_BIAS16 | EPI_BIAS32, p.bias != nullptr) ? (hb32 ? b32[j][r] : (float)b16[j][r]) : -0.0f);
+                const float g = acc[i][j + 1][r] + (EPI_ON(EPI_BIAS16 | EPI_BIAS32, p.bias != nullptr) ? (hb32 ? b32[j + 1][r] : (float)b16[j + 1][r]) : -0.0f);
                 o[r] = (f16)(v * osg_gelu_erf(g));
             }
             *reinterpret_cast<f16x4*>(C + (long)m * No + c) = o;
@@ -764,6 +773,22 @@
 }
 
 int launch_splitk_reduce(osg_ctx* ctx, const GemmParams& p, int batch);
+inline int no_epi_prefetch();
+inline EpiLaunch epi_launch_of(const GemmParams& p, int batch) {
+    EpiLaunch l;
+    l.M = p.M; l.N = p.N; l.batch = batch; l.splits = p.splits; l.fold = p.fold_acc != 0;
+    l.bias = p.bias != nullptr; l.bias_f32 = p.bias_f32 != 0; l.rowbias = p.rowbias != nullptr; l.residual = p.residual != nullptr; l.c2 = p.C2 != nullptr;
+    l.rowstats = p.rs_out != nullptr; l.sinks = p.sink[0].table || p.sink[1].table; l.act = (int)p.act;
+    l.other = no_epi_prefetch() != 0;
+    l.ldc = p.ldc; l.ldc2 = p.C2 ? p.ldc2 : 0; l.rb_ld = p.rb_ld; l.rs_np = p.rs_np;
+    l.align_or = (uintptr_t)p.C | (uintptr_t)p.C2 | (uintptr_t)p.residual | (uintptr_t)p.rowbias | (uintptr_t)p.bias | (uintptr_t)p.rs_out;
+    return l;
+}
+inline bool epi_generic_forced() {
+    const char* e = getenv("OSG_EPI_GENERIC");
+    return e && atoi(e) != 0;
+}
+int launch_v2_lean(int lean, osg_ctx* ctx, GemmParams& p, int batch);
 template <int UNIT> int launch_v2_unit(int entry, osg_ctx* ctx, GemmParams& p, int batch);
 template <> int launch_v2_unit<0>(int entry, osg_ctx* ctx, GemmParams& p, int batch);
 template <> int launch_v2_unit<1>(int entry, osg_ctx* ctx, GemmParams& p, int batch);
diff --git a/onnxstream_amd/csrc/osg_gemm_epi.h b/onnxstream_amd/csrc/osg_gemm_epi.h
--- /dev/null
+++ b/onnxstream_amd/csrc/osg_gemm_epi.h
@@ -0,0 +1,123 @@
+#pragma once
+#include "osg_gemm_routes.h"
+#include <cstdint>
+
+namespace osg_mm {
+
+enum : int {
+    EPI_BIAS16 = 1,
+    EPI_BIAS32 = 2,
+    EPI_ROWBIAS = 4,
+    EPI_RESIDUAL = 8,
+    EPI_SILU = 16,
+    EPI_C2 = 32,
+    EPI_ROWSTATS = 64,
+    EPI_SPLIT = 128,
+    EPI_FOLD = 256,
+    EPI_GEGLU = 512,
+    EPI_SINKS = 1024,
+    EPI_OTHER = 2048,
+};
+constexpr int EPI_ANY = -1;
+constexpr int kEpiLeanBits = EPI_BIAS16 | EPI_BIAS32 | EPI_ROWBIAS | EPI_RESIDUAL | EPI_SILU | EPI_C2 | EPI_ROWSTATS | EPI_SPLIT | EPI_GEGLU;
+
+struct EpiLaunch {
+    int M = 0, N = 0, batch = 1, splits = 1;
+    bool fold = false;
+    bool bias = false, bias_f32 = false, rowbias = false, residual = false, c2 = false, rowstats = false, sinks = false;
+    int act = 0;
+    bool other = false;
+    long ldc = 0, ldc2 = 0, rb_ld = 0;
+    int rs_np = 0;
+    uintptr_t align_or = 0;
+};
+
+constexpr int epi_form(const EpiLaunch& l) {
+    if (l.other || l.batch != 1) return EPI_OTHER;
+    if (l.splits > 1 && !l.fold) return EPI_SPLIT;
+    int m = 0;
+    if (l.splits > 1) m |= EPI_FOLD;
+    if (l.bias) m |= l.bias_f32 ? EPI_BIAS32 : EPI_BIAS16;
+    if (l.rowbias) m |= EPI_ROWBIAS;
+    if (l.residual) m |= EPI_RESIDUAL;
+    if (l.act == 1) m |= EPI_SILU;
+    else if (l.act == 3) m |= EPI_GEGLU;
+    else if (l.act != 0) m |= EPI_OTHER;
+    if (l.c2) m |= EPI_C2;
+    if (l.rowstats) m |= EPI_ROWSTATS;
+    if (l.sinks) m |= EPI_SINKS;
+    return m;
+}
+constexpr bool epi_whole(const EpiLaunch& l, int bm, int bn) {
+    return l.M > 0 && l.N > 0 && l.M % bm == 0 && l.N % bn == 0 && (l.ldc & 3) == 0 && (l.ldc2 & 3) == 0 && (!l.rowbias || (l.rb_ld & 3) == 0) && (l.align_or & 7) == 0 &&
+           (!l.rowstats || l.rs_np * 32 == l.N);
+}
+
+struct LeanEntry { V2Entry e; int mask; };
+constexpr bool v2_same(const V2Entry& a, const V2Entry& b) {
+    return a.bm == b.bm && a.bn == b.bn && a.nst == b.nst && a.conv == b.conv && a.spec == b.spec && a.ln == b.ln && a.nch == b.nch && a.ks == b.ks && a.wgn == b.wgn && a.wq == b.wq;
+}
+constexpr int v2_index(const V2Entry& e) {
+    for (int i = 0; i < kV2Count; i++)
+        if (v2_same(kV2Entries[i], e)) return i;
+    return -1;
+}
+constexpr bool lean_holds(const V2Entry& e, int mask) {
+    if (mask == EPI_ANY || (mask & ~kEpiLeanBits)) return false;
+    if ((mask & EPI_BIAS16) && (mask & EPI_BIAS32)) return false;
+    if ((mask & EPI_SPLIT) && (mask != EPI_SPLIT || e.ln != 0)) return false;
+    if (e.ln != 0 && !(mask & EPI_BIAS32)) return false;
+    if ((mask & (EPI_ROWSTATS | EPI_GEGLU)) && (e.bn / e.wgn) % 32 != 0) return false;
+    if ((mask & EPI_GEGLU) && (mask & ~(EPI_GEGLU | EPI_BIAS16 | EPI_BIAS32))) return false;
+    return true;
+}
+
+inline constexpr LeanEntry kLeanEntries[] = {
+    {{64, 64, 4, 0, 0, 0, 5, 1, 2, 0}, EPI_BIAS16 | EPI_RESIDUAL | EPI_ROWSTATS},
+    {{64, 80, 4, 0, 0, 0, 5, 1, 1, 0}, EPI_BIAS16 | EPI_RESIDUAL},
+    {{64, 64, 4, 0, 0, 2, 20, 1, 2, 0}, EPI_BIAS32},
+    {{64, 64, 4, 0, 0, 0, 5, 2, 2, 0}, EPI_BIAS16 | EPI_ROWSTATS},
+    {{64, 64, 2, 0, 0, 0, 5, 1, 2, 0}, EPI_BIAS16 | EPI_ROWSTATS},
+    {{64, 64, 4, 0, 0, 0, 5, 1, 2, 0}, EPI_BIAS16 | EPI_ROWSTATS},
+    {{128, 128, 4, 0, 1, 2, 10, 1, 2, 0}, EPI_BIAS32},
+    {{64, 64, 4, 0, 0, 2, 10, 1, 2, 0}, EPI_BIAS32},
+    {{128, 64, 4, 0, 0, 2, 20, 1, 2, 0}, EPI_BIAS32},
+    {{128, 64, 2, 0, 0, 2, 10, 1, 2, 0}, EPI_BIAS32 | EPI_GEGLU},
+    {{128, 160, 4, 0, 0, 2, 20, 1, 1, 0}, EPI_BIAS32 | EPI_GEGLU},
+    {{128, 80, 4, 0, 0, 0, 5, 1, 1, 0}, EPI_SPLIT},
+    {{64, 64, 4, 0, 0, 0, 5, 1, 2, 0}, EPI_SPLIT},
+    {{64, 80, 4, 0, 0, 0, 5, 1, 1, 0}, EPI_BIAS16},
+    {{64, 64, 4, 0, 0, 0, 5, 1, 2, 0}, EPI_BIAS16},
+    {{64, 64, 4, 0, 0, 0, 5, 1, 2, 0}, EPI_BIAS16 | EPI_RESIDUAL},
+    {{128, 80, 4, 0, 0, 0, 5, 1, 1, 0}, EPI_BIAS16},
+    {{64, 80, 4, 0, 0, 0, 5, 1, 1, 0}, EPI_BIAS16 | EPI_RESIDUAL | EPI_C2},
+    {{64, 64, 4, 0, 0, 0, 5, 1, 2, 0}, EPI_BIAS16 | EPI_RESIDUAL | EPI_C2},
+    {{64, 64, 6, 0, 0, 0, 5, 1, 2, 0}, EPI_BIAS16 | EPI_RESIDUAL | EPI_ROWSTATS},
+    {{128, 64, 4, 0, 0, 2, 20, 1, 2, 0}, EPI_BIAS32 | EPI_GEGLU},
+    {{64, 64, 4, 1, 0, 0, 5, 2, 2, 0}, EPI_BIAS16 | EPI_C2},
+    {{64, 64, 4, 1, 0, 0, 5, 2, 2, 0}, EPI_SPLIT},
+    {{64, 128, 4, 1, 0, 0, 5, 1, 2, 0}, EPI_SPLIT},
+};
+inline constexpr int kLeanCount = sizeof(kLeanEntries) / sizeof(kLeanEntries[0]);
+
+constexpr bool lean_list_ok() {
+    for (int i = 0; i < kLeanCount; i++) {
+        if (v2_index(kLeanEntries[i].e) < 0 || !lean_holds(kLeanEntries[i].e, kLeanEntries[i].mask)) return false;
+        for (int j = 0; j < i; j++)
+            if (v2_same(kLeanEntries[i].e, kLeanEntries[j].e) && kLeanEntries[i].mask == kLeanEntries[j].mask) return false;
+    }
+    return true;
+}
+static_assert(lean_list_ok(), "kLeanEntries: every pair names an entry of kV2Entries and a mask the kernel compiles lean, once");
+
+constexpr int select_epi(int entry, const EpiLaunch& l, bool force_generic) {
+    if (force_generic || entry < 0 || entry >= kV2Count) return -1;
+    const V2Entry& e = kV2Entries[entry];
+    const int form = epi_form(l);
+    if (!lean_holds(e, form) || !epi_whole(l, e.bm, e.bn)) return -1;
+    for (int i = 0; i < kLeanCount; i++)
+        if (kLeanEntries[i].mask == form && v2_same(kLeanEntries[i].e, e)) return i;
+    return -1;
+}
+
+}
diff --git a/onnxstream_amd/csrc/osg_gemm_lean.hip b/onnxstream_amd/csrc/osg_gemm_lean.hip
--- /dev/null
+++ b/onnxstream_amd/csrc/osg_gemm_lean.hip
@@ -0,0 +1,17 @@
+#include "osg_gemm2.h"
+
+namespace {
+template <int I>
+constexpr V2Launch lean_launcher() {
+    constexpr V2Entry e = kLeanEntries[I].e;
+    return launch_v2<e.bm, e.bn, e.nst, e.conv != 0, 0, e.spec, e.ln, e.nch, e.ks, e.wgn, e.wq, kLeanEntries[I].mask>;
+}
+template <size_t... I>
+constexpr std::array<V2Launch, kLeanCount> lean_launchers(std::index_sequence<I...>) { return {lean_launcher<(int)I>()...}; }
+}
+
+int osg_mm::launch_v2_lean(int lean, osg_ctx* ctx, GemmParams& p, int batch) {
+    static constexpr std::array<V2Launch, kLeanCount> table = lean_launchers(std::make_index_sequence<kLeanCount>{});
+    if (lean < 0 || lean >= kLeanCount) OSG_FAIL(ctx, "osg_gemm: no such lean epilogue variant");
+    return table[lean](ctx, p, batch);
+}
diff --git a/onnxstream_amd/osgpu.py b/onnxstream_amd/osgpu.py
--- a/onnxstream_amd/osgpu.py
+++ b/onnxstream_amd/osgpu.py
@@ -19,7 +19,7 @@
     "osg_device_count", "osg_init", "osg_destroy", "osg_last_error", "osg_device_name", "osg_stream", "osg_set_autotune", "osg_tune_misses",
     "osg_malloc", "osg_free", "osg_upload", "osg_upload_sync", "osg_host_register", "osg_host_unregister", "osg_upload_pinned", "osg_upload_pinned_async", "osg_copy_fence", "osg_download", "osg_copy", "osg_memset", "osg_sync",
     "osg_graph_begin", "osg_graph_end", "osg_graph_launch", "osg_graph_destroy", "osg_timer_start", "osg_timer_stop",
-    "osg_conv2d_nhwc", "osg_conv2d_nhwc_rb", "osg_conv2d_nhwc_v", "osg_gemm", "osg_gemm_ln", "osg_gemm_rowstats", "osg_last_route", "osg_last_kernel", "osg_gemm_kernarg_check", "osg_attention_kernarg_check", "osg_gemm_w8", "osg_conv2d_nhwc_w8", "osg_gemm_w8_v", "osg_conv2d_nhwc_w8_v", "osg_transpose_kn_to_nk", "osg_attention", "osg_attention_strided", "osg_sdpa", "osg_rms_norm", "osg_rope",
+    "osg_conv2d_nhwc", "osg_conv2d_nhwc_rb", "osg_conv2d_nhwc_v", "osg_gemm", "osg_gemm_ln", "osg_gemm_rowstats", "osg_last_route", "osg_last_epilogue", "osg_last_kernel", "osg_gemm_kernarg_check", "osg_attention_kernarg_check", "osg_gemm_w8", "osg_conv2d_nhwc_w8", "osg_gemm_w8_v", "osg_conv2d_nhwc_w8_v", "osg_transpose_kn_to_nk", "osg_attention", "osg_attention_strided", "osg_sdpa", "osg_rms_norm", "osg_rope",
     "osg_instance_norm", "osg_group_norm_nhwc", "osg_layer_norm", "osg_reduce_mean_last", "osg_softmax_last",
     "osg_unary", "osg_binary", "osg_geglu", "osg_transpose", "osg_copy_2d", "osg_concat2", "osg_resize_nearest", "osg_gather_rows",
     "osg_maxpool_nhwc", "osg_convert", "osg_sampler_prepare", "osg_sampler_cfg_euler_a", "osg_sampler_cfg_multistep", "osg_sampler_prepare_rescale",
@@ -106,6 +106,8 @@
     lib.osg_gemm_rowstats.argtypes = [vp, vp, vp, vp, ci, vp, vp, ci, ci, ci, ci, vp]
     lib.osg_last_route.argtypes = [vp, ctypes.POINTER(ci)]
     lib.osg_last_kernel.argtypes = [vp, ctypes.POINTER(ci)]
+    if hasattr(lib, "osg_last_epilogue"):
+        lib.osg_last_epilogue.argtypes = [vp, ctypes.POINTER(ci)]
     if hasattr(lib, "osg_gemm_kernarg_check"):
         lib.osg_gemm_kernarg_check.argtypes = [vp, cl, ci]
         lib.osg_attention_kernarg_check.argtypes = [vp, cl, ci, ci]
@@ -224,6 +226,11 @@
         self._ck(self.lib.osg_last_route(self.ctx, r))
         return tuple(r)
 
+    def last_epilogue(self):
+        r = (ctypes.c_int * 2)()
+        self._ck(self.lib.osg_last_epilogue(self.ctx, r))
+        return tuple(r)
+
     def last_kernel(self):
         r = (ctypes.c_int * 8)()
         self._ck(self.lib.osg_last_kernel(self.ctx, r))
```

Result: faster. 10.21, median of 6 (+1.8%).
